# cortes-ciriano-lab/DeMethify

Hardware: AMD Instinct MI355X
Metric: NMF update iters/sec (1e6 CpG x 256 samples x 16 types) (higher is better)
Workload: dtype f64; 1 GPU; headline_1e6x256_12+4; N_cpg=1000000, S_samples=256, n_known=12, n_unknown=4, inner_iters=20, restarts=64, restart_seed=1 + k, restart_placement=k mod n_gpus, parallelism=restart-sharded x1

## Files before the change

demethify_amd/_lib.py:

```python
from __future__ import annotations

import ctypes as C
from pathlib import Path

LIB_PATH = Path(__file__).resolve().parent / "libdemethify_hip.so"

DMF_OK = 0
DMF_PTR_DEVICE = 1
DMF_INIT_IN_UNIT_RANGE = 4
DMF_SELECT_COUNTS_F32_EXACT, DMF_SELECT_PURITY, DMF_SELECT_ALPHA_OUTSIDE_UNIT, DMF_SELECT_V_UNALIGNED = 1, 2, 4, 8
DMF_SELECT_X16 = 16
DMF_COUNTS_F64 = 2
DMF_WLS_TARGET_V, DMF_WLS_TARGET_DV = 0, 1
DMF_WLS_F64_ARRAYS = 8
DMF_ERR_BAD_ARG, DMF_ERR_NONFINITE, DMF_ERR_UNSUPPORTED = 1, 4, 5
DMF_ERR_BAD_SHAPE = 2
DMF_GRAM_INTEGER, DMF_GRAM_FP64, DMF_GRAM_LAST = 0, 1, 2
DMF_ROUTE_SOLVER, DMF_ROUTE_UPDATE_U = 0, 1
MOMENTUM_SCALARS = ("a1", "a2", "l_w", "l_w_prev", "l_h", "l_h_prev", "dsq", "rt_norm2", "u_norm2", "cf", "cf_prev",
                    "iters", "done", "arrive", "mom_n", "mom_i")
REPORT_INTS = ("N", "S", "n_c", "ND", "SD", "N16", "plane_stride", "has_D16", "has_X16", "has_W16", "has_Dt8", "has_mask_bits",
               "rtp_width", "rtp_borrows_rt", "n_test", "d_f32_exact")
REPORT_DBLS = ("kDsq", "kRtSumsq", "kDmax", "kF32ResidualMax", "kIntCountMax", "kRtOutsideUnit", "x16_dev", "x16_sum")
PROBLEM_ARRAYS = {"V": 0, "D": 1, "Rt": 2, "Rtp": 3, "D16": 4, "X16": 5, "W16": 6, "Dt8": 7, "mask_bits": 8, "consts": 9}
DMF_MODE_PARTIAL = 0
DMF_MODE_UNSUPERVISED = 1
MAX_K = 64
SVD_MAX_S, SVD_MAX_NC, SVD_MAX_RANK, SVD_MAX_LDS = 512, 64, 64, 160 * 1024


def svd_project_lds_bytes(n_samples, rank):
    return 8 * (n_samples * rank + 8 * ((n_samples + 63) // 64 * 64 + 16) + 512)


KERNEL_ROWPASS, KERNEL_GRAM, KERNEL_ALPHA, KERNEL_COST = 0, 1, 2, 3
KERNEL_FAMILIES = ("rowpass", "gram", "alpha", "cost")

_p = C.c_void_p
_i64 = C.c_int64
_dbl_p = C.POINTER(C.c_double)

SIGNATURES = {
    "dmf_status_string": (C.c_char_p, [C.c_int]),
    "dmf_last_error": (C.c_char_p, []),
    "dmf_abi_version": (C.c_int, []),
    "dmf_context_create": (C.c_int, [C.c_int, _p, C.POINTER(_p)]),
    "dmf_context_destroy": (C.c_int, [_p]),
    "dmf_context_synchronize": (C.c_int, [_p]),
    "dmf_context_set_profiling": (C.c_int, [_p, C.c_int]),
    "dmf_context_kernel_time": (C.c_int, [_p, C.c_int, _dbl_p, C.POINTER(_i64)]),
    "dmf_context_reset_kernel_time": (C.c_int, [_p]),
    "dmf_context_set_generic": (C.c_int, [_p, C.c_int]),
    "dmf_context_set_x16": (C.c_int, [_p, C.c_int]),
    "dmf_context_set_rowpass_pair": (C.c_int, [_p, C.c_int]),
    "dmf_context_set_stop_confirmation": (C.c_int, [_p, C.c_int]),
    "dmf_problem_create": (C.c_int, [_p, _i64, _i64, _i64, _p, _p, _p, C.c_int, C.POINTER(_p)]),
    "dmf_problem_gather": (C.c_int, [_p, _p, _p, _i64, C.POINTER(_p)]),
    "dmf_problem_gather_device": (C.c_int, [_p, _p, _p, _i64, C.POINTER(_p)]),
    "dmf_problem_mask": (C.c_int, [_p, _p, _p, C.c_int, C.POINTER(_p)]),
    "dmf_solver_holdout_error": (C.c_int, [_p, _p, _dbl_p, C.POINTER(_i64)]),
    "dmf_problem_destroy": (C.c_int, [_p]),
    "dmf_problem_shape": (C.c_int, [_p, C.POINTER(_i64), C.POINTER(_i64), C.POINTER(_i64)]),
    "dmf_problem_gram_known": (C.c_int, [_p, _p, C.c_char_p, _i64]),
    "dmf_problem_report": (C.c_int, [_p, C.POINTER(_i64), _dbl_p]),
    "dmf_problem_copy_out": (C.c_int, [_p, C.c_int, _p, _i64]),
    "dmf_gram_i8_describe": (C.c_int, [_i64, _i64, _i64, _i64, C.c_int, C.c_char_p, _i64]),
    "dmf_solver_gram": (C.c_int, [_p, C.c_int, _p, C.c_char_p, _i64]),
    "dmf_solver_row_moments": (C.c_int, [_p, _p, C.c_char_p, _i64]),
    "dmf_solver_momentum_state": (C.c_int, [_p, _dbl_p, _p, _p]),
    "dmf_cost": (C.c_int, [_p, _p, _p, _i64, _p, C.c_int, _dbl_p]),
    "dmf_cost_describe": (C.c_int, [_i64, _i64, _i64, C.c_int, _i64, C.c_int, C.c_int, C.c_int, C.c_char_p, _i64]),
    "dmf_problem_cost_describe": (C.c_int, [_p, _p, _i64, C.c_char_p, _i64]),
    "dmf_project_simplex": (C.c_int, [_p, _p, _i64, _i64, C.c_double, C.c_int, _p]),
    "dmf_update_u": (C.c_int, [_p, _p, _p, _p, _p, _i64, _i64, C.c_int, C.c_int, _dbl_p, _p, _p]),
    "dmf_update_alpha": (C.c_int, [_p, _p, _p, _i64, _p, _p, _i64, C.c_int, _dbl_p, _p, _p]),
    "dmf_wls_intercept": (C.c_int, [_p, _p, _p, _i64, C.c_int, C.c_int, _p, C.POINTER(C.c_int)]),
    "dmf_svd_gram": (C.c_int, [_p, _p, _p, C.c_int, _p, C.POINTER(_i64)]),
    "dmf_svd_factor": (C.c_int, [_p, _p, _p, _p, _i64, C.c_int, _p, C.POINTER(_p)]),
    "dmf_svd_finish": (C.c_int, [_p, _p, _i64, _i64, _p, _p, C.c_int, _p]),
    "dmf_percentile_axis0": (C.c_int, [_p, _p, _i64, _i64, _p, _i64, C.c_int, _p]),
    "dmf_solver_create": (C.c_int, [_p, _p, _p, _p, _i64, C.c_int, C.c_int, C.POINTER(_p)]),
    "dmf_solver_set_purity": (C.c_int, [_p, _p, C.c_int]),
    "dmf_solver_step": (C.c_int, [_p, _i64, _i64, C.c_double, C.POINTER(_i64), C.POINTER(C.c_int)]),
    "dmf_solver_get": (C.c_int, [_p, C.c_int, _p, _p, _dbl_p, C.POINTER(_i64)]),
    "dmf_solver_match_components": (C.c_int, [_p, _p, _i64, _p, _p]),
    "dmf_solver_get_u_permuted": (C.c_int, [_p, C.POINTER(C.c_int32), _p]),
    "dmf_solver_cost": (C.c_int, [_p, _dbl_p]),
    "dmf_solver_cost_begin": (C.c_int, [_p]),
    "dmf_solver_cost_end": (C.c_int, [_p, _dbl_p]),
    "dmf_solver_destroy": (C.c_int, [_p]),
    "dmf_solver_describe": (C.c_int, [_p, _i64, C.c_char_p, _i64]),
    "dmf_select_describe": (C.c_int, [_i64, _i64, _i64, _i64, C.c_int, C.c_int, _i64, C.c_int, C.c_char_p, _i64]),
    "dmf_u_phase_describe": (C.c_int, [_i64, _i64, _i64, _i64, C.c_int, C.c_int, _i64, C.c_int, C.c_int, C.c_char_p, _i64]),
    "dmf_solver_u_phase_describe": (C.c_int, [_p, _i64, C.c_int, C.c_char_p, _i64]),
    "dmf_solver_stop_info": (C.c_int, [_p, C.POINTER(C.c_int), C.POINTER(_i64), C.POINTER(_i64), _dbl_p]),
    "dmf_solver_rowpass_launches": (C.c_int, [_p, C.POINTER(_i64), C.POINTER(_i64)]),
    "dmf_table_scan": (C.c_int, [C.c_char_p, C.c_char, C.POINTER(_i64), C.POINTER(C.c_int), C.POINTER(C.c_int),
                                 C.POINTER(C.c_int)]),
    "dmf_table_read": (C.c_int, [C.c_char_p, C.c_char, C.c_int, C.c_int, _i64, _p, _i64, C.c_double, _p, _i64, C.c_int]),
    "dmf_host_alloc": (_p, [C.c_size_t, C.POINTER(C.c_int)]),
    "dmf_host_free": (None, [_p, C.c_int]),
    "dmf_write_interval_csv": (C.c_int, [C.c_char_p, C.c_char_p, _p, _p, _i64, C.c_int, C.c_int, C.c_int]),
    "dmf_stage_upload": (C.c_int, [_p, _p, C.c_size_t, C.POINTER(C.c_void_p)]),
    "dmf_stage_free": (C.c_int, [_p, _p]),
    "dmf_stage_download": (C.c_int, [_p, _p, C.c_size_t, _p]),
    "dmf_mask_draw": (C.c_int, [_p, _p, C.POINTER(C.c_int), _i64, _i64, C.c_uint64, C.POINTER(C.c_void_p),
                                C.POINTER(_i64)]),
    "dmf_solve": (C.c_int, [_p, _p, _p, _p, _i64, C.c_int, _i64, _i64, C.c_double, C.c_int, _p, _p,
                            _dbl_p, C.POINTER(_i64)]),
}

_lib = None


class DemethifyHipError(RuntimeError):

    def __init__(self, status: int, where: str, detail: str = ""):
        self.status = status
        msg = f"{where}: status {status}"
        if detail:
            msg += f" ({detail})"
        super().__init__(msg)


def _preload_torch_hip_runtime():
    import importlib.util
    import os

    if os.environ.get("DEMETHIFY_SYSTEM_HIP") == "1":
        return
    try:
        spec = importlib.util.find_spec("torch")
        if spec is None or not spec.submodule_search_locations:
            return
        cand = Path(list(spec.submodule_search_locations)[0]) / "lib" / "libamdhip64.so"
        if cand.exists():
            C.CDLL(str(cand), mode=C.RTLD_GLOBAL)
    except Exception:
        pass


def load():
    global _lib
    if _lib is not None:
        return _lib
    if not LIB_PATH.exists():
        raise ImportError(
            f"{LIB_PATH} is missing: build it with `python -m demethify_amd._build` "
            "(there is no CPU fallback)")
    import sys

    torch = sys.modules.get("torch")
    if torch is not None:
        try:
            if torch.cuda.is_available():
# ... 21 lines not shown
```

demethify_amd/csrc/dmf_api.h:

```cpp
#pragma once
#include <hip/hip_runtime.h>

#include <cmath>
#include <cstdio>
#include <cstdlib>
#include <cstring>
#include <memory>
#include <mutex>
#include <new>
#include <unordered_map>
#include <utility>
#include <vector>

#include "../../include/demethify_hip.h"
#include "dmf_internal.h"
#include "dmf_select.h"

using dmf::SolverState;

namespace dmf_api {

int hip_fail(hipError_t e, const char* what, const char* file, int line);

#define HIP_TRY(expr)                                                                          \
    do {                                                                                       \
        hipError_t e_ = (expr);                                                                \
        if (e_ != hipSuccess) return dmf_api::hip_fail(e_, #expr, __FILE_NAME__, __LINE__);    \
    } while (0)

#define DMF_TRY(expr)                 \
    do {                              \
        int s_ = (expr);              \
        if (s_ != DMF_OK) return s_;  \
    } while (0)

constexpr int kEventPool = 2048;

struct FamilyClock {
    std::vector<hipEvent_t> start, stop;
    int used = 0;
    double total_ms = 0.0;
    int64_t launches = 0;
};

}

struct dmf_context {
    int device = 0;
    hipStream_t stream = nullptr;
    bool own_stream = false;
    unsigned profiling = 0;
    int stop_confirmation = 0;
    int generic_level = 0;
    bool x16 = true;
    bool rowpass_pair = true;
    double* scratch = nullptr;
    hipMemPool_t pool = nullptr;
    std::unordered_map<void*, size_t> live;
    std::unordered_map<size_t, std::vector<void*>> kept;
    size_t kept_bytes = 0;
    std::vector<hipEvent_t> events;
    std::vector<double*> pinned_moms;
    std::vector<void*> pinned_states;
    hipStream_t copy_stream = nullptr;
    std::mutex copy_mutex;
    dmf_api::FamilyClock clocks[DMF_KERNEL_FAMILIES];
};

namespace dmf_api {

hipError_t pool_alloc(dmf_context* ctx, void** p, size_t bytes);
void pool_free(dmf_context* ctx, void* p);
hipError_t stage_alloc(dmf_context* ctx, hipStream_t st, void** p, size_t bytes);
void stage_release(dmf_context* ctx, hipStream_t st, void* p);

template <class T>
class DevBuf {
  public:
    DevBuf() = default;
    DevBuf(DevBuf&& o) noexcept : ctx_(o.ctx_), ptr_(o.ptr_), owned_(o.owned_), stage_(o.stage_) {
        o.ptr_ = nullptr, o.owned_ = false;
    }
    DevBuf& operator=(DevBuf&& o) noexcept {
        if (this != &o) {
            reset();
            ctx_ = o.ctx_, ptr_ = o.ptr_, owned_ = o.owned_, stage_ = o.stage_;
            o.ptr_ = nullptr, o.owned_ = false;
        }
        return *this;
    }
    ~DevBuf() { reset(); }
    hipError_t alloc(dmf_context* ctx, size_t count) {
        reset();
        const hipError_t e = pool_alloc(ctx, (void**)&ptr_, count * sizeof(T));
        if (e != hipSuccess) ptr_ = nullptr;
        ctx_ = ctx, owned_ = e == hipSuccess, stage_ = nullptr;
        return e;
    }
    hipError_t alloc_staged(dmf_context* ctx, size_t count, hipStream_t st) {
        reset();
        const hipError_t e = stage_alloc(ctx, st, (void**)&ptr_, count * sizeof(T));
        if (e != hipSuccess) ptr_ = nullptr;
        ctx_ = ctx, owned_ = e == hipSuccess, stage_ = st;
        return e;
    }
    T* release() {
        T* p = ptr_;
        ptr_ = nullptr, owned_ = false;
        return p;
    }
    void borrow(const T* p) { reset(), ptr_ = const_cast<T*>(p); }
    void reset() {
        if (owned_ && stage_ != nullptr) stage_release(ctx_, stage_, ptr_);
        else if (owned_) pool_free(ctx_, ptr_);
        ptr_ = nullptr, owned_ = false;
    }
    T* get() const { return ptr_; }
    operator T*() const { return ptr_; }
    T* operator->() const { return ptr_; }

  private:
    dmf_context* ctx_ = nullptr;
    T* ptr_ = nullptr;
    bool owned_ = false;
    hipStream_t stage_ = nullptr;
};

enum ProblemConst { kDsq, kRtSumsq, kDmax, kF32ResidualMax, kIntCountMax, kRtOutsideUnit, kProblemConsts };

struct JobTable {
    std::vector<short> h_k, h_l;
    std::vector<int> h_dst;
    DevBuf<short> k, l;
    DevBuf<int> dst;
    int n = 0;
    template <class Keep>
    void build(int l_first, int l_last, Keep keep) {
        for (int ll = l_first; ll <= l_last; ++ll)
            for (int kk = 0; kk <= ll; ++kk) {
                if (!keep(kk, ll)) continue;
                h_k.push_back((short)kk);
                h_l.push_back((short)ll);
                h_dst.push_back(dmf::tri(kk, ll));
            }
        n = (int)h_k.size();
    }
    int upload(dmf_context* ctx) {
        HIP_TRY(k.alloc(ctx, n));
        HIP_TRY(l.alloc(ctx, n));
        HIP_TRY(dst.alloc(ctx, n));
        HIP_TRY(hipMemcpyAsync(k, h_k.data(), n * sizeof(short), hipMemcpyHostToDevice, ctx->stream));
        HIP_TRY(hipMemcpyAsync(l, h_l.data(), n * sizeof(short), hipMemcpyHostToDevice, ctx->stream));
        HIP_TRY(hipMemcpyAsync(dst, h_dst.data(), n * sizeof(int), hipMemcpyHostToDevice, ctx->stream));
        return DMF_OK;
    }
};

}

struct dmf_problem {
    dmf_context* ctx = nullptr;
    int64_t N = 0, S = 0, n_c = 0;
    dmf_api::DevBuf<double> V, D, Rt;
    dmf_api::DevBuf<double> Rtp;
    dmf_api::DevBuf<double> consts;
    double h_consts[dmf_api::kProblemConsts] = {};
    dmf_api::DevBuf<unsigned short> D16;
    dmf_api::DevBuf<signed char> Dt8;
    int ND = 0;
    int SD = 0;
    int64_t N16 = 0, plane_stride = 0;
    dmf_api::DevBuf<unsigned short> X16;
    double x16_dev = 0.0, x16_sum = 0.0;
    bool d_f32_exact = false;
    dmf_api::DevBuf<double> gb_known;
    dmf::GramRan known_ran;
    dmf_api::DevBuf<unsigned char> mask_bits;
    dmf_api::DevBuf<unsigned short> W16;
    int64_t n_test = 0;
    dmf::ProblemView view() const {
        dmf::ProblemView v;
        v.V = V, v.D = D, v.D16 = D16, v.X16 = X16, v.Dt8 = Dt8;
        v.plane_stride = plane_stride, v.SD = SD, v.ND = ND;
        v.Rt = Rt, v.Rtp = Rtp;
        v.N = N, v.S = (int)S, v.n_c = (int)n_c;
        return v;
    }
};

constexpr size_t kPinnedStateBytes = (sizeof(SolverState) + 15) / 16 * 16 + 16;

struct dmf_solver {
    dmf_context* ctx = nullptr;
    const dmf_problem* p = nullptr;
    int64_t n_u = 0;
    int mode = 0;
    dmf::ShapeKey key;
    dmf::PathSpec spec;
    dmf_api::DevBuf<double> cm;
    dmf_api::DevBuf<double> beta_tab;
    int64_t beta_cap = 0;
    dmf_api::DevBuf<long long> slab_i8;
    int64_t slab_i8_words = 0;
    dmf_api::DevBuf<long long> acc_i8;
    dmf_api::DevBuf<double> purity;
    dmf_api::DevBuf<double> u2_partials;
    dmf_api::DevBuf<double> u, u_prev, u_next;
    dmf_api::DevBuf<double> alpha, alpha_prev;
    dmf_api::DevBuf<double> gb;
    dmf::GramRan last_gram;
    int last_gram_source = -1;
    dmf_api::DevBuf<double> slab;
    int64_t slab_doubles = 0;
    dmf_api::DevBuf<double> partials;
    dmf_api::DevBuf<SolverState> state;
    SolverState* h_state = nullptr;
    dmf_api::JobTable jobs;
    bool cf_pending = true;
    double* mom_host = nullptr;
    dmf_api::DevBuf<double> mom_dev;
    hipEvent_t cost_event = nullptr;
    bool cost_pending = false;
    bool in_flight = false;
    bool confirm_stops = false;
    double cf_stream = 0.0;
    long long cf_stream_iter = -1;
    long long n_rowpass = 0, n_rowpass_pair = 0;
    long long n_confirmed = 0, n_unconfirmed = 0;
    dmf::IterateView iterate() const {
        dmf::IterateView it;
        it.u = u, it.u_prev = u_prev, it.alpha = alpha, it.state = state;
        it.n_u = (int)n_u, it.mode = mode;
        return it;
    }
    dmf::AlphaView alpha_view() const {
        dmf::AlphaView a;
        a.gb = gb, a.alpha = alpha, a.alpha_prev = alpha_prev, a.purity = purity, a.state = state, a.partials = partials;
        a.S = (int)p->S, a.n_c = (int)p->n_c, a.n_u = (int)n_u;
        return a;
    }
    dmf::UScratch scratch() const {
        dmf::UScratch sc;
        sc.cm = cm, sc.beta = beta_tab, sc.slab = slab, sc.u2_partials = u2_partials;
        return sc;
    }
};

namespace dmf_api {

struct HandleDeleter {
    void operator()(dmf_problem* p) const { dmf_problem_destroy(p); }
    void operator()(dmf_solver* s) const { dmf_solver_destroy(s); }
};
using ProblemPtr = std::unique_ptr<dmf_problem, HandleDeleter>;
using SolverPtr = std::unique_ptr<dmf_solver, HandleDeleter>;

int clock_drain(dmf_context* ctx, FamilyClock& c);

struct FamilyScope {
    dmf_context* ctx;
    FamilyClock* c = nullptr;
    int slot = -1;
    FamilyScope(dmf_context* ctx_, int family) : ctx(ctx_) {
        if (!((ctx->profiling >> family) & 1u)) return;
        c = &ctx->clocks[family];
        if (c->start.empty()) {
            c->start.resize(kEventPool);
            c->stop.resize(kEventPool);
            for (int i = 0; i < kEventPool; ++i) {
                hipEventCreateWithFlags(&c->start[i], hipEventDisableSystemFence);
                hipEventCreateWithFlags(&c->stop[i], hipEventDisableSystemFence);
            }
        }
        if (c->used == kEventPool) clock_drain(ctx, *c);
        slot = c->used++;
        hipEventRecord(c->start[slot], ctx->stream);
    }
    ~FamilyScope() {
        if (c != nullptr) hipEventRecord(c->stop[slot], ctx->stream);
    }
};

int check_ctx(dmf_context* ctx);

template <class T>
int import_array(dmf_context* ctx, const void* src, size_t count, int flags, DevBuf<T>& dst) {
    dst.reset();
    if (count == 0) return DMF_OK;
    if (flags & DMF_PTR_DEVICE) {
        dst.borrow(static_cast<const T*>(src));
        return DMF_OK;
    }
    HIP_TRY(dst.alloc(ctx, count));
    HIP_TRY(hipMemcpyAsync(dst, src, count * sizeof(T), hipMemcpyHostToDevice, ctx->stream));
    HIP_TRY(hipStreamSynchronize(ctx->stream));
    return DMF_OK;
}
int export_array(dmf_context* ctx, const void* dev_src, size_t bytes, int flags, void* dst);

hipError_t enqueue_cost(dmf_context* ctx, const dmf::ProblemView& p, const double* u, const double* alpha, int n_u,
                        double* scratch, double* out);
// ... 14 lines not shown
```

demethify_amd/csrc/dmf_api_context.hip:

```cpp
#include "dmf_api.h"

namespace dmf_api {

static thread_local char g_last_error[512] = "";

int hip_fail(hipError_t e, const char* what, const char* file, int line) {
    snprintf(g_last_error, sizeof(g_last_error), "%s failed at %s:%d: %s", what, file, line, hipGetErrorString(e));
    return DMF_ERR_HIP;
}

int clock_drain(dmf_context* ctx, FamilyClock& c) {
    if (c.used == 0) return DMF_OK;
    HIP_TRY(hipStreamSynchronize(ctx->stream));
    for (int i = 0; i < c.used; ++i) {
        float ms = 0.f;
        HIP_TRY(hipEventElapsedTime(&ms, c.start[i], c.stop[i]));
        c.total_ms += ms;
    }
    c.launches += c.used;
    c.used = 0;
    return DMF_OK;
}

static bool pool_enabled() {
// ... 206 lines not shown
    if (ctx == nullptr || key == nullptr || pos == nullptr || out_bits == nullptr || n_kept == nullptr) return DMF_ERR_BAD_ARG;
    *out_bits = nullptr;
    if (*pos < 0 || *pos > 624 || N < 1 || S < 1 || threshold > ((uint64_t)1 << 53)) return DMF_ERR_BAD_ARG;
    if (S > dmf::kMaskDrawMaxS || N > dmf::kMaskDrawMaxElements / S) return DMF_ERR_UNSUPPORTED;
    HIP_TRY(hipSetDevice(ctx->device));
    std::lock_guard<std::mutex> lock(ctx->copy_mutex);
    if (ctx->copy_stream == nullptr) HIP_TRY(hipStreamCreateWithFlags(&ctx->copy_stream, hipStreamNonBlocking));
    const hipStream_t st = ctx->copy_stream;
    constexpr size_t kStateWords = 624 + 4;
    DevBuf<unsigned char> bits;
    DevBuf<uint32_t> state;
    HIP_TRY(bits.alloc_staged(ctx, (size_t)N * (size_t)((S + 7) / 8), st));
    HIP_TRY(state.alloc_staged(ctx, kStateWords, st));
    uint32_t h_state[kStateWords] = {};
    std::memcpy(h_state, key, 624 * sizeof(uint32_t));
    HIP_TRY(hipMemcpyAsync(state, h_state, sizeof(h_state), hipMemcpyHostToDevice, st));
    HIP_TRY(dmf::launch_mask_draw(state, *pos, N, S, threshold, bits, reinterpret_cast<unsigned long long*>(state + 624), st));
    HIP_TRY(hipMemcpyAsync(h_state, state, sizeof(h_state), hipMemcpyDeviceToHost, st));
    HIP_TRY(hipStreamSynchronize(st));
    unsigned long long result[2];
    std::memcpy(result, h_state + 624, sizeof(result));
    std::memcpy(key, h_state, 624 * sizeof(uint32_t));
    *pos = (int)result[1];
    *n_kept = (int64_t)result[0];
    *out_bits = bits.release();
    return DMF_OK;
}

int dmf_stage_free(dmf_context* ctx, void* dev) {
    if (ctx == nullptr) return DMF_ERR_BAD_ARG;
    if (dev == nullptr) return DMF_OK;
    HIP_TRY(hipSetDevice(ctx->device));
    pool_free(ctx, dev);
    return DMF_OK;
}

int dmf_context_synchronize(dmf_context* ctx) {
    DMF_TRY(check_ctx(ctx));
    HIP_TRY(hipStreamSynchronize(ctx->stream));
    return DMF_OK;
}

int dmf_context_set_profiling(dmf_context* ctx, int enabled) {
    DMF_TRY(check_ctx(ctx));
    if (!enabled)
        for (auto& c : ctx->clocks) DMF_TRY(clock_drain(ctx, c));
    ctx->profiling = enabled == 0 ? 0u : enabled == 1 ? ~0u : (unsigned)enabled >> 1;
    return DMF_OK;
}

int dmf_context_kernel_time(dmf_context* ctx, int family, double* total_ms, int64_t* launches) {
    DMF_TRY(check_ctx(ctx));
    if (family < 0 || family >= DMF_KERNEL_FAMILIES) return DMF_ERR_BAD_ARG;
    FamilyClock& c = ctx->clocks[family];
    DMF_TRY(clock_drain(ctx, c));
    if (total_ms) *total_ms = c.total_ms;
    if (launches) *launches = c.launches;
    return DMF_OK;
}

int dmf_context_reset_kernel_time(dmf_context* ctx) {
    DMF_TRY(check_ctx(ctx));
    for (auto& c : ctx->clocks) {
        DMF_TRY(clock_drain(ctx, c));
        c.total_ms = 0.0;
        c.launches = 0;
    }
    return DMF_OK;
}

int dmf_context_set_generic(dmf_context* ctx, int enabled) {
    if (ctx == nullptr) return DMF_ERR_BAD_ARG;
    if (enabled < 0 || enabled > 4) return DMF_ERR_BAD_ARG;
    ctx->generic_level = enabled;
    return DMF_OK;
}

int dmf_context_set_x16(dmf_context* ctx, int enabled) {
    if (ctx == nullptr || enabled < 0 || enabled > 1) return DMF_ERR_BAD_ARG;
    ctx->x16 = enabled != 0;
    return DMF_OK;
}

int dmf_context_set_rowpass_pair(dmf_context* ctx, int enabled) {
    if (ctx == nullptr || enabled < 0 || enabled > 1) return DMF_ERR_BAD_ARG;
    ctx->rowpass_pair = enabled != 0;
    return DMF_OK;
}

int dmf_context_set_stop_confirmation(dmf_context* ctx, int mode) {
    if (ctx == nullptr || mode < 0 || mode > 2) return DMF_ERR_BAD_ARG;
    ctx->stop_confirmation = mode;
    return DMF_OK;
}

}
```

demethify_amd/csrc/dmf_api_entry.hip:

```cpp
#include "dmf_api.h"

using namespace dmf_api;

static double advance_momentum(double a, int64_t n) {
    for (int64_t t = 0; t < n; ++t) a = (1.0 + std::sqrt(1.0 + 4.0 * a * a)) / 2.0;
    return a;
}

static dmf::PercentilePlan percentile_plan(int64_t n, double q_percent) {
#pragma clang fp contract(off)
    dmf::PercentilePlan pl{};
    const double quantile = q_percent / 100.0;
    const double vi = (double)(n - 1) * quantile;
    if (vi >= (double)(n - 1)) {
        pl.k_prev = pl.k_next = n - 1;
        pl.gamma = 0.0;
    } else if (vi < 0.0) {
        pl.k_prev = pl.k_next = 0;
        pl.gamma = 0.0;
    } else {
        const double fl = std::floor(vi);
        pl.k_prev = (long long)fl;
        pl.k_next = pl.k_prev + 1;
        pl.gamma = vi - fl;
    }
    return pl;
}

static int result_array(dmf_context* ctx, double* out, size_t count, int flags, DevBuf<double>& dst) {
    if (flags & DMF_PTR_DEVICE) dst.borrow(out);
    else HIP_TRY(dst.alloc(ctx, count));
    return DMF_OK;
}
static int deliver_result(dmf_context* ctx, const double* dev, size_t count, int flags, double* out) {
    if (!(flags & DMF_PTR_DEVICE)) HIP_TRY(hipMemcpyAsync(out, dev, count * sizeof(double), hipMemcpyDeviceToHost, ctx->stream));
    HIP_TRY(hipStreamSynchronize(ctx->stream));
    return DMF_OK;
}

extern "C" {

static int select_key(int64_t N, int64_t S, int64_t n_c, int64_t n_u, int nd, int level, int64_t n_iter2, int flags,
                      const char* buf, int64_t cap, dmf::ShapeKey& key) {
    if (buf == nullptr || cap < 1 || N < 1 || S < 1 || n_c < 0 || n_u < 1 || nd < 0 || nd > 2 || n_iter2 < 0 ||
        n_c + n_u > dmf::kMaxK)
        return DMF_ERR_BAD_ARG;
    key.N = N;
    key.S = (int)S;
    key.n_c = (int)n_c;
    key.n_u = (int)n_u;
    key.nd = (S >= 2 && S <= 2048 && n_c <= 48) ? nd : 0;
    key.SD = key.nd > 0 ? (int)((S + 63) / 64 * 64) : 0;
    key.level = level;
    key.d_f32_exact = (flags & DMF_SELECT_COUNTS_F32_EXACT) != 0;
    key.rtp_present = true;
    key.v_align = (flags & DMF_SELECT_V_UNALIGNED) ? 8 : 0;
    key.x16 = key.nd > 0 && (flags & DMF_SELECT_X16) != 0;
    key.rtp_align = 0;
    key.alpha_unit = !(flags & DMF_SELECT_ALPHA_OUTSIDE_UNIT);
    return DMF_OK;
}

int dmf_u_phase_describe(int64_t N, int64_t S, int64_t n_c, int64_t n_u, int nd, int level, int64_t n_iter2, int flags, int route,
                         char* buf, int64_t cap) {
    dmf::ShapeKey key;
    if (n_iter2 > (1 << 20) || S > (1 << 24) || (route != DMF_ROUTE_SOLVER && route != DMF_ROUTE_UPDATE_U)) return DMF_ERR_BAD_ARG;
    DMF_TRY(select_key(N, S, n_c, n_u, nd, level, n_iter2, flags, buf, cap, key));
    const dmf::PathSpec spec = dmf::select_path(key);
    if (!spec.supported) return DMF_ERR_UNSUPPORTED;
    dmf::describe_u_phase(key, spec, (int)n_iter2, (flags & DMF_SELECT_PURITY) != 0, route == DMF_ROUTE_UPDATE_U, buf, (size_t)cap);
    return DMF_OK;
}

int dmf_select_describe(int64_t N, int64_t S, int64_t n_c, int64_t n_u, int nd, int level, int64_t n_iter2, int flags,
                        char* buf, int64_t cap) {
    dmf::ShapeKey key;
    DMF_TRY(select_key(N, S, n_c, n_u, nd, level, n_iter2, flags, buf, cap, key));
    const dmf::PathSpec spec = dmf::select_path(key);
    if (!spec.supported) return DMF_ERR_UNSUPPORTED;
    const dmf::IterationPlan plan = dmf::plan_iteration(key, spec, (int)n_iter2, (flags & DMF_SELECT_PURITY) != 0);
    dmf::describe_plan(key, plan, buf, (size_t)cap);
    return DMF_OK;
}

int dmf_cost_describe(int64_t S, int64_t n_c, int64_t n_u, int has_u16, int64_t SD, int v_align, int rtp_present, int level,
                      char* buf, int64_t cap) {
    if (buf == nullptr || cap < 1 || S < 1 || S > (1 << 24) || n_c < 0 || n_u < 0 || n_c + n_u < 1 || n_c + n_u > dmf::kMaxK ||
        SD < 0 || SD > (1 << 24) || (has_u16 && SD < S) || v_align < 0 || v_align > 15 || level < 0 || level > 4)
        return DMF_ERR_BAD_ARG;
    dmf::CostKey key;
    key.S = (int)S;
    key.n_c = (int)n_c;
    key.n_u = (int)n_u;
    key.d16 = has_u16 != 0;
    key.SD = (int)SD;
    key.v_align = (unsigned)v_align;
    key.rtp_present = rtp_present != 0;
    key.level = level;
    dmf::describe_cost_plan(dmf::cost_plan(key), buf, (size_t)cap);
    return DMF_OK;
}

int dmf_gram_i8_describe(int64_t N, int64_t S, int64_t n_c, int64_t n_u, int nd, char* buf, int64_t cap) {
    if (buf == nullptr || cap < 1 || N < 1 || S < 1 || S > (1 << 24) || n_c < 0 || n_u < 0 || n_c + n_u < 1 ||
        n_c + n_u > dmf::kMaxK)
        return DMF_ERR_BAD_ARG;
    const dmf::GramI8Plan g = dmf::gram_i8_plan(N, (int)((S + 63) / 64 * 64), (int)n_c, (int)n_u, nd);
    if (!g.supported) return DMF_ERR_UNSUPPORTED;
    dmf::describe_gram_i8_plan(g, buf, (size_t)cap);
    return DMF_OK;
}

int dmf_cost(dmf_context* ctx, const dmf_problem* p, const double* u, int64_t n_u, const double* alpha,
             int flags, double* out_cost) {
    DMF_TRY(check_ctx(ctx));
    if (p == nullptr || alpha == nullptr || out_cost == nullptr || n_u < 0) return DMF_ERR_BAD_ARG;
    if (n_u > 0 && u == nullptr) return DMF_ERR_BAD_ARG;
    const int64_t K = p->n_c + n_u;
    if (K < 1) return DMF_ERR_BAD_ARG;
    DevBuf<double> du, da, dout;
    DMF_TRY(import_array(ctx, u, (size_t)p->N * n_u, flags, du));
    DMF_TRY(import_array(ctx, alpha, (size_t)K * p->S, flags, da));
    HIP_TRY(dout.alloc(ctx, 1));
    {
        FamilyScope scope(ctx, DMF_KERNEL_COST);
        HIP_TRY(enqueue_cost(ctx, p->view(), du, da, (int)n_u, ctx->scratch + 1024, dout));
    }
    HIP_TRY(hipMemcpyAsync(out_cost, dout, sizeof(double), hipMemcpyDeviceToHost, ctx->stream));
    HIP_TRY(hipStreamSynchronize(ctx->stream));
    return DMF_OK;
}

int dmf_project_simplex(dmf_context* ctx, const double* X, int64_t K, int64_t S, double z, int flags,
                        double* out) {
    DMF_TRY(check_ctx(ctx));
    if (X == nullptr || out == nullptr || K < 1 || S < 1) return DMF_ERR_BAD_ARG;
    if (K > dmf::kMaxK) return DMF_ERR_UNSUPPORTED;
    const size_t count = (size_t)K * S;
    DevBuf<double> dx, dout;
    DMF_TRY(import_array(ctx, X, count, flags, dx));
    DMF_TRY(result_array(ctx, out, count, flags, dout));
    HIP_TRY(dmf::launch_project_simplex(dx, dout, (int)K, (int)S, z, ctx->stream));
    return deliver_result(ctx, dout, count, flags, out);
}

int dmf_percentile_axis0(dmf_context* ctx, const double* x, int64_t n, int64_t m, const double* q, int64_t n_q,
                         int flags, double* out) {
    DMF_TRY(check_ctx(ctx));
    if (x == nullptr || q == nullptr || out == nullptr || n < 1 || m < 1 || n_q < 1) return DMF_ERR_BAD_ARG;
    for (int64_t i = 0; i < n_q; ++i)
        if (!(q[i] >= 0.0 && q[i] <= 100.0)) return DMF_ERR_BAD_ARG;
    if (n > dmf::percentile_max_replicates()) return DMF_ERR_UNSUPPORTED;
    DevBuf<double> dx, dout;
    DMF_TRY(import_array(ctx, x, (size_t)n * m, flags, dx));
    DMF_TRY(result_array(ctx, out, (size_t)n_q * m, flags, dout));
    for (int64_t i = 0; i < n_q; i += 2) {
        const dmf::PercentilePlan p0 = percentile_plan(n, q[i]);
        const bool two = i + 1 < n_q;
        const dmf::PercentilePlan p1 = two ? percentile_plan(n, q[i + 1]) : p0;
        HIP_TRY(dmf::launch_percentile_pair(dx, n, m, p0, p1, dout + i * m, two ? dout + (i + 1) * m : nullptr, ctx->stream));
    }
    return deliver_result(ctx, dout, (size_t)n_q * m, flags, out);
}

int dmf_update_u(dmf_context* ctx, const dmf_problem* p, const double* u, const double* u_prev,
                 const double* alpha, int64_t n_u, int64_t n_iter2, int mode, int flags,
                 double* scalars_io, double* out_u, double* out_u_prev) {
    if (u_prev == nullptr || scalars_io == nullptr || out_u == nullptr || out_u_prev == nullptr || n_iter2 < 0)
        return DMF_ERR_BAD_ARG;
    dmf_solver* raw = nullptr;
    DMF_TRY(dmf_solver_create(ctx, p, u, alpha, n_u, mode, flags, &raw));
    SolverPtr s(raw);
    const size_t un = (size_t)p->N * n_u * sizeof(double);
    const hipMemcpyKind in_kind = (flags & DMF_PTR_DEVICE) ? hipMemcpyDeviceToDevice : hipMemcpyHostToDevice;
    HIP_TRY(hipMemcpyAsync(s->u_prev, u_prev, un, in_kind, ctx->stream));
    DMF_TRY(fetch_state(raw));
    s->h_state->a1 = scalars_io[0];
    s->h_state->l_w_prev = scalars_io[1];
    s->h_state->l_w = scalars_io[2];
    DMF_TRY(push_state(raw));
    DMF_TRY(enqueue_u_phase(raw, (int)n_iter2, standalone_row_kind(raw, (int)n_iter2)));
    DMF_TRY(export_array(ctx, s->u, un, flags, out_u));
    DMF_TRY(export_array(ctx, s->u_prev, un, flags, out_u_prev));
// ... 34 lines not shown
```

demethify_amd/csrc/dmf_api_problem.hip:

```cpp
#include "dmf_api.h"

namespace dmf_api {

static int alloc_count_copies(dmf_problem* p, int ND, bool x16, bool w16) {
    dmf_context* ctx = p->ctx;
    p->ND = ND;
    p->SD = (int)((p->S + 63) / 64 * 64);
    p->N16 = (p->N + 15) / 16 * 16;
    p->plane_stride = ((p->N + 31) / 32) * (p->SD / 32) * 1024;
    const size_t u16_elems = (size_t)p->N16 * p->SD;
    HIP_TRY(p->D16.alloc(ctx, u16_elems));
    HIP_TRY(p->Dt8.alloc(ctx, (size_t)p->plane_stride * ND));
    if (x16) HIP_TRY(p->X16.alloc(ctx, u16_elems));
    if (w16) HIP_TRY(p->W16.alloc(ctx, u16_elems));
    return DMF_OK;
}

static void known_route(dmf_problem* p, const char* piece) {
    char* t = p->known_ran.text;
    const size_t have = std::strlen(t), cap = sizeof(p->known_ran.text);
    snprintf(t + have, cap - have, "%s%s", have > 0 ? " " : "", piece);
}

static int problem_finalize(dmf_problem* p, bool counts_done = false) {
    dmf_context* ctx = p->ctx;
    const int64_t N = p->N, S = p->S, n_c = p->n_c;
    double* const h = p->h_consts;
    HIP_TRY(p->consts.alloc(ctx, kProblemConsts));
    if (!counts_done) HIP_TRY(dmf::launch_max_f64(p->D, N * S, ctx->scratch, p->consts + kDmax, ctx->stream));
    if (n_c > 0) {
        HIP_TRY(dmf::launch_sumsq_f64(p->Rt, N * n_c, ctx->scratch + 1024, p->consts + kRtSumsq, nullptr, ctx->stream));
    } else {
        HIP_TRY(hipMemsetAsync(p->consts + kRtSumsq, 0, sizeof(double), ctx->stream));
    }
    if (!counts_done) {
        HIP_TRY(dmf::launch_f32_residual_max(p->D, N * S, ctx->scratch + 2048, p->consts + kF32ResidualMax, ctx->stream));
        HIP_TRY(dmf::launch_int_count_max(p->D, N * S, ctx->scratch + 3072, p->consts + kIntCountMax, ctx->stream));
        if (n_c > 0) {
            HIP_TRY(dmf::launch_unit_range_check(p->Rt, N * n_c, ctx->scratch, p->consts + kRtOutsideUnit, ctx->stream));
        } else {
            HIP_TRY(hipMemsetAsync(p->consts + kRtOutsideUnit, 0, sizeof(double), ctx->stream));
        }
    }
    {
        double got[kProblemConsts];
        HIP_TRY(hipMemcpyAsync(got, p->consts, sizeof(got), hipMemcpyDeviceToHost, ctx->stream));
        HIP_TRY(hipStreamSynchronize(ctx->stream));
        h[kRtSumsq] = got[kRtSumsq];
        if (!counts_done)
            for (int i = kDmax; i < kProblemConsts; ++i) h[i] = got[i];
    }
    h[kDsq] = h[kDmax] * h[kDmax];
    p->d_f32_exact = h[kF32ResidualMax] == 0.0;
    HIP_TRY(hipMemcpyAsync(p->consts, h, kProblemConsts * sizeof(double), hipMemcpyHostToDevice, ctx->stream));
    HIP_TRY(hipStreamSynchronize(ctx->stream));
    if (!std::isfinite(h[kDmax]) || !std::isfinite(h[kRtSumsq])) return DMF_ERR_NONFINITE;

    if (!counts_done && ctx->generic_level == 0 && h[kIntCountMax] <= 32639.0 && h[kRtOutsideUnit] == 0.0 && S >= 2 &&
        S <= 2048 && n_c <= 48) {
        DMF_TRY(alloc_count_copies(p, h[kIntCountMax] <= 127.0 ? 1 : 2, ctx->x16, false));
        DevBuf<unsigned long long> x_stats;
        if (ctx->x16) HIP_TRY(x_stats.alloc(ctx, 3));
        HIP_TRY(dmf::launch_build_counts_int(p->D, p->V, N, (int)S, p->ND, p->D16, p->X16, p->N16, p->SD, p->Dt8,
                                             p->plane_stride, x_stats, ctx->stream));
        if (p->X16 != nullptr) {
            unsigned long long got[3] = {1, 0, 0};
            HIP_TRY(hipMemcpyAsync(got, x_stats, sizeof(got), hipMemcpyDeviceToHost, ctx->stream));
            HIP_TRY(hipStreamSynchronize(ctx->stream));
            if (got[0] != 0) {
                p->X16.reset();
            } else {
                std::memcpy(&p->x16_dev, &got[1], sizeof(double));
                p->x16_sum = (double)got[2];
            }
        }
    }

    if (n_c > 0 && n_c <= 48) {
        const int nct = (int)((n_c + 3) / 4 * 4);
        if (nct == n_c) {
            p->Rtp.borrow(p->Rt);
        } else {
            HIP_TRY(p->Rtp.alloc(ctx, (size_t)N * nct));
            HIP_TRY(dmf::launch_pad_rows(p->Rt, p->Rtp, N, (int)n_c, nct, ctx->stream));
        }
    }

    const dmf::ProblemView pv = p->view();
    JobTable jobs;
    jobs.build(0, (int)n_c, [](int, int) { return true; });
    const int n_jobs = jobs.n;
    const bool mfma = n_c >= 1 && ctx->generic_level != 1 && ctx->generic_level != 2;
    const int n_fast = mfma ? n_jobs - 1 : 0, n_dense = (int)(n_c * (n_c + 1) / 2);
    const bool int_known = mfma && ctx->generic_level == 0 && p->Dt8 != nullptr && p->D16 != nullptr && p->Rtp != nullptr &&
                           (reinterpret_cast<uintptr_t>(p->Rtp.get()) & 15) == 0 &&
                           dmf::gram_i8_known_supported((int)n_c, p->ND, N, p->SD);
    int64_t slab_doubles = dmf::gram_slab_doubles(N, (int)S, mfma ? 1 : n_jobs);
    if (mfma && !int_known) {
        const int64_t need = dmf::gram_mfma_slab_doubles(N, (int)S, n_fast);
        if (need > slab_doubles) slab_doubles = need;
    }
    DevBuf<double> slab, slab_bu;
    DevBuf<long long> slab_i8, acc;
    HIP_TRY(p->gb_known.alloc(ctx, (size_t)n_jobs * S));
    DMF_TRY(jobs.upload(ctx));
    HIP_TRY(slab.alloc(ctx, (size_t)slab_doubles));
    bool vdv_done = true;
    if (int_known) {
        const int64_t slab_words = dmf::gram_i8_slab_words_nf(N, p->SD, n_dense);
        const int64_t acc_words = dmf::gram_i8_acc_words_nf((int)S, n_dense, (int)n_c + 1);
        HIP_TRY(slab_i8.alloc(ctx, (size_t)slab_words));
        HIP_TRY(acc.alloc(ctx, (size_t)acc_words));
        HIP_TRY(slab_bu.alloc(ctx, (size_t)dmf::bu_cols_grid(N) * (n_c + 1) * S));
        HIP_TRY(hipMemsetAsync(acc, 0, (size_t)acc_words * sizeof(long long), ctx->stream));
        int ny = 0, n_slabs = 0;
        dmf::GramRan ran;
        HIP_TRY(dmf::launch_gram_i8(pv, nullptr, 0, jobs.k, jobs.l, n_dense, slab_i8, slab_words, nullptr, &ny, ctx->stream, &ran));
        known_route(p, "int_known");
        known_route(p, ran.text);
        HIP_TRY(dmf::launch_bu_cols(pv, p->Rt, (int)n_c, slab_bu, nullptr, &n_slabs, ctx->stream, &vdv_done));
        known_route(p, vdv_done ? "+ k_bu_cols2 with vDv" : "+ k_bu_cols");
        HIP_TRY(dmf::launch_gram_v2_reduce(slab_i8, ny, n_dense, p->SD, slab_bu, n_slabs, (int)n_c + (vdv_done ? 1 : 0), (int)S,
                                           acc, jobs.dst, p->gb_known, nullptr, nullptr, 0, nullptr, ctx->stream));
    } else if (mfma) {
        dmf::GramJobTable fast{jobs.k, jobs.l, jobs.dst, n_fast};
        int ny = 0;
        dmf::GramRan ran;
        HIP_TRY(dmf::launch_gram_mfma(pv, nullptr, 0, fast, n_dense, slab, slab_doubles, nullptr, &ny, ctx->stream, &ran));
        known_route(p, "fp64");
        known_route(p, ran.text);
        HIP_TRY(dmf::launch_gram_reduce(slab, ny, n_fast, (int)S, jobs.dst, p->gb_known, nullptr, ctx->stream));
    }
    if (int_known && vdv_done) {
    } else if (n_jobs - n_fast == 1 && ctx->generic_level != 1 && ctx->generic_level != 2 &&
               (int64_t)dmf::vdv_cols_grid(N) * S <= slab_doubles) {
        HIP_TRY(dmf::launch_vdv_cols(pv, slab, p->gb_known + (int64_t)jobs.h_dst[n_jobs - 1] * S, ctx->stream));
        known_route(p, p->known_ran.text[0] == 0 ? "fp64 k_vdv_cols" : "+ k_vdv_cols");
    } else {
        dmf::GramJobTable rest{jobs.k + n_fast, jobs.l + n_fast, jobs.dst + n_fast, n_jobs - n_fast};
        dmf::GramRan ran;
        if (p->known_ran.text[0] == 0) known_route(p, "fp64");
        else known_route(p, "+");
        HIP_TRY(dmf::launch_gram(pv, nullptr, 0, rest, slab, slab_doubles, p->gb_known, nullptr, ctx->stream, &ran));
        known_route(p, ran.text);
    }
    HIP_TRY(hipStreamSynchronize(ctx->stream));
    return DMF_OK;
}

static dmf::CostPlan cost_plan_of(dmf_context* ctx, const dmf::ProblemView& p, int n_u) {
    return dmf::cost_plan(dmf::cost_key(p, n_u, ctx->generic_level));
}

hipError_t enqueue_cost(dmf_context* ctx, const dmf::ProblemView& p, const double* u, const double* alpha, int n_u,
                        double* scratch, double* out) {
    return dmf::launch_cost_plan(cost_plan_of(ctx, p, n_u), p, u, alpha, n_u, scratch, out, ctx->stream);
}

bool cost_reads_u16_only(dmf_context* ctx, const dmf::ProblemView& p, int n_u) { return cost_plan_of(ctx, p, n_u).d16; }

int cost_to_host(dmf_context* ctx, const dmf::ProblemView& p, const double* u, const double* alpha, int n_u,
                 double* host_slot, bool wait) {
    {
        FamilyScope scope(ctx, DMF_KERNEL_COST);
        HIP_TRY(enqueue_cost(ctx, p, u, alpha, n_u, ctx->scratch + 1024, ctx->scratch + 3072));
    }
    HIP_TRY(hipMemcpyAsync(host_slot, ctx->scratch + 3072, sizeof(double), hipMemcpyDeviceToHost, ctx->stream));
    if (wait) HIP_TRY(hipStreamSynchronize(ctx->stream));
    return DMF_OK;
}

static int problem_gather(dmf_context* ctx, const dmf_problem* src, const int64_t* idx, int64_t n_idx, bool idx_dev,
                          dmf_problem** out) {
    DevBuf<long long> d_idx;
    if (idx_dev) {
        DevBuf<unsigned int> d_bad;
        unsigned int h_bad = 1;
        HIP_TRY(d_bad.alloc(ctx, 1));
        HIP_TRY(dmf::launch_index_range_check(reinterpret_cast<const long long*>(idx), n_idx, src->N, d_bad, ctx->stream));
        HIP_TRY(hipMemcpyAsync(&h_bad, d_bad, sizeof(h_bad), hipMemcpyDeviceToHost, ctx->stream));
        HIP_TRY(hipStreamSynchronize(ctx->stream));
        if (h_bad != 0) return DMF_ERR_BAD_ARG;
        d_idx.borrow(reinterpret_cast<const long long*>(idx));
    } else {
        HIP_TRY(d_idx.alloc(ctx, (size_t)n_idx));
        HIP_TRY(hipMemcpyAsync(d_idx, idx, (size_t)n_idx * sizeof(long long), hipMemcpyHostToDevice, ctx->stream));
    }
    ProblemPtr p(new (std::nothrow) dmf_problem());
    if (p == nullptr) return DMF_ERR_BAD_ARG;
    p->ctx = ctx;
    p->N = n_idx;
    p->S = src->S;
    p->n_c = src->n_c;
    HIP_TRY(p->V.alloc(ctx, (size_t)n_idx * p->S));
    HIP_TRY(p->D.alloc(ctx, (size_t)n_idx * p->S));
    if (p->n_c > 0) HIP_TRY(p->Rt.alloc(ctx, (size_t)n_idx * p->n_c));
    HIP_TRY(dmf::launch_gather_rows(src->V, p->V, d_idx, n_idx, p->S, ctx->stream));
    HIP_TRY(dmf::launch_gather_rows(src->D, p->D, d_idx, n_idx, p->S, ctx->stream));
    if (p->n_c > 0) HIP_TRY(dmf::launch_gather_rows(src->Rt, p->Rt, d_idx, n_idx, p->n_c, ctx->stream));
    bool counts_done = false;
    if (src->D16 != nullptr && src->ND > 0 && ctx->generic_level == 0) {
        const bool x16 = src->X16 != nullptr && ctx->x16;
        DevBuf<unsigned int> d_max;
        DevBuf<unsigned long long> d_xsum;
        DMF_TRY(alloc_count_copies(p.get(), src->ND, x16, false));
        HIP_TRY(d_max.alloc(ctx, 1));
        if (x16) HIP_TRY(d_xsum.alloc(ctx, 1));
        HIP_TRY(dmf::launch_gather_counts_int(src->D16, x16 ? src->X16.get() : nullptr, d_idx, n_idx, p->SD, p->ND, p->D16,
                                              p->X16, p->N16, p->Dt8, p->plane_stride, d_max, d_xsum, ctx->stream));
        unsigned int h_max = 0;
        unsigned long long h_xsum = 0;
        HIP_TRY(hipMemcpyAsync(&h_max, d_max, sizeof(h_max), hipMemcpyDeviceToHost, ctx->stream));
        if (x16) HIP_TRY(hipMemcpyAsync(&h_xsum, d_xsum, sizeof(h_xsum), hipMemcpyDeviceToHost, ctx->stream));
        HIP_TRY(hipStreamSynchronize(ctx->stream));
        p->h_consts[kDmax] = p->h_consts[kIntCountMax] = (double)h_max;
        p->h_consts[kF32ResidualMax] = src->h_consts[kF32ResidualMax];
        p->h_consts[kRtOutsideUnit] = src->h_consts[kRtOutsideUnit];
        p->x16_dev = x16 ? src->x16_dev : 0.0;
        p->x16_sum = (double)h_xsum;
        counts_done = true;
    }
    HIP_TRY(hipStreamSynchronize(ctx->stream));
    d_idx.reset();
    DMF_TRY(problem_finalize(p.get(), counts_done));
    *out = p.release();
    return DMF_OK;
}

}

using namespace dmf_api;

extern "C" {

int dmf_problem_create(dmf_context* ctx, int64_t N, int64_t S, int64_t n_c, const double* V,
                       const void* counts, const double* Rt, int flags, dmf_problem** out) {
    DMF_TRY(check_ctx(ctx));
    if (out == nullptr) return DMF_ERR_BAD_ARG;
    *out = nullptr;
    if (N <= 0 || S <= 0 || n_c < 0 || V == nullptr || counts == nullptr) return DMF_ERR_BAD_ARG;
    if (n_c > 0 && Rt == nullptr) return DMF_ERR_BAD_ARG;
    if (n_c > dmf::kMaxK || S > (1 << 24)) return DMF_ERR_UNSUPPORTED;
    ProblemPtr p(new (std::nothrow) dmf_problem());
    if (p == nullptr) return DMF_ERR_BAD_ARG;
    p->ctx = ctx;
    p->N = N;
    p->S = S;
    p->n_c = n_c;
    DMF_TRY(import_array(ctx, V, (size_t)N * S, flags, p->V));
    if (flags & DMF_COUNTS_F64) {
        DMF_TRY(import_array(ctx, counts, (size_t)N * S, flags, p->D));
    } else {
        DevBuf<long long> raw;
        DMF_TRY(import_array(ctx, counts, (size_t)N * S, flags, raw));
        HIP_TRY(p->D.alloc(ctx, (size_t)N * S));
        HIP_TRY(dmf::launch_convert_counts(raw, p->D, N * S, ctx->stream));
        HIP_TRY(hipStreamSynchronize(ctx->stream));
    }
    DMF_TRY(import_array(ctx, Rt, (size_t)N * n_c, flags, p->Rt));
    DMF_TRY(problem_finalize(p.get()));
    *out = p.release();
    return DMF_OK;
}

int dmf_problem_gather(dmf_context* ctx, const dmf_problem* src, const int64_t* idx, int64_t n_idx,
                       dmf_problem** out) {
    DMF_TRY(check_ctx(ctx));
    if (src == nullptr || idx == nullptr || out == nullptr || n_idx <= 0) return DMF_ERR_BAD_ARG;
    *out = nullptr;
    if (src->mask_bits != nullptr) return DMF_ERR_BAD_ARG;
    for (int64_t r = 0; r < n_idx; ++r)
        if (idx[r] < 0 || idx[r] >= src->N) return DMF_ERR_BAD_ARG;
    return problem_gather(ctx, src, idx, n_idx, false, out);
}

int dmf_problem_gather_device(dmf_context* ctx, const dmf_problem* src, const int64_t* idx_dev, int64_t n_idx,
                              dmf_problem** out) {
    DMF_TRY(check_ctx(ctx));
    if (src == nullptr || idx_dev == nullptr || out == nullptr || n_idx <= 0) return DMF_ERR_BAD_ARG;
    *out = nullptr;
    if (src->mask_bits != nullptr) return DMF_ERR_BAD_ARG;
    return problem_gather(ctx, src, idx_dev, n_idx, true, out);
}

int dmf_problem_mask(dmf_context* ctx, const dmf_problem* src, const uint8_t* train_bits, int flags, dmf_problem** out) {
    DMF_TRY(check_ctx(ctx));
    if (src == nullptr || train_bits == nullptr || out == nullptr) return DMF_ERR_BAD_ARG;
    *out = nullptr;
    if (src->ctx != ctx || src->mask_bits != nullptr) return DMF_ERR_BAD_ARG;
    ProblemPtr p(new (std::nothrow) dmf_problem());
    if (p == nullptr) return DMF_ERR_BAD_ARG;
    const int64_t N = src->N, S = src->S, n_c = src->n_c;
    p->ctx = ctx;
    p->N = N;
    p->S = S;
    p->n_c = n_c;
    const size_t bit_bytes = (size_t)N * (size_t)((S + 7) / 8), elems = (size_t)N * S;
    HIP_TRY(p->mask_bits.alloc(ctx, bit_bytes));
    HIP_TRY(hipMemcpyAsync(p->mask_bits, train_bits, bit_bytes,
                           (flags & DMF_PTR_DEVICE) ? hipMemcpyDeviceToDevice : hipMemcpyHostToDevice, ctx->stream));
    HIP_TRY(p->V.alloc(ctx, elems));
    HIP_TRY(p->D.alloc(ctx, elems));
    if (n_c > 0) {
        HIP_TRY(p->Rt.alloc(ctx, (size_t)N * n_c));
        HIP_TRY(hipMemcpyAsync(p->Rt, src->Rt, (size_t)N * n_c * sizeof(double), hipMemcpyDeviceToDevice, ctx->stream));
    }
    const bool ints = src->D16 != nullptr && src->ND > 0 && ctx->generic_level == 0;
    const bool x16 = ints && src->X16 != nullptr && ctx->x16;
    if (ints) DMF_TRY(alloc_count_copies(p.get(), src->ND, x16, true));
    DevBuf<unsigned long long> d_stats;
    HIP_TRY(d_stats.alloc(ctx, 3));
    HIP_TRY(dmf::launch_mask_problem(src->V, src->D, ints ? src->D16.get() : nullptr, x16 ? src->X16.get() : nullptr,
                                     p->mask_bits, p->V, p->D, p->D16, p->X16, p->W16, N, p->N16, (int)S, p->SD, d_stats,
                                     ctx->stream));
    if (ints) HIP_TRY(dmf::launch_build_dt8(p->D16, N, p->SD, p->ND, p->Dt8, p->plane_stride, ctx->stream));
    unsigned long long h_stats[3] = {0, 0, 0};
    HIP_TRY(hipMemcpyAsync(h_stats, d_stats, sizeof(h_stats), hipMemcpyDeviceToHost, ctx->stream));
    HIP_TRY(hipStreamSynchronize(ctx->stream));
    d_stats.reset();
    double dmax;
    std::memcpy(&dmax, &h_stats[0], sizeof(dmax));
    p->h_consts[kDmax] = dmax;
    p->h_consts[kF32ResidualMax] = src->h_consts[kF32ResidualMax];
    p->h_consts[kIntCountMax] = std::isfinite(src->h_consts[kIntCountMax]) ? dmax : src->h_consts[kIntCountMax];
    p->h_consts[kRtOutsideUnit] = src->h_consts[kRtOutsideUnit];
    p->x16_dev = x16 ? src->x16_dev : 0.0;
    p->x16_sum = (double)h_stats[1];
    p->n_test = (int64_t)h_stats[2];
    DMF_TRY(problem_finalize(p.get(), true));
    *out = p.release();
    return DMF_OK;
}

int dmf_problem_destroy(dmf_problem* p) {
    if (p == nullptr) return DMF_OK;
    hipSetDevice(p->ctx->device);
    delete p;
    return DMF_OK;
}

int dmf_problem_cost_describe(dmf_context* ctx, const dmf_problem* p, int64_t n_u, char* buf, int64_t cap) {
    if (ctx == nullptr || p == nullptr || buf == nullptr || cap < 1 || n_u < 0 || p->ctx != ctx) return DMF_ERR_BAD_ARG;
    if (p->n_c + n_u < 1 || p->n_c + n_u > dmf::kMaxK) return DMF_ERR_BAD_ARG;
    dmf::describe_cost_plan(cost_plan_of(ctx, p->view(), (int)n_u), buf, (size_t)cap);
    return DMF_OK;
}

int dmf_problem_gram_known(const dmf_problem* p, double* out, char* out_text, int64_t cap) {
    if (p == nullptr || out == nullptr || (out_text != nullptr && cap < 1)) return DMF_ERR_BAD_ARG;
    dmf_context* ctx = p->ctx;
    DMF_TRY(check_ctx(ctx));
    const size_t n = (size_t)(p->n_c + 1) * (p->n_c + 2) / 2 * p->S;
    HIP_TRY(hipMemcpyAsync(out, p->gb_known, n * sizeof(double), hipMemcpyDeviceToHost, ctx->stream));
    HIP_TRY(hipStreamSynchronize(ctx->stream));
    if (out_text != nullptr) snprintf(out_text, (size_t)cap, "%s", p->known_ran.text);
    return DMF_OK;
}

int dmf_problem_report(const dmf_problem* p, int64_t* out_ints, double* out_dbls) {
    if (p == nullptr || out_ints == nullptr || out_dbls == nullptr) return DMF_ERR_BAD_ARG;
    const int64_t rtp_width = p->Rtp != nullptr ? (p->n_c + 3) / 4 * 4 : 0;
    const int64_t ints[DMF_REPORT_INTS] = {p->N, p->S, p->n_c, p->ND, p->SD, p->N16, p->plane_stride,
                                           p->D16 != nullptr, p->X16 != nullptr, p->W16 != nullptr, p->Dt8 != nullptr,
                                           p->mask_bits != nullptr, rtp_width,
                                           p->Rtp != nullptr && p->Rtp.get() == p->Rt.get(), p->n_test, p->d_f32_exact};
    std::memcpy(out_ints, ints, sizeof(ints));
    for (int i = 0; i < kProblemConsts; ++i) out_dbls[i] = p->h_consts[i];
    out_dbls[kProblemConsts] = p->x16_dev;
    out_dbls[kProblemConsts + 1] = p->x16_sum;
    return DMF_OK;
}

int dmf_problem_copy_out(const dmf_problem* p, int which, void* out, int64_t bytes) {
    if (p == nullptr || out == nullptr) return DMF_ERR_BAD_ARG;
    dmf_context* ctx = p->ctx;
    DMF_TRY(check_ctx(ctx));
    const size_t elems = (size_t)p->N * p->S, u16_bytes = (size_t)p->N16 * p->SD * sizeof(unsigned short);
    const void* src = nullptr;
    size_t size = 0;
    switch (which) {
        case DMF_ARRAY_V: src = p->V, size = elems * sizeof(double); break;
        case DMF_ARRAY_D: src = p->D, size = elems * sizeof(double); break;
        case DMF_ARRAY_RT: src = p->Rt, size = (size_t)p->N * p->n_c * sizeof(double); break;
        case DMF_ARRAY_RTP: src = p->Rtp, size = (size_t)p->N * ((p->n_c + 3) / 4 * 4) * sizeof(double); break;
        case DMF_ARRAY_D16: src = p->D16, size = u16_bytes; break;
        case DMF_ARRAY_X16: src = p->X16, size = u16_bytes; break;
        case DMF_ARRAY_W16: src = p->W16, size = u16_bytes; break;
        case DMF_ARRAY_DT8: src = p->Dt8, size = (size_t)p->plane_stride * p->ND; break;
        case DMF_ARRAY_MASK_BITS: src = p->mask_bits, size = (size_t)p->N * (size_t)((p->S + 7) / 8); break;
        case DMF_ARRAY_CONSTS: src = p->consts, size = kProblemConsts * sizeof(double); break;
        default: return DMF_ERR_BAD_ARG;
    }
    if (src == nullptr || size == 0) return DMF_ERR_BAD_ARG;
    if (bytes < 0 || (size_t)bytes != size) return DMF_ERR_BAD_SHAPE;
    return export_array(ctx, src, size, 0, out);
}

int dmf_problem_shape(const dmf_problem* p, int64_t* N, int64_t* S, int64_t* n_c) {
    if (p == nullptr) return DMF_ERR_BAD_ARG;
    if (N) *N = p->N;
    if (S) *S = p->S;
    if (n_c) *n_c = p->n_c;
    return DMF_OK;
}

}
```

demethify_amd/csrc/dmf_api_solver.hip:

```cpp
#include "dmf_api.h"

namespace dmf_api {

using dmf::kSplitInnerSteps;

static int ensure_split_scratch(dmf_solver* s, int n_iter2) {
    dmf_context* ctx = s->ctx;
    if (s->cm == nullptr) HIP_TRY(s->cm.alloc(ctx, (size_t)dmf::u_phase_split_cm_doubles(s->p->N, (int)s->n_u)));
    if (s->beta_cap < n_iter2 || s->beta_tab == nullptr) {
        s->beta_cap = n_iter2 > 0 ? n_iter2 : 1;
        HIP_TRY(s->beta_tab.alloc(ctx, (size_t)s->beta_cap));
    }
    return DMF_OK;
}

int enqueue_u_phase(dmf_solver* s, int n_iter2, dmf::RowKind row) {
    dmf_context* ctx = s->ctx;
    const dmf::ProblemView pv = s->p->view();
    FamilyScope scope(ctx, DMF_KERNEL_ROWPASS);
    switch (row) {
        case dmf::RowKind::CmI8InnerRows:
            DMF_TRY(ensure_split_scratch(s, n_iter2));
            HIP_TRY(dmf::launch_u_phase_split_i8(pv, s->iterate(), n_iter2, s->scratch(), ctx->stream));
            return DMF_OK;
// ... 113 lines not shown
    return enqueue_alpha_phase(s, alpha, n_iter2);
}

static int enqueue_outer_iteration(dmf_solver* s, int n_iter2) {
    dmf_context* ctx = s->ctx;
    s->in_flight = true;
    const dmf_problem* p = s->p;
    const int S = (int)p->S;
    const dmf::IterationPlan plan = dmf::plan_iteration(s->key, s->spec, n_iter2, s->purity != nullptr);
    if (plan.row == dmf::RowKind::RowpassV2) {
        int grid = 0;
        bool paired = false;
        {
            FamilyScope scope(ctx, DMF_KERNEL_ROWPASS);
            dmf::ProblemView pv = p->view();
            if (!s->key.x16) pv.X16 = nullptr;
            HIP_TRY(dmf::launch_rowpass_v2(pv, s->iterate(), n_iter2, s->scratch(), &grid, s->key.rowpass_pair, &paired,
                                           ctx->stream));
            ++s->n_rowpass;
            s->n_rowpass_pair += paired ? 1 : 0;
        }
        return enqueue_gram_i8_tail(s, plan.alpha, n_iter2, grid);
    }
    if (plan.row == dmf::RowKind::CmI8InnerBu) {
        int grid = 0;
        DMF_TRY(ensure_split_scratch(s, n_iter2));
        {
            FamilyScope scope(ctx, DMF_KERNEL_ROWPASS);
            HIP_TRY(dmf::launch_u_phase_split_i8_bu(p->view(), s->iterate(), n_iter2, s->scratch(), &grid, ctx->stream));
        }
        return enqueue_gram_i8_tail(s, plan.alpha, n_iter2, grid);
    }
    if (plan.row == dmf::RowKind::RowpassFused) {
        const int64_t n_full = p->N - (p->N & 15), n_tail = p->N - n_full;
        const dmf::ProblemView pv = p->view();
        int grid = 0, ny_tail = 0;
        {
            FamilyScope scope(ctx, DMF_KERNEL_ROWPASS);
            HIP_TRY(dmf::launch_rowpass_fused(pv.rows(0, n_full), s->iterate(), n_iter2, s->scratch(), &grid, ctx->stream));
        }
        if (n_tail > 0) {
            const dmf::ProblemView tail = pv.rows(n_full, n_tail);
            const dmf::IterateView it_tail = s->iterate().rows(n_full);
            HIP_TRY(dmf::launch_u_phase_mfma(tail, it_tail, n_iter2, ctx->stream));
            HIP_TRY(dmf::launch_sumsq_f64(it_tail.u, n_tail * s->n_u, ctx->scratch, s->u2_partials + grid, &s->state->done,
                                          ctx->stream));
            HIP_TRY(dmf::launch_gram_u(tail, it_tail.u, it_tail.n_u, s->slab + (int64_t)2 * grid * s->jobs.n * S,
                                       &s->state->done, &ny_tail, ctx->stream));
        }
        if (dmf::GramRan* ran = last_gram_slot(s, kLastGramFused))
            snprintf(ran->text, sizeof(ran->text), "k_rowpass_fused<%d,%d> phase C slabs=%d%s", (int)(p->n_c + 3) / 4, (int)s->n_u,
                     2 * grid, n_tail > 0 ? " + k_gram_u tail" : "");
        HIP_TRY(dmf::launch_finish_u_norm(s->u2_partials, grid + (n_tail > 0 ? 1 : 0), s->state, ctx->stream));
        {
            FamilyScope scope(ctx, DMF_KERNEL_GRAM);
            HIP_TRY(dmf::launch_gram_reduce(s->slab, 2 * grid + ny_tail, s->jobs.n, S, s->jobs.dst, s->gb,
                                            &s->state->done, ctx->stream));
        }
        return enqueue_alpha_phase(s, plan.alpha, n_iter2);
    }
    DMF_TRY(enqueue_u_phase(s, n_iter2, plan.row));
    HIP_TRY(dmf::launch_sumsq_f64(s->u, p->N * s->n_u, ctx->scratch, &s->state->u_norm2, &s->state->done,
                                  ctx->stream));
    HIP_TRY(dmf::launch_set_lh(s->state, ctx->stream));
    DMF_TRY(enqueue_gram(s, plan.gram, true, last_gram_slot(s, (int)plan.gram)));
    return enqueue_alpha_phase(s, plan.alpha, n_iter2);
}

int fetch_state(dmf_solver* s) {
    HIP_TRY(hipMemcpyAsync(s->h_state, s->state, sizeof(SolverState), hipMemcpyDeviceToHost, s->ctx->stream));
    HIP_TRY(hipStreamSynchronize(s->ctx->stream));
    s->in_flight = false;
    return DMF_OK;
}

int push_state(dmf_solver* s) {
    HIP_TRY(hipMemcpyAsync(s->state, s->h_state, sizeof(SolverState), hipMemcpyHostToDevice, s->ctx->stream));
    HIP_TRY(hipStreamSynchronize(s->ctx->stream));
    return DMF_OK;
}

constexpr int kMomRows = 64, kMomSteps = 64;

__global__ void k_set_momentum(SolverState* state, const double* mom, int stride, int rows, int n) {
    state->mom = mom;
    state->mom_stride = stride;
    state->mom_rows = rows;
    state->mom_i = 0;
    state->mom_n = n;
}

static double momentum_advance(double& a) {
#pragma clang fp contract(off)
    const double a0 = a;
    const double sq = 4.0 * a0 * a0;
    a = (1.0 + std::sqrt(1.0 + sq)) / 2.0;
    return (a0 - 1.0) / a;
}

static int upload_momentum_rows(dmf_solver* s, int rows, int n) {
    dmf_context* ctx = s->ctx;
    const int stride = 2 + 2 * n;
    if (s->mom_host == nullptr) {
        if (!ctx->pinned_moms.empty()) {
            s->mom_host = ctx->pinned_moms.back();
            ctx->pinned_moms.pop_back();
        } else {
            HIP_TRY(hipHostMalloc((void**)&s->mom_host, (size_t)kMomRows * (2 + 2 * kMomSteps) * sizeof(double)));
        }
        HIP_TRY(s->mom_dev.alloc(ctx, (size_t)kMomRows * (2 + 2 * kMomSteps)));
    }
    double a1 = s->h_state->a1, a2 = s->h_state->a2;
    for (int r = 0; r < rows; ++r) {
        double* row = s->mom_host + (size_t)r * stride;
        for (int t = 0; t < n; ++t) {
            row[2 + t] = momentum_advance(a1);
            row[2 + n + t] = momentum_advance(a2);
        }
        row[0] = a1;
        row[1] = a2;
    }
    HIP_TRY(hipMemcpyAsync(s->mom_dev, s->mom_host, (size_t)rows * stride * sizeof(double), hipMemcpyHostToDevice, ctx->stream));
    hipLaunchKernelGGL(k_set_momentum, dim3(1), dim3(1), 0, ctx->stream, s->state.get(), (const double*)s->mom_dev.get(), stride,
                       rows, n);
    HIP_TRY(hipGetLastError());
    return DMF_OK;
}

__global__ void k_set_tol(SolverState* state, double tol, double band) {
    state->tol = tol;
    state->band = band;
}

constexpr double kConfirmBand = 10.0;
constexpr double kGramCostRelErr = 1e-15;

static double* cost_slot(const dmf_solver* s) {
    return reinterpret_cast<double*>(reinterpret_cast<char*>(s->h_state) + kPinnedStateBytes - 16);
}

static int solver_setup(dmf_solver* s, const double* u0, const double* alpha0, int flags) {
    dmf_context* ctx = s->ctx;
    const dmf_problem* p = s->p;
    const int64_t N = p->N, S = p->S, n_c = p->n_c, n_u = s->n_u, K = n_c + n_u;
    dmf::ShapeKey& key = s->key;
    key.N = N;
    key.S = (int)S;
    key.n_c = (int)n_c;
    key.n_u = (int)n_u;
    key.nd = (p->ND > 0 && p->D16 != nullptr) ? p->ND : 0;
    key.SD = p->SD;
    key.x16 = key.nd > 0 && p->X16 != nullptr;
    key.rowpass_pair = ctx->rowpass_pair;
    key.level = ctx->generic_level;
    key.d_f32_exact = p->d_f32_exact;
    key.rtp_present = n_c == 0 || p->Rtp != nullptr;
    key.v_align = (unsigned)(reinterpret_cast<uintptr_t>(p->V.get()) & 15);
    key.rtp_align = (unsigned)(reinterpret_cast<uintptr_t>(p->Rtp.get()) & 15);
    key.alpha_unit = true;
    s->spec = dmf::select_path(key);
    if ((s->spec.use_v2 || s->spec.use_cm_i8) && !(flags & DMF_INIT_IN_UNIT_RANGE)) {
        bool in_unit = true;
        if (flags & DMF_PTR_DEVICE) {
            double outside = 0.0;
            HIP_TRY(dmf::launch_unit_range_check(alpha0, K * S, ctx->scratch, ctx->scratch + 2048, ctx->stream));
            HIP_TRY(hipMemcpyAsync(&outside, ctx->scratch + 2048, sizeof(double), hipMemcpyDeviceToHost, ctx->stream));
            HIP_TRY(hipStreamSynchronize(ctx->stream));
            in_unit = outside == 0.0;
        } else {
            for (int64_t i = 0; i < K * S; ++i)
                if (!(alpha0[i] >= 0.0 && alpha0[i] <= 1.0)) {
                    in_unit = false;
                    break;
                }
        }
        if (!in_unit) {
            key.alpha_unit = false;
            s->spec = dmf::select_path(key);
        }
    }
    if (!s->spec.supported) return DMF_ERR_UNSUPPORTED;
    s->in_flight = true;
    s->jobs.build((int)n_c, (int)K, [n_c, K](int k, int l) {
        if (l == (int)K && k < (int)n_c) return false;
        return !(l == (int)K && k == (int)K);
    });
    const int n_jobs = s->jobs.n;
    s->slab_doubles = dmf::gram_slab_doubles(N, (int)S, n_jobs);
    if (s->spec.use_gram_spec) {
        const int64_t spec = dmf::gram_u_slab_doubles(N, (int)S, (int)n_c, (int)n_u);
        if (spec > s->slab_doubles) s->slab_doubles = spec;
    }
    if (s->spec.use_gram_mfma) {
        const int64_t need = dmf::gram_mfma_slab_doubles(N, (int)S, n_jobs);
        if (need > s->slab_doubles) s->slab_doubles = need;
    }
    if (s->spec.use_fused) {
        const int64_t spec = dmf::rowpass_fused_slab_doubles(N - (N & 15), (int)S, (int)n_c, (int)n_u) +
                             dmf::gram_u_slab_doubles(16, (int)S, (int)n_c, (int)n_u);
        if (spec > s->slab_doubles) s->slab_doubles = spec;
    }
    if (s->spec.use_v2) {
        const int64_t bu = (int64_t)dmf::rowpass_v2_grid(N, (int)S) * n_u * S;
        if (bu > s->slab_doubles) s->slab_doubles = bu;
    }
    if (s->spec.use_gram_i8) {
        const int64_t bu = (int64_t)dmf::bu_cols_grid(N) * n_u * S;
        if (bu > s->slab_doubles) s->slab_doubles = bu;
        if (s->spec.use_cm_i8) {
            const int64_t bu2 = (int64_t)dmf::u_inner_bu_grid(N, (int)S) * n_u * S;
            if (bu2 > s->slab_doubles) s->slab_doubles = bu2;
        }
    }
    const size_t un = (size_t)N * n_u, an = (size_t)K * S;
    const size_t un_alloc = (un + 1) & ~(size_t)1;
    const size_t gbn = (size_t)(K + 1) * (K + 2) / 2 * S;
    const int nb_alpha = (int)((S + 63) / 64);
    HIP_TRY(s->u.alloc(ctx, un_alloc));
    HIP_TRY(s->u_prev.alloc(ctx, un_alloc));
    if (s->spec.u_path == 2) HIP_TRY(s->u_next.alloc(ctx, un_alloc));
    HIP_TRY(s->alpha.alloc(ctx, an));
    HIP_TRY(s->alpha_prev.alloc(ctx, an));
    HIP_TRY(s->gb.alloc(ctx, gbn));
    HIP_TRY(s->slab.alloc(ctx, (size_t)s->slab_doubles));
    HIP_TRY(s->partials.alloc(ctx, (size_t)2 * (nb_alpha + S)));
    HIP_TRY(s->u2_partials.alloc(ctx, 4096));
    if (s->spec.use_v2 || s->spec.use_gram_i8) {
        s->slab_i8_words = dmf::gram_i8_slab_words(N, p->SD, (int)n_c, (int)n_u);
        HIP_TRY(s->slab_i8.alloc(ctx, (size_t)s->slab_i8_words));
        const size_t acc_words = (size_t)dmf::gram_i8_acc_words((int)S, (int)n_c, (int)n_u);
        HIP_TRY(s->acc_i8.alloc(ctx, acc_words));
        HIP_TRY(hipMemsetAsync(s->acc_i8, 0, acc_words * sizeof(long long), ctx->stream));
    }
    HIP_TRY(s->state.alloc(ctx, 1));
    if (!ctx->pinned_states.empty()) {
        s->h_state = (SolverState*)ctx->pinned_states.back();
        ctx->pinned_states.pop_back();
    } else {
        HIP_TRY(hipHostMalloc((void**)&s->h_state, kPinnedStateBytes));
    }
    const hipMemcpyKind in_kind = (flags & DMF_PTR_DEVICE) ? hipMemcpyDeviceToDevice : hipMemcpyHostToDevice;
    HIP_TRY(hipMemsetAsync(s->state, 0, sizeof(SolverState), ctx->stream));
    HIP_TRY(hipMemsetAsync(s->gb, 0, gbn * sizeof(double), ctx->stream));
    HIP_TRY(hipMemcpyAsync(s->u, u0, un * sizeof(double), in_kind, ctx->stream));
    HIP_TRY(hipMemcpyAsync(s->u_prev, s->u, un * sizeof(double), hipMemcpyDeviceToDevice, ctx->stream));
    HIP_TRY(hipMemcpyAsync(s->alpha, alpha0, an * sizeof(double), in_kind, ctx->stream));
    HIP_TRY(hipMemcpyAsync(s->alpha_prev, s->alpha, an * sizeof(double), hipMemcpyDeviceToDevice, ctx->stream));
    DMF_TRY(s->jobs.upload(ctx));
    HIP_TRY(dmf::launch_scatter_known_block(p->gb_known, s->gb, (int)n_c, (int)K, (int)S, ctx->stream));
    HIP_TRY(dmf::launch_sumsq_f64(s->u, N * n_u, ctx->scratch, &s->state->u_norm2, nullptr, ctx->stream));
    HIP_TRY(dmf::launch_init_state(s->state, p->consts, s->alpha, (int)S, (int)n_c, (int)n_u, ctx->stream));
    if (!(flags & DMF_PTR_DEVICE)) HIP_TRY(hipStreamSynchronize(ctx->stream));
    return DMF_OK;
}

}

using namespace dmf_api;

extern "C" {

int dmf_solver_create(dmf_context* ctx, const dmf_problem* p, const double* u0, const double* alpha0,
                      int64_t n_u, int mode, int flags, dmf_solver** out) {
    DMF_TRY(check_ctx(ctx));
    if (out == nullptr) return DMF_ERR_BAD_ARG;
    *out = nullptr;
    if (p == nullptr || u0 == nullptr || alpha0 == nullptr || n_u < 1) return DMF_ERR_BAD_ARG;
    if (mode != DMF_MODE_PARTIAL && mode != DMF_MODE_UNSUPERVISED) return DMF_ERR_BAD_ARG;
    if (p->n_c + n_u > dmf::kMaxK) return DMF_ERR_UNSUPPORTED;
    SolverPtr s(new (std::nothrow) dmf_solver());
    if (s == nullptr) return DMF_ERR_BAD_ARG;
    s->ctx = ctx;
    s->p = p;
    s->n_u = n_u;
    s->mode = mode;
    DMF_TRY(solver_setup(s.get(), u0, alpha0, flags));
    *out = s.release();
    return DMF_OK;
}

int dmf_solver_step(dmf_solver* s, int64_t n_outer, int64_t n_iter2, double tol,
                    int64_t* iters_done_total, int* converged) {
    if (s == nullptr || n_outer < 0 || n_iter2 < 0 || n_iter2 > (1 << 20)) return DMF_ERR_BAD_ARG;
    dmf_context* ctx = s->ctx;
    DMF_TRY(check_ctx(ctx));
    const dmf_problem* p = s->p;
    const double gram_err = kGramCostRelErr * (double)p->N * (double)p->S * p->h_consts[kDmax] +
                            (s->key.x16 ? p->x16_dev * p->x16_sum : 0.0);
    s->confirm_stops = tol > 0.0 && ctx->stop_confirmation != 2 && (ctx->stop_confirmation == 1 || gram_err >= tol / 20.0);
    hipLaunchKernelGGL(k_set_tol, dim3(1), dim3(1), 0, ctx->stream, s->state.get(), tol, s->confirm_stops ? kConfirmBand : 1.0);
    HIP_TRY(hipGetLastError());
    if (s->cf_pending && tol > 0.0 && n_outer > 0) {
        FamilyScope scope(ctx, DMF_KERNEL_COST);
        HIP_TRY(enqueue_cost(ctx, p->view(), s->u, s->alpha, (int)s->n_u, ctx->scratch + 1024, &s->state->cf));
        s->cf_pending = false;
        s->cf_stream_iter = -2;
    }
    DMF_TRY(fetch_state(s));
    if (s->cf_stream_iter == -2) {
        s->cf_stream = s->h_state->cf;
        s->cf_stream_iter = s->h_state->iters;
    }
    int64_t check_every = s->spec.u_path != 2 ? 8 : 1;
    if (tol == 0.0 && s->spec.u_path != 2) check_every = kMomRows;
    const long long iters0 = s->h_state->iters;
    const dmf::IterationPlan plan = dmf::plan_iteration(s->key, s->spec, (int)n_iter2, s->purity != nullptr);
    const bool use_mom = n_iter2 >= 1 && n_iter2 <= kMomSteps && plan.row == dmf::RowKind::RowpassV2 &&
                         plan.alpha == dmf::AlphaKind::PhaseRow16;
    if (!use_mom && s->h_state->mom_n >= 0) {
        hipLaunchKernelGGL(k_set_momentum, dim3(1), dim3(1), 0, ctx->stream, s->state.get(), (const double*)nullptr, 0, 0, -1);
        HIP_TRY(hipGetLastError());
    }
    while (s->h_state->iters - iters0 < n_outer && s->h_state->done != 1) {
        const int64_t left = n_outer - (s->h_state->iters - iters0);
        const int64_t batch = left < check_every ? left : check_every;
        if (use_mom) DMF_TRY(upload_momentum_rows(s, (int)batch, (int)n_iter2));
        for (int64_t b = 0; b < batch; ++b) DMF_TRY(enqueue_outer_iteration(s, (int)n_iter2));
        DMF_TRY(fetch_state(s));
        if (s->h_state->iters > iters0) s->cf_pending = false;
        if (s->h_state->done == 2) {
            double cs = 0.0;
            DMF_TRY(cost_to_host(ctx, p->view(), s->u, s->alpha, (int)s->n_u, &cs, true));
            bool stop;
            if (s->cf_stream_iter == s->h_state->iters - 1) {
                stop = std::fabs(cs - s->cf_stream) < tol;
                s->n_confirmed += 1;
            } else {
                stop = std::fabs(s->h_state->cf - s->h_state->cf_prev) < tol;
                s->n_unconfirmed += 1;
            }
            s->cf_stream = cs;
            s->cf_stream_iter = s->h_state->iters;
            s->h_state->done = stop ? 1 : 0;
            DMF_TRY(push_state(s));
            check_every = 1;
        } else if (s->spec.u_path != 2 && check_every < 64 && check_every > 1) {
            check_every *= 2;
        }
    }
    if (iters_done_total) *iters_done_total = s->h_state->iters;
    if (converged) *converged = s->h_state->done == 1;
    return DMF_OK;
}

int dmf_solver_set_purity(dmf_solver* s, const double* purity, int flags) {
    if (s == nullptr || purity == nullptr) return DMF_ERR_BAD_ARG;
    dmf_context* ctx = s->ctx;
    DMF_TRY(check_ctx(ctx));
    if (s->mode != DMF_MODE_PARTIAL) return DMF_ERR_BAD_ARG;
    const size_t bytes = (size_t)s->p->S * sizeof(double);
    if (s->purity == nullptr) HIP_TRY(s->purity.alloc(ctx, (size_t)s->p->S));
    const hipMemcpyKind kind = (flags & DMF_PTR_DEVICE) ? hipMemcpyDeviceToDevice : hipMemcpyHostToDevice;
    HIP_TRY(hipMemcpyAsync(s->purity, purity, bytes, kind, ctx->stream));
    HIP_TRY(hipStreamSynchronize(ctx->stream));
    return DMF_OK;
}

int dmf_solver_get(dmf_solver* s, int flags, double* out_u, double* out_alpha, double* out_cost,
                   int64_t* out_iters) {
    if (s == nullptr) return DMF_ERR_BAD_ARG;
    dmf_context* ctx = s->ctx;
    DMF_TRY(check_ctx(ctx));
    const dmf_problem* p = s->p;
    DMF_TRY(export_array(ctx, s->u, (size_t)p->N * s->n_u * sizeof(double), flags, out_u));
    DMF_TRY(export_array(ctx, s->alpha, (size_t)(p->n_c + s->n_u) * p->S * sizeof(double), flags, out_alpha));
    if (s->cf_pending && out_cost != nullptr) {
        FamilyScope scope(ctx, DMF_KERNEL_COST);
        HIP_TRY(enqueue_cost(ctx, p->view(), s->u, s->alpha, (int)s->n_u, ctx->scratch + 1024, &s->state->cf));
        s->cf_pending = false;
    }
    DMF_TRY(fetch_state(s));
    if (out_cost) *out_cost = s->h_state->cf;
    if (out_iters) *out_iters = s->h_state->iters;
    return DMF_OK;
}

int dmf_solver_cost(dmf_solver* s, double* out_cost) {
    if (s == nullptr || out_cost == nullptr) return DMF_ERR_BAD_ARG;
    DMF_TRY(check_ctx(s->ctx));
    return cost_to_host(s->ctx, s->p->view(), s->u, s->alpha, (int)s->n_u, out_cost, true);
}

int dmf_solver_cost_begin(dmf_solver* s) {
    if (s == nullptr) return DMF_ERR_BAD_ARG;
    dmf_context* ctx = s->ctx;
    DMF_TRY(check_ctx(ctx));
    if (s->cost_event == nullptr) {
        if (!ctx->events.empty()) {
            s->cost_event = ctx->events.back();
            ctx->events.pop_back();
        } else {
            HIP_TRY(hipEventCreateWithFlags(&s->cost_event, hipEventDisableTiming));
        }
    }
    DMF_TRY(cost_to_host(ctx, s->p->view(), s->u, s->alpha, (int)s->n_u, cost_slot(s), false));
    HIP_TRY(hipEventRecord(s->cost_event, ctx->stream));
    s->cost_pending = true;
    return DMF_OK;
}

int dmf_solver_cost_end(dmf_solver* s, double* out_cost) {
    if (s == nullptr || out_cost == nullptr || !s->cost_pending) return DMF_ERR_BAD_ARG;
    DMF_TRY(check_ctx(s->ctx));
    HIP_TRY(hipEventSynchronize(s->cost_event));
    s->cost_pending = false;
    *out_cost = *cost_slot(s);
    return DMF_OK;
}

int dmf_solver_holdout_error(dmf_solver* s, const dmf_problem* full, double* sum_sq, int64_t* n_test) {
    if (s == nullptr || full == nullptr || sum_sq == nullptr || n_test == nullptr) return DMF_ERR_BAD_ARG;
    dmf_context* ctx = s->ctx;
    DMF_TRY(check_ctx(ctx));
    const dmf_problem* p = s->p;
    if (p->mask_bits == nullptr || full->mask_bits != nullptr || full->ctx != ctx) return DMF_ERR_BAD_ARG;
    if (full->N != p->N || full->S != p->S || full->n_c != p->n_c) return DMF_ERR_BAD_SHAPE;
    *n_test = p->n_test;
    *sum_sq = 0.0;
    if (p->n_test == 0) return DMF_OK;
    dmf::ProblemView pv;
    pv.N = p->N, pv.S = (int)p->S, pv.n_c = (int)p->n_c;
    pv.V = full->V, pv.Rt = p->Rt, pv.Rtp = p->Rtp;
// ... 177 lines not shown
```

demethify_amd/csrc/dmf_internal.h:

```cpp
#pragma once
#include <hip/hip_runtime.h>
#include <stdint.h>

#include "dmf_select.h"

namespace dmf {

struct SolverState {
    double a1;
    double a2;
    double l_w;
    double l_w_prev;
    double l_h;
    double l_h_prev;
    double dsq;
    double rt_norm2;
    double u_norm2;
    double cf;
    double cf_prev;
    double tol;
    long long iters;
    double band;
    int done;
    int arrive;
    const double* mom;
    int mom_stride, mom_rows, mom_i, mom_n;
};

__device__ __forceinline__ const double* momentum_row(const SolverState* __restrict__ state, int n_iter2) {
    return (state->mom != nullptr && state->mom_n == n_iter2 && state->mom_i < state->mom_rows)
               ? state->mom + (int64_t)state->mom_i * state->mom_stride
               : nullptr;
}

__host__ __device__ inline int tri(int k, int l) { return l * (l + 1) / 2 + k; }

constexpr int kMaxK = 64;
constexpr int kGramChunk = 16;
constexpr int kRowsPerBlockU = 64;

struct GramJobTable {
    const short* k_idx;
    const short* l_idx;
    const int* dst_row;
    int count;
};

struct PercentilePlan {
    long long k_prev, k_next;
    double gamma;
    int from_top;
    int pad;
};

struct ProblemView {
    const double* V = nullptr;
    const double* D = nullptr;
    const unsigned short* D16 = nullptr;
    const unsigned short* X16 = nullptr;
    const signed char* Dt8 = nullptr;
    int64_t plane_stride = 0;
    int SD = 0, ND = 0;
    const double* Rt = nullptr;
    const double* Rtp = nullptr;
    int64_t N = 0;
    int S = 0, n_c = 0;
    unsigned v_align() const { return (unsigned)(reinterpret_cast<uintptr_t>(V) & 15); }
    ProblemView rows(int64_t first, int64_t count) const {
        ProblemView r;
        r.V = V + first * S;
        r.D = D + first * S;
        r.Rt = Rt ? Rt + first * n_c : nullptr;
        r.Rtp = Rtp ? Rtp + first * ((n_c + 3) / 4 * 4) : nullptr;
        r.N = count;
        r.S = S;
        r.n_c = n_c;
        return r;
    }
};

struct IterateView {
    double* u = nullptr;
    double* u_prev = nullptr;
    const double* alpha = nullptr;
    SolverState* state = nullptr;
    int n_u = 0, mode = 0;
    IterateView rows(int64_t first) const {
        IterateView r = *this;
        r.u = u + first * n_u;
        r.u_prev = u_prev + first * n_u;
        return r;
    }
};

struct AlphaView {
    const double* gb = nullptr;
    double* alpha = nullptr;
    double* alpha_prev = nullptr;
    const double* purity = nullptr;
    SolverState* state = nullptr;
    double* partials = nullptr;
    int S = 0, n_c = 0, n_u = 0;
};

struct UScratch {
    double* cm = nullptr;
    double* beta = nullptr;
    double* slab = nullptr;
    double* u2_partials = nullptr;
};


hipError_t launch_convert_counts(const long long* src, double* dst, int64_t n, hipStream_t st);
hipError_t launch_max_f64(const double* x, int64_t n, double* scratch, double* out, hipStream_t st);
hipError_t launch_f32_residual_max(const double* x, int64_t n, double* scratch, double* out, hipStream_t st);
hipError_t launch_int_count_max(const double* x, int64_t n, double* scratch, double* out, hipStream_t st);
hipError_t launch_unit_range_check(const double* x, int64_t n, double* scratch, double* out, hipStream_t st);
hipError_t launch_sumsq_f64(const double* x, int64_t n, double* scratch, double* out,
                            const int* done_flag, hipStream_t st);
hipError_t launch_pad_rows(const double* src, double* dst, int64_t n_rows, int width_src, int width_dst,
                           hipStream_t st);
hipError_t launch_index_range_check(const long long* idx, int64_t n_idx, int64_t n_src, unsigned int* flag, hipStream_t st);
hipError_t launch_gather_rows(const double* src, double* dst, const long long* idx, int64_t n_idx,
                              int64_t width, hipStream_t st);

inline CostKey cost_key(const ProblemView& p, int n_u, int level) {
    CostKey k;
    k.S = p.S, k.n_c = p.n_c, k.n_u = n_u;
    k.d16 = p.D16 != nullptr;
    k.SD = p.SD;
    k.v_align = p.v_align();
    k.rtp_present = p.Rtp != nullptr;
    k.level = level;
    return k;
}
hipError_t launch_cost_plan(const CostPlan& plan, const ProblemView& p, const double* u, const double* alpha, int n_u,
                            double* scratch, double* out, hipStream_t st);
int vdv_cols_grid(int64_t N);
hipError_t launch_vdv_cols(const ProblemView& p, double* slab, double* out, hipStream_t st);

struct GramRan {
    char text[192] = "";
};

hipError_t launch_gram(const ProblemView& p, const double* u, int n_u, GramJobTable jobs, double* slab, int64_t slab_doubles,
                       double* gb, const int* done_flag, hipStream_t st, GramRan* ran = nullptr);
int64_t gram_slab_doubles(int64_t N, int S, int n_jobs);
hipError_t launch_gram_reduce(const double* slab, int ny, int n_jobs, int S, const int* dst_row,
                              double* gb, const int* done_flag, hipStream_t st);
bool gram_u_supported(int n_c, int n_u);
int64_t gram_u_slab_doubles(int64_t N, int S, int n_c, int n_u);
hipError_t launch_gram_u(const ProblemView& p, const double* u, int n_u, double* slab, const int* done_flag, int* ny_out,
                         hipStream_t st, GramRan* ran = nullptr);

struct RowLaunch {
    bool supported = false;
    int nw = 0;
    int grid = 0;
    size_t lds = 0;
    bool raise = false;
    int64_t blocks_per_wg = 0;
};
struct UPhaseMfmaPlan : RowLaunch {
    int nkc = 0, nu = 0;
    bool vec = false, d16 = false;
    bool split = false;
};
UPhaseMfmaPlan u_phase_mfma_plan(int64_t N, int S, int n_c, int n_u, int n_iter2, bool has_d16, int SD, bool split);
struct RowpassFusedPlan : RowLaunch {
    int nkc = 0, nu = 0;
};
RowpassFusedPlan rowpass_fused_plan(int64_t N, int S, int n_c, int n_u, int n_iter2);
struct UPhaseBigPlan : RowLaunch {
    int nkc = 0, gs = 16, n_u = 0;
};
UPhaseBigPlan u_phase_big_plan(int64_t N, int S, int n_c, int n_u, int n_iter2);
struct UPhaseGramPlan : RowLaunch {
    int nu = 0;
    bool alpha_in_lds = false;
};
UPhaseGramPlan u_phase_gram_plan(int64_t N, int S, int n_c, int n_u);
struct UStepDirectPlan : RowLaunch {
    int n_u = 0;
};
UStepDirectPlan u_step_direct_plan(int64_t N, int S, int n_c, int n_u);
int describe_row_launch(const UPhaseMfmaPlan& g, char* buf, size_t cap);
int describe_row_launch(const RowpassFusedPlan& g, char* buf, size_t cap);
int describe_row_launch(const UPhaseBigPlan& g, char* buf, size_t cap);
int describe_row_launch(const UPhaseGramPlan& g, char* buf, size_t cap);
int describe_row_launch(const UStepDirectPlan& g, char* buf, size_t cap);

hipError_t launch_u_phase_gram(const ProblemView& p, const IterateView& it, int n_iter2, hipStream_t st);
bool u_phase_gram_supported(int S, int n_c, int n_u);
bool u_phase_mfma_supported(int S, int n_c, int n_u);
hipError_t launch_u_phase_mfma(const ProblemView& p, const IterateView& it, int n_iter2, hipStream_t st);
hipError_t launch_u_phase_mfma_impl(const ProblemView& p, const IterateView& it, int n_iter2, double* cm_out, hipStream_t st);
bool rowpass_fused_supported(int S, int n_c, int n_u);
int rowpass_fused_grid(int64_t N, int S);
int64_t rowpass_fused_slab_doubles(int64_t N, int S, int n_c, int n_u);
hipError_t launch_rowpass_fused(const ProblemView& p, const IterateView& it, int n_iter2, const UScratch& scratch,
                                int* grid_out, hipStream_t st);
hipError_t launch_finish_u_norm(const double* u2_partials, int n, SolverState* state, hipStream_t st);
hipError_t launch_u_step_direct(const ProblemView& p, const IterateView& it, double* u_next, int t, hipStream_t st);
bool u_step_direct_supported(int S, int n_c, int n_u);

hipError_t launch_alpha(AlphaKind kind, const AlphaView& a, int n_iter2, hipStream_t st);
hipError_t launch_set_lh(SolverState* state, hipStream_t st);
hipError_t launch_project_simplex(const double* X, double* out, int K, int S, double z,
                                  hipStream_t st);
hipError_t launch_scatter_known_block(const double* gb_known, double* gb, int n_c, int K, int S,
                                      hipStream_t st);
hipError_t launch_init_state(SolverState* state, const double* consts, const double* alpha,
                             int S, int n_c, int n_u, hipStream_t st);

int64_t u_phase_split_cm_doubles(int64_t N, int n_u);
hipError_t launch_u_phase_split(const ProblemView& p, const IterateView& it, int n_iter2, const UScratch& scratch,
                                hipStream_t st);

bool cm_i8_supported(unsigned v_align, int S, int n_c, int n_u, int ND, int SD);
struct CmI8Launch {
    int mt0 = 0, mt1 = 0;
    int c_tile = 0, c_store = 0;
    size_t lds = 0;
    int grid = 0;
    int64_t blocks_per_wave = 0;
};
struct CmI8Panel {
    int col0 = 0, Sp = 0;
    bool s4 = false;
    int ncgx = 2;
    int tpl = 0;
    int n_launch = 0;
    CmI8Launch first, last;
};
constexpr int kCmMaxPanels = 8;
struct CmI8Plan {
    bool supported = false;
    int64_t N = 0;
    int S = 0, n_c = 0, n_u = 0;
    int nkc = 0, nd = 1;
    int nmt = 0, n_ct = 0;
    int n_panels = 0;
    CmI8Panel panel[kCmMaxPanels];
};
CmI8Plan cm_i8_plan(int64_t N, int S, int n_c, int n_u, int ND);
CmI8Launch cm_i8_launch_of(const CmI8Plan& g, int panel, int li);
int describe_cm_i8_plan(const CmI8Plan& g, char* buf, size_t cap);
struct CmRan {
    char text[2048] = "";
};
hipError_t launch_cm_i8(const ProblemView& p, const IterateView& it, double* cm, hipStream_t st, CmRan* ran = nullptr);
hipError_t launch_u_phase_split_i8(const ProblemView& p, const IterateView& it, int n_iter2, const UScratch& scratch,
                                   hipStream_t st);

bool u_inner_bu_supported(unsigned v_align, int S, int SD, int n_u, int n_iter2);
int u_inner_bu_grid(int64_t N, int S);
hipError_t launch_u_phase_split_i8_bu(const ProblemView& p, const IterateView& it, int n_iter2, const UScratch& scratch,
                                      int* grid_out, hipStream_t st);

bool u_phase_big_supported(int S, int n_c, int n_u, int n_iter2);
hipError_t launch_u_phase_big(const ProblemView& p, const IterateView& it, int n_iter2, hipStream_t st);

hipError_t launch_gram_mfma(const ProblemView& p, const double* u, int n_u, GramJobTable jobs, int n_dense, double* slab,
                            int64_t slab_doubles, const int* done_flag, int* ny_out, hipStream_t st, GramRan* ran = nullptr);
int64_t gram_mfma_slab_doubles(int64_t N, int S, int n_jobs);

hipError_t launch_gather_counts_int(const unsigned short* src16, const unsigned short* src_x16, const long long* idx,
                                    int64_t n_idx, int SD, int ND, unsigned short* D16, unsigned short* X16, int64_t N16,
                                    signed char* Dt8, int64_t plane_stride, unsigned int* max_out,
                                    unsigned long long* xsum_out, hipStream_t st);
constexpr double kX16MaxDev = 8.0 * 0x1p-53;
hipError_t launch_build_counts_int(const double* D, const double* V, int64_t N, int S, int ND, unsigned short* D16,
                                   unsigned short* X16, int64_t N16, int SD, signed char* Dt8, int64_t plane_stride,
                                   unsigned long long* x_stats, hipStream_t st);
hipError_t launch_build_dt8(const unsigned short* D16, int64_t N, int SD, int ND, signed char* Dt8, int64_t plane_stride,
                            hipStream_t st);
hipError_t launch_mask_problem(const double* srcV, const double* srcD, const unsigned short* src16,
                               const unsigned short* srcX, const unsigned char* bits, double* dstV, double* dstD,
                               unsigned short* dst16, unsigned short* dstX, unsigned short* W16, int64_t N, int64_t N16, int S,
                               int SD, unsigned long long* stats, hipStream_t st);
hipError_t launch_holdout_weights_f64(const unsigned char* bits, double* W, int64_t N, int S, hipStream_t st);
constexpr int64_t kMaskDrawMaxS = ((int64_t)1 << 31) - 1, kMaskDrawMaxElements = (int64_t)1 << 60;
hipError_t launch_mask_draw(unsigned int* key_io, int pos, int64_t N, int64_t S, unsigned long long threshold,
                            unsigned char* bits, unsigned long long* result, hipStream_t st);
bool rowpass_v2_supported(int S, int n_c, int n_u, int n_iter2);
int rowpass_v2_grid(int64_t N, int S);
hipError_t launch_rowpass_v2(const ProblemView& p, const IterateView& it, int n_iter2, const UScratch& scratch, int* grid_out,
                             bool pair, bool* paired_out, hipStream_t st);
bool rowpass_v2_pair_fits(int S, int n_u, int n_iter2);
bool gram_i8_supported(int n_c, int n_u, int ND, int64_t N, int SD);
struct GramI8Plan {
    bool supported = false;
    int xl = 1, nd = 1, ring = 8;
    int nf = 0, launches = 0;
    int nsh = 0, ny = 0;
    int64_t rows_per_wg = 0;
    int blocks = 0, last = 0;
    int tail = 0;
    bool xcd = false;
};
GramI8Plan gram_i8_plan(int64_t N, int SD, int n_c, int n_u, int ND);
void describe_gram_i8_plan(const GramI8Plan& g, char* buf, size_t cap);
int64_t gram_i8_slab_words(int64_t N, int SD, int n_c, int n_u);
int64_t gram_i8_acc_words(int S, int n_c, int n_u);
bool gram_i8_known_supported(int n_c, int ND, int64_t N, int SD);
int64_t gram_i8_slab_words_nf(int64_t N, int SD, int nf);
int64_t gram_i8_acc_words_nf(int S, int nf, int n_bu);
hipError_t launch_gram_i8(const ProblemView& p, const double* u, int n_u, const short* feat_a, const short* feat_b, int NF,
                          long long* slab, int64_t slab_words, const int* done_flag, int* ny_out, hipStream_t st,
                          GramRan* ran = nullptr);
int bu_cols_grid(int64_t N);
hipError_t launch_bu_cols(const ProblemView& p, const double* u, int n_u, double* slab, const int* done_flag,
                          int* n_slabs_out, hipStream_t st, bool* with_vdv = nullptr);
hipError_t launch_gram_v2_reduce(const long long* slab_i8, int ny, int NF, int SD, const double* slab_bu, int n_bu_slabs,
                                 int n_u, int S, long long* acc_words, const int* dst_row, double* gb, const int* done_flag,
                                 const double* u2_partials, int n_u2, SolverState* state, hipStream_t st);

hipError_t launch_percentile_pair(const double* x, int64_t n, int64_t m, PercentilePlan p0, PercentilePlan p1,
                                  double* out0, double* out1, hipStream_t st);
int64_t percentile_max_replicates();

int wls_moments_grid(int64_t N);
int64_t wls_slab_doubles(int64_t N, int S, int K);
hipError_t launch_wls_moments(const ProblemView& p, const double* u, int n_u, int target_dv, double* slab, double* mom,
                              hipStream_t st);
hipError_t launch_nnls_intercept(const double* gb, const double* mom, int K, int S, double* out, int* status, hipStream_t st);

constexpr int kSvdMaxS = 512, kSvdMaxNc = 64, kSvdMaxRank = 64;
constexpr size_t kSvdMaxLds = 160 * 1024;
size_t svd_project_lds_bytes(int S, int rank);
struct SvdColumns {
    double sign[kSvdMaxRank], scale[kSvdMaxRank];
};
bool svd_supported(int S, int n_c, int rank);
int svd_gram_grid(int64_t N, int S);
int64_t svd_gram_slab_doubles(int64_t N, int S);
hipError_t launch_svd_gram(const ProblemView& p, const double* H1, double* slab, int* flags, double* C, hipStream_t st);
int64_t svd_project_slab_doubles(int64_t N, int rank);
hipError_t launch_svd_project(const ProblemView& p, const double* H1, const double* Es, int rank, double* T, double* slab,
                              double* norms, hipStream_t st);
hipError_t launch_svd_finish(double* T, int64_t N, int rank, const SvdColumns& cols, hipStream_t st);

struct MatchColumns {
    int src[kMaxK];
};
int match_gram_grid(int64_t N, int n_u);
int64_t match_gram_slab_doubles(int64_t N, int n_u);
hipError_t launch_match_gram(const double* u, const double* anchor, const long long* idx, int64_t N, int64_t n_anchor_rows,
                             int n_u, double* slab, int* flags, double* P, hipStream_t st);
hipError_t launch_copy_cols_permuted(const double* u, double* dst, int64_t N, int n_u, const MatchColumns& cols,
                                     hipStream_t st);

}
```

demethify_amd/csrc/dmf_kernels_alpha.hip:

```cpp
#include "dmf_device.h"
#include "dmf_dispatch.h"
#include "dmf_internal.h"

namespace dmf {

template <int KMAX>
__device__ __forceinline__ void sort_desc(double (&x)[KMAX]) {
#pragma unroll
    for (int k = 2; k <= KMAX; k <<= 1) {
#pragma unroll
        for (int j = k >> 1; j > 0; j >>= 1) {
#pragma unroll
            for (int i = 0; i < KMAX; ++i) {
                const int l = i ^ j;
                if (l > i) {
                    const double lo = fmin(x[i], x[l]), hi = fmax(x[i], x[l]);
                    if ((i & k) == 0) { x[i] = hi; x[l] = lo; }
                    else { x[i] = lo; x[l] = hi; }
                }
            }
        }
    }
}

// ... 647 lines not shown
        const int in_lds = lds <= 150 * 1024;
        if (in_lds && lds > 48 * 1024) {
            const hipError_t e = raise_dynamic_lds<k_alpha_phase<KMAX>>(lds);
            if (e != hipSuccess) return e;
        }
        hipLaunchKernelGGL(k_alpha_phase<KMAX>, dim3(nb), dim3(64), in_lds ? lds : 0, st, a.gb, a.alpha, a.alpha_prev, a.state,
                           a.S, K, a.n_u, n_iter2, in_lds, a.partials);
    } else {
        hipLaunchKernelGGL(k_alpha_phase_dyn, dim3(nb), dim3(64), 0, st, a.gb, a.alpha, a.alpha_prev, a.state, a.S, K, a.n_u,
                           n_iter2, a.partials);
    }
    return launch_finish_iteration(a.partials, nb, a.state, n_iter2, st);
}

template <int G>
static hipError_t launch_alpha_lanes(const AlphaView& a, int n_iter2, hipStream_t st) {
    const int nb = (a.S * G + 63) / 64;
    hipLaunchKernelGGL(k_alpha_phase_lanes<G>, dim3(nb), dim3(64), 0, st, a.gb, a.alpha, a.alpha_prev, a.state, a.S,
                       a.n_c + a.n_u, a.n_u, n_iter2, a.partials);
    return launch_finish_iteration(a.partials, nb, a.state, n_iter2, st);
}

hipError_t launch_alpha(AlphaKind kind, const AlphaView& a, int n_iter2, hipStream_t st) {
    const int S = a.S, K = a.n_c + a.n_u, nb4 = (S + 3) / 4, nb64 = (S + 63) / 64;
    if (K < 1 || K > kMaxK) return hipErrorInvalidValue;
    switch (kind) {
        case AlphaKind::PhaseRow16:
            if (K > 16) break;
            hipLaunchKernelGGL(k_alpha_phase_row16, dim3(nb4), dim3(64), 0, st, a.gb, a.alpha, a.alpha_prev, a.state, S, K, a.n_u,
                               n_iter2, a.partials);
            return hipGetLastError();
        case AlphaKind::PhaseLanes:
            if (K <= 16) break;
            return K <= 32 ? launch_alpha_lanes<32>(a, n_iter2, st) : launch_alpha_lanes<64>(a, n_iter2, st);
        case AlphaKind::Phase:
            if (K > 16) break;
            return dispatch_kmax(K, [&](auto kmax) { return launch_alpha_thread<kmax>(a, n_iter2, st); });
        case AlphaKind::PhaseDyn:
            if (K <= 16) break;
            return launch_alpha_thread<0>(a, n_iter2, st);
        case AlphaKind::FrankWolfeRow16:
            if (K > 16 || a.n_c < 1 || a.purity == nullptr) break;
            hipLaunchKernelGGL(k_alpha_frank_wolfe_row16, dim3(nb4), dim3(64), 0, st, a.gb, a.alpha, a.purity, a.state, S, K,
                               a.n_u, n_iter2, a.partials);
            return launch_finish_iteration(a.partials, nb4, a.state, n_iter2, st);
        case AlphaKind::FrankWolfe:
            if (a.purity == nullptr) break;
            hipLaunchKernelGGL(k_alpha_frank_wolfe, dim3(nb64), dim3(64), 0, st, a.gb, a.alpha, a.purity, a.state, S, K, a.n_u,
                               n_iter2, a.partials);
            return launch_finish_iteration(a.partials, nb64, a.state, n_iter2, st);
    }
    return hipErrorInvalidValue;
}

template <int KMAX>
__global__ __launch_bounds__(64) void k_project(const double* __restrict__ X, double* __restrict__ out,
                                                int K, int S, double z) {
    const int s = blockIdx.x * 64 + threadIdx.x;
    if (s >= S) return;
    double x[KMAX];
#pragma unroll
    for (int k = 0; k < KMAX; ++k) x[k] = k < K ? X[(int64_t)k * S + s] : 0.0;
    project_column<KMAX>(x, K, z);
#pragma unroll
    for (int k = 0; k < KMAX; ++k)
        if (k < K) out[(int64_t)k * S + s] = x[k];
}

hipError_t launch_project_simplex(const double* X, double* out, int K, int S, double z,
                                  hipStream_t st) {
    const dim3 grid((S + 63) / 64), block(64);
    if (K < 1 || K > kMaxK) return hipErrorInvalidValue;
    return dispatch_kmax(K, [&](auto kmax) {
        if constexpr (kmax > 0) hipLaunchKernelGGL(k_project<kmax>, grid, block, 0, st, X, out, K, S, z);
        else hipLaunchKernelGGL(k_project_dyn, grid, block, 0, st, X, out, K, S, z);
        return hipGetLastError();
    });
}

__global__ __launch_bounds__(256) void k_scatter_known(const double* __restrict__ gb_known,
                                                       double* __restrict__ gb, int n_c, int K, int S) {
    const int s = blockIdx.x * 256 + threadIdx.x;
    if (s >= S) return;
    for (int l = 0; l <= n_c; ++l) {
        const int ld = l == n_c ? K : l;
        for (int k = 0; k <= l; ++k) {
            const int kd = k == n_c ? K : k;
            gb[(int64_t)tri(kd, ld) * S + s] = gb_known[(int64_t)tri(k, l) * S + s];
        }
    }
}

hipError_t launch_scatter_known_block(const double* gb_known, double* gb, int n_c, int K, int S,
                                      hipStream_t st) {
    hipLaunchKernelGGL(k_scatter_known, dim3((S + 255) / 256), dim3(256), 0, st, gb_known, gb, n_c, K, S);
    return hipGetLastError();
}

__global__ __launch_bounds__(256) void k_init_state(SolverState* __restrict__ state,
                                                    const double* __restrict__ consts,
                                                    const double* __restrict__ alpha, int S, int n_c,
                                                    int n_u) {
    __shared__ double red[4];
    double acc = 0.0;
    const double* A2 = alpha + (int64_t)n_c * S;
    for (int i = threadIdx.x; i < n_u * S; i += 256) acc = fma(A2[i], A2[i], acc);
    const double n2 = block_sum<256>(acc, red);
    if (threadIdx.x == 0) {
        const double dsq = consts[0], rt2 = consts[1];
        state->a1 = 1.0;
        state->a2 = 1.0;
        state->dsq = dsq;
        state->rt_norm2 = rt2;
        state->l_w = n2 * dsq;
        state->l_w_prev = state->l_w;
        state->l_h = (rt2 + state->u_norm2) * dsq;
        state->l_h_prev = state->l_h;
        state->cf = __longlong_as_double(0x7FF8000000000000ll);
        state->cf_prev = state->cf;
        state->tol = 0.0;
        state->band = 1.0;
        state->mom = nullptr;
        state->mom_n = -1;
        state->iters = 0;
        state->done = 0;
        state->arrive = 0;
    }
}

hipError_t launch_init_state(SolverState* state, const double* consts, const double* alpha, int S,
                             int n_c, int n_u, hipStream_t st) {
    hipLaunchKernelGGL(k_init_state, dim3(1), dim3(256), 0, st, state, consts, alpha, S, n_c, n_u);
    return hipGetLastError();
}

}
```

demethify_amd/csrc/dmf_kernels_gram_i8.hip:

```cpp
#include <cstdint>
#include <cstdio>
#include <cstdlib>

#include "dmf_device.h"
#include "dmf_dispatch.h"
#include "dmf_internal.h"
#include "dmf_fixedpoint.h"

namespace dmf {

typedef int v4i __attribute__((ext_vector_type(4)));
typedef int v16i __attribute__((ext_vector_type(16)));
typedef unsigned int v4u __attribute__((ext_vector_type(4)));

namespace {
constexpr int kNSL = 7;
constexpr int kRing = 8;
constexpr int kMaxFeat = 576;
}

__global__ __launch_bounds__(256) void k_build_d16(const double* __restrict__ D, const double* __restrict__ V, int64_t N, int S,
                                                   unsigned short* __restrict__ D16, unsigned short* __restrict__ X16,
                                                   int64_t N16, int SD, unsigned long long* __restrict__ x_stats) {
    const int64_t chunks = N16 * (SD / 8);
    unsigned long long bad = 0, xsum = 0;
    double dev = 0.0;
    for (int64_t c = (int64_t)blockIdx.x * 256 + threadIdx.x; c < chunks; c += (int64_t)gridDim.x * 256) {
        const int64_t row = c / (SD / 8);
        const int col0 = (int)(c - row * (SD / 8)) * 8;
        unsigned int w[4], xw[4];
#pragma unroll
        for (int e = 0; e < 4; ++e) {
            unsigned int dh[2] = {0, 0}, xh[2] = {0, 0};
#pragma unroll
            for (int h = 0; h < 2; ++h) {
                const int col = col0 + 2 * e + h;
                if (row < N && col < S) {
                    const double d = D[row * S + col];
                    dh[h] = (unsigned int)d;
                    if (X16 != nullptr && d > 0.0) {
                        const double v = V[row * S + col];
                        const double x = rint(v * d);
                        const double err = fabs(fma(v, d, -x));
                        const double xm = fmax(x, 1.0);
                        if (x >= 0.0 && x <= d && err <= kX16MaxDev * xm) {
                            xh[h] = (unsigned int)x;
                            xsum += xh[h];
                            dev = fmax(dev, err / xm);
                        } else {
                            ++bad;
                        }
                    }
                }
            }
            w[e] = dh[0] | (dh[1] << 16);
            xw[e] = xh[0] | (xh[1] << 16);
        }
        *reinterpret_cast<v4u*>(D16 + row * SD + col0) = v4u{w[0], w[1], w[2], w[3]};
        if (X16 != nullptr) *reinterpret_cast<v4u*>(X16 + row * SD + col0) = v4u{xw[0], xw[1], xw[2], xw[3]};
    }
    if (X16 == nullptr) return;
#pragma unroll
    for (int off = 32; off > 0; off >>= 1) {
        bad += __shfl_xor(bad, off, 64);
        xsum += __shfl_xor(xsum, off, 64);
        dev = fmax(dev, __shfl_xor(dev, off, 64));
    }
    __shared__ unsigned long long wst[4][3];
    const int wave = threadIdx.x >> 6;
    if ((threadIdx.x & 63) == 0) {
        wst[wave][0] = bad;
        wst[wave][1] = (unsigned long long)__double_as_longlong(dev);
        wst[wave][2] = xsum;
    }
    __syncthreads();
    if (threadIdx.x == 0) {
        unsigned long long b = 0, m = 0, x = 0;
        for (int w = 0; w < 4; ++w) {
            b += wst[w][0];
            m = m > wst[w][1] ? m : wst[w][1];
            x += wst[w][2];
        }
        if (b > 0) atomicAdd(x_stats, b);
        if (m > 0) atomicMax(x_stats + 1, m);
        if (x > 0) atomicAdd(x_stats + 2, x);
    }
}

__global__ __launch_bounds__(256) void k_build_dt8(const unsigned short* __restrict__ D16, int64_t N, int SD, int ND,
                                                   signed char* __restrict__ Dt8, int64_t plane_stride, int64_t n_tiles) {
    const int lane = threadIdx.x & 63;
    const int n = lane & 31, h = lane >> 5;
    const int SB = SD / 32;
    for (int64_t tile = (int64_t)blockIdx.x * 4 + (threadIdx.x >> 6); tile < n_tiles; tile += (int64_t)gridDim.x * 4) {
        const int64_t rb = tile / SB;
        const int sb = (int)(tile - rb * SB);
        unsigned int p0[4] = {0, 0, 0, 0}, p1[4] = {0, 0, 0, 0};
#pragma unroll
        for (int j = 0; j < 16; ++j) {
            const int64_t row = rb * 32 + 16 * h + j;
            unsigned int d = row < N ? D16[row * SD + sb * 32 + n] : 0u;
            unsigned int b0 = d, b1 = 0;
            if (ND == 2) {
                d += 128u;
                b0 = (d & 0xFFu) ^ 0x80u;
                b1 = d >> 8;
            }
            p0[j >> 2] |= (b0 & 0xFFu) << (8 * (j & 3));
            p1[j >> 2] |= (b1 & 0xFFu) << (8 * (j & 3));
        }
        signed char* __restrict__ dst = Dt8 + tile * 1024 + n * 32 + h * 16;
        *reinterpret_cast<v4u*>(dst) = v4u{p0[0], p0[1], p0[2], p0[3]};
        if (ND == 2) *reinterpret_cast<v4u*>(dst + plane_stride) = v4u{p1[0], p1[1], p1[2], p1[3]};
    }
}

hipError_t launch_build_counts_int(const double* D, const double* V, int64_t N, int S, int ND, unsigned short* D16,
                                   unsigned short* X16, int64_t N16, int SD, signed char* Dt8, int64_t plane_stride,
                                   unsigned long long* x_stats, hipStream_t st) {
    const int64_t chunks = N16 * (SD / 8);
    int64_t g = (chunks + 255) / 256;
    if (g > 8192) g = 8192;
    if (g < 1) g = 1;
    if (X16 != nullptr) {
        if (V == nullptr || x_stats == nullptr) return hipErrorInvalidValue;
        const hipError_t e = hipMemsetAsync(x_stats, 0, 3 * sizeof(unsigned long long), st);
        if (e != hipSuccess) return e;
    }
    hipLaunchKernelGGL(k_build_d16, dim3((unsigned)g), dim3(256), 0, st, D, V, N, S, D16, X16, N16, SD, x_stats);
    if (Dt8 != nullptr) {
        const int64_t n_tiles = ((N + 31) / 32) * (SD / 32);
        int64_t gt = (n_tiles + 3) / 4;
        if (gt > 16384) gt = 16384;
        hipLaunchKernelGGL(k_build_dt8, dim3((unsigned)gt), dim3(256), 0, st, D16, N, SD, ND, Dt8, plane_stride, n_tiles);
    }
    return hipGetLastError();
}

hipError_t launch_build_dt8(const unsigned short* D16, int64_t N, int SD, int ND, signed char* Dt8, int64_t plane_stride,
                            hipStream_t st) {
    const int64_t n_tiles = ((N + 31) / 32) * (SD / 32);
    int64_t gt = (n_tiles + 3) / 4;
    if (gt > 16384) gt = 16384;
    hipLaunchKernelGGL(k_build_dt8, dim3((unsigned)gt), dim3(256), 0, st, D16, N, SD, ND, Dt8, plane_stride, n_tiles);
    return hipGetLastError();
}

__global__ __launch_bounds__(256) void k_gather_rows_u16(const unsigned short* __restrict__ src, unsigned short* __restrict__ dst,
                                                         const unsigned short* __restrict__ src_x, unsigned short* __restrict__ dst_x,
                                                         const long long* __restrict__ idx, int64_t n_idx, int64_t N16, int SD,
                                                         unsigned int* __restrict__ max_out, unsigned long long* __restrict__ xsum_out) {
    const int wave = threadIdx.x >> 6, lane = threadIdx.x & 63;
    unsigned int mx = 0u;
    unsigned long long xs = 0;
    for (int64_t r = (int64_t)blockIdx.x * 4 + wave; r < N16; r += (int64_t)gridDim.x * 4) {
        const int64_t r_src = r < n_idx ? idx[r] : -1;
        const unsigned short* __restrict__ s = r_src >= 0 ? src + r_src * SD : nullptr;
        for (int c = lane * 8; c < SD; c += 512) {
            v4u w = v4u{0u, 0u, 0u, 0u};
            if (s != nullptr) w = *reinterpret_cast<const v4u*>(s + c);
            *reinterpret_cast<v4u*>(dst + r * SD + c) = w;
#pragma unroll
            for (int e = 0; e < 4; ++e) {
                const unsigned int lo = w[e] & 0xFFFFu, hi = w[e] >> 16;
                mx = mx > lo ? mx : lo;
                mx = mx > hi ? mx : hi;
            }
            if (dst_x != nullptr) {
                v4u x = v4u{0u, 0u, 0u, 0u};
                if (s != nullptr) x = *reinterpret_cast<const v4u*>(src_x + r_src * SD + c);
                *reinterpret_cast<v4u*>(dst_x + r * SD + c) = x;
#pragma unroll
                for (int e = 0; e < 4; ++e) xs += (x[e] & 0xFFFFu) + (x[e] >> 16);
            }
        }
    }
#pragma unroll
    for (int off = 32; off > 0; off >>= 1) {
        const unsigned int o = (unsigned int)__shfl_xor((int)mx, off, 64);
        mx = mx > o ? mx : o;
        xs += __shfl_xor(xs, off, 64);
    }
    __shared__ unsigned int wmax[4];
    __shared__ unsigned long long wsum[4];
    if (lane == 0) wmax[wave] = mx, wsum[wave] = xs;
    __syncthreads();
    if (threadIdx.x == 0) {
        unsigned int m = wmax[0];
        unsigned long long x = wsum[0];
        for (int w = 1; w < 4; ++w) m = m > wmax[w] ? m : wmax[w], x += wsum[w];
        if (m > 0u) atomicMax(max_out, m);
        if (dst_x != nullptr && x > 0) atomicAdd(xsum_out, x);
    }
}

hipError_t launch_gather_counts_int(const unsigned short* src16, const unsigned short* src_x16, const long long* idx,
                                    int64_t n_idx, int SD, int ND, unsigned short* D16, unsigned short* X16, int64_t N16,
                                    signed char* Dt8, int64_t plane_stride, unsigned int* max_out,
                                    unsigned long long* xsum_out, hipStream_t st) {
    int64_t g = (N16 + 3) / 4;
    if (g > 2048) g = 2048;
    if (g < 1) g = 1;
    if ((src_x16 == nullptr) != (X16 == nullptr) || (X16 != nullptr && xsum_out == nullptr)) return hipErrorInvalidValue;
    hipError_t e = hipMemsetAsync(max_out, 0, sizeof(unsigned int), st);
    if (e == hipSuccess && X16 != nullptr) e = hipMemsetAsync(xsum_out, 0, sizeof(unsigned long long), st);
    if (e != hipSuccess) return e;
    hipLaunchKernelGGL(k_gather_rows_u16, dim3((unsigned)g), dim3(256), 0, st, src16, D16, src_x16, X16, idx, n_idx, N16, SD,
                       max_out, xsum_out);
    if (Dt8 != nullptr) {
// ... 655 lines not shown
```

demethify_amd/csrc/dmf_kernels_stream.hip:

```cpp
#include <cstdio>

#include "dmf_device.h"
#include "dmf_dispatch.h"
#include "dmf_internal.h"

namespace dmf {

__global__ __launch_bounds__(256) void k_convert_counts(const long long* __restrict__ src,
                                                        double* __restrict__ dst, int64_t n) {
    int64_t i = (int64_t)blockIdx.x * 256 + threadIdx.x;
    const int64_t stride = (int64_t)gridDim.x * 256;
    for (; i < n; i += stride) dst[i] = (double)src[i];
}

hipError_t launch_convert_counts(const long long* src, double* dst, int64_t n, hipStream_t st) {
    if (n <= 0) return hipSuccess;
    int blocks = (int)((n + 255) / 256 < 8192 ? (n + 255) / 256 : 8192);
    hipLaunchKernelGGL(k_convert_counts, dim3(blocks), dim3(256), 0, st, src, dst, n);
    return hipGetLastError();
}

template <int MODE>
__global__ __launch_bounds__(256) void k_reduce_partial(const double* __restrict__ x, int64_t n,
                                                        double* __restrict__ partial,
                                                        const int* __restrict__ done_flag) {
    __shared__ double red[4];
    if (done_flag != nullptr && *done_flag) return;
    double acc = MODE == 1 ? 0.0 : -INFINITY;
    int64_t i = (int64_t)blockIdx.x * 256 + threadIdx.x;
    const int64_t stride = (int64_t)gridDim.x * 256;
    for (; i < n; i += stride) {
        const double v = x[i];
        if (MODE == 1) acc = fma(v, v, acc);
        else if (MODE == 0) acc = fmax(acc, v);
        else if (MODE == 2) acc = fmax(acc, fabs(v - (double)(float)v));
        else if (MODE == 3) acc = fmax(acc, (v >= 0.0 && v == rint(v)) ? v : INFINITY);
        else acc = fmax(acc, (v >= 0.0 && v <= 1.0) ? 0.0 : 1.0);
    }
    const double tot = MODE == 1 ? block_sum<256>(acc, red) : block_max<256>(acc, red);
    if (threadIdx.x == 0) partial[blockIdx.x] = tot;
}

template <int MODE>
__global__ __launch_bounds__(256) void k_reduce_final(const double* __restrict__ partial, int n,
                                                      double* __restrict__ out,
                                                      const int* __restrict__ done_flag) {
    __shared__ double red[4];
    if (done_flag != nullptr && *done_flag) return;
    double acc = MODE == 1 ? 0.0 : -INFINITY;
    for (int i = threadIdx.x; i < n; i += 256) {
        if (MODE == 1) acc += partial[i];
        else acc = fmax(acc, partial[i]);
    }
    const double tot = MODE == 1 ? block_sum<256>(acc, red) : block_max<256>(acc, red);
    if (threadIdx.x == 0) *out = tot;
}

static inline int reduce_blocks(int64_t n) {
    int64_t b = (n + 255) / 256;
    if (b > 1024) b = 1024;
    if (b < 1) b = 1;
    return (int)b;
}

hipError_t launch_max_f64(const double* x, int64_t n, double* scratch, double* out, hipStream_t st) {
    const int nb = reduce_blocks(n);
    hipLaunchKernelGGL(k_reduce_partial<0>, dim3(nb), dim3(256), 0, st, x, n, scratch, (const int*)nullptr);
    hipLaunchKernelGGL(k_reduce_final<0>, dim3(1), dim3(256), 0, st, scratch, nb, out, (const int*)nullptr);
    return hipGetLastError();
}

hipError_t launch_f32_residual_max(const double* x, int64_t n, double* scratch, double* out, hipStream_t st) {
    const int nb = reduce_blocks(n);
    hipLaunchKernelGGL(k_reduce_partial<2>, dim3(nb), dim3(256), 0, st, x, n, scratch, (const int*)nullptr);
    hipLaunchKernelGGL(k_reduce_final<0>, dim3(1), dim3(256), 0, st, scratch, nb, out, (const int*)nullptr);
    return hipGetLastError();
}

hipError_t launch_int_count_max(const double* x, int64_t n, double* scratch, double* out, hipStream_t st) {
    const int nb = reduce_blocks(n);
    hipLaunchKernelGGL(k_reduce_partial<3>, dim3(nb), dim3(256), 0, st, x, n, scratch, (const int*)nullptr);
    hipLaunchKernelGGL(k_reduce_final<0>, dim3(1), dim3(256), 0, st, scratch, nb, out, (const int*)nullptr);
    return hipGetLastError();
}

hipError_t launch_unit_range_check(const double* x, int64_t n, double* scratch, double* out, hipStream_t st) {
    const int nb = reduce_blocks(n);
    hipLaunchKernelGGL(k_reduce_partial<4>, dim3(nb), dim3(256), 0, st, x, n, scratch, (const int*)nullptr);
    hipLaunchKernelGGL(k_reduce_final<0>, dim3(1), dim3(256), 0, st, scratch, nb, out, (const int*)nullptr);
    return hipGetLastError();
}

hipError_t launch_sumsq_f64(const double* x, int64_t n, double* scratch, double* out,
                            const int* done_flag, hipStream_t st) {
    const int nb = reduce_blocks(n);
    hipLaunchKernelGGL(k_reduce_partial<1>, dim3(nb), dim3(256), 0, st, x, n, scratch, done_flag);
    hipLaunchKernelGGL(k_reduce_final<1>, dim3(1), dim3(256), 0, st, scratch, nb, out, done_flag);
    return hipGetLastError();
}

__global__ __launch_bounds__(256) void k_gather_rows(const double* __restrict__ src,
                                                     double* __restrict__ dst,
                                                     const long long* __restrict__ idx,
                                                     int64_t n_idx, int64_t width) {
    const int wave = threadIdx.x >> 6, lane = threadIdx.x & 63;
    int64_t r = (int64_t)blockIdx.x * 4 + wave;
    const int64_t stride = (int64_t)gridDim.x * 4;
    for (; r < n_idx; r += stride) {
        const double* s = src + idx[r] * width;
        double* d = dst + r * width;
        for (int64_t c = lane; c < width; c += 64) d[c] = s[c];
    }
}

hipError_t launch_gather_rows(const double* src, double* dst, const long long* idx, int64_t n_idx,
                              int64_t width, hipStream_t st) {
    if (n_idx <= 0 || width <= 0) return hipSuccess;
    int64_t b = (n_idx + 3) / 4;
    if (b > 65536) b = 65536;
    hipLaunchKernelGGL(k_gather_rows, dim3((unsigned)b), dim3(256), 0, st, src, dst, idx, n_idx, width);
    return hipGetLastError();
}

__global__ __launch_bounds__(256) void k_index_range_check(const long long* __restrict__ idx, int64_t n_idx, int64_t n_src,
                                                           unsigned int* __restrict__ flag) {
    bool bad = false;
    for (int64_t r = (int64_t)blockIdx.x * 256 + threadIdx.x; r < n_idx; r += (int64_t)gridDim.x * 256) {
        const long long v = idx[r];
        bad = bad || v < 0 || v >= n_src;
    }
    if (__ballot(bad) != 0ull && (threadIdx.x & 63) == 0) atomicOr(flag, 1u);
}

hipError_t launch_index_range_check(const long long* idx, int64_t n_idx, int64_t n_src, unsigned int* flag, hipStream_t st) {
    hipError_t e = hipMemsetAsync(flag, 0, sizeof(unsigned int), st);
    if (e != hipSuccess) return e;
    int64_t b = (n_idx + 255) / 256;
    if (b > 1024) b = 1024;
    hipLaunchKernelGGL(k_index_range_check, dim3((unsigned)(b < 1 ? 1 : b)), dim3(256), 0, st, idx, n_idx, n_src, flag);
    return hipGetLastError();
}

__global__ __launch_bounds__(256) void k_pad_rows(const double* __restrict__ src, double* __restrict__ dst,
                                                  int64_t n_rows, int width_src, int width_dst) {
    int64_t e = (int64_t)blockIdx.x * 256 + threadIdx.x;
    const int64_t total = n_rows * width_dst, stride = (int64_t)gridDim.x * 256;
    for (; e < total; e += stride) {
        const int64_t r = e / width_dst;
        const int c = (int)(e - r * width_dst);
        dst[e] = c < width_src ? src[r * width_src + c] : 0.0;
    }
}

hipError_t launch_pad_rows(const double* src, double* dst, int64_t n_rows, int width_src, int width_dst,
                           hipStream_t st) {
    if (n_rows <= 0 || width_dst <= 0) return hipSuccess;
    int64_t b = (n_rows * width_dst + 255) / 256;
    if (b > 8192) b = 8192;
    hipLaunchKernelGGL(k_pad_rows, dim3((unsigned)b), dim3(256), 0, st, src, dst, n_rows, width_src, width_dst);
    return hipGetLastError();
}

__global__ __launch_bounds__(256) void k_cost(const double* __restrict__ V, const double* __restrict__ D,
                                              const double* __restrict__ Rt, const double* __restrict__ u,
                                              const double* __restrict__ alpha, int64_t N, int S,
                                              int n_c, int n_u, int alpha_in_lds,
                                              double* __restrict__ partial) {
    extern __shared__ double lds_dyn[];
    __shared__ double red[4];
    const int K = n_c + n_u;
    const double* A = alpha;
    if (alpha_in_lds) {
        for (int i = threadIdx.x; i < K * S; i += 256) lds_dyn[i] = alpha[i];
        __syncthreads();
        A = lds_dyn;
    }
    const int tpr = S < 256 ? S : 256;
    const int rows_per_tile = 256 / tpr;
    const int r = threadIdx.x / tpr, c = threadIdx.x - r * tpr;
    double acc = 0.0;
    if (r < rows_per_tile) {
        const int64_t stride = (int64_t)gridDim.x * rows_per_tile;
        for (int64_t i0 = (int64_t)blockIdx.x * rows_per_tile + r; i0 < N; i0 += 4 * stride) {
// ... 6 lines not shown
                row[x] = i < N ? i : N - 1;
            }
            for (int s = c; s < S; s += tpr) {
                double v[4], d[4], pred[4];
#pragma unroll
                for (int x = 0; x < 4; ++x) {
                    v[x] = V[row[x] * S + s];
                    d[x] = D[row[x] * S + s];
                    pred[x] = 0.0;
                }
                for (int k = 0; k < n_c; ++k) {
                    const double ak = A[k * S + s];
#pragma unroll
                    for (int x = 0; x < 4; ++x) pred[x] = fma(Rt[row[x] * n_c + k], ak, pred[x]);
                }
                for (int j = 0; j < n_u; ++j) {
                    const double aj = A[(n_c + j) * S + s];
#pragma unroll
                    for (int x = 0; x < 4; ++x) pred[x] = fma(u[row[x] * n_u + j], aj, pred[x]);
                }
#pragma unroll
                for (int x = 0; x < 4; ++x) {
                    const double e = v[x] - pred[x];
                    acc = fma(w[x] * d[x] * e, e, acc);
                }
            }
        }
    }
    const double tot = block_sum<256>(acc, red);
    if (threadIdx.x == 0) partial[blockIdx.x] = tot;
}

template <int NKC, int NU, bool D16>
__global__ __launch_bounds__(256) void k_cost_cols(const double* __restrict__ V, const void* __restrict__ Dv, int SD,
                                                   const double* __restrict__ Rtp, const double* __restrict__ u,
                                                   const double* __restrict__ alpha, int64_t N, int S, int n_c,
                                                   double* __restrict__ partial) {
    constexpr int NCT = 4 * NKC;
    constexpr int kRows = 8;
    __shared__ double red[4];
    const int wave = __builtin_amdgcn_readfirstlane(threadIdx.x >> 6), lane = threadIdx.x & 63;
    const int s = blockIdx.y * 64 + lane;
    const bool active = s < S;
    const int sc = active ? s : S - 1;
    double ak[NCT > 0 ? NCT : 1], aj[NU > 0 ? NU : 1];
#pragma unroll
    for (int k = 0; k < NCT; ++k) ak[k] = k < n_c ? alpha[(int64_t)k * S + sc] : 0.0;
#pragma unroll
    for (int j = 0; j < NU; ++j) aj[j] = alpha[(int64_t)(n_c + j) * S + sc];
    const double* __restrict__ Df = reinterpret_cast<const double*>(Dv);
    const unsigned short* __restrict__ Dh = reinterpret_cast<const unsigned short*>(Dv);
    double acc = 0.0;
    const int64_t stride = (int64_t)gridDim.x * 4;
    for (int64_t i0 = (int64_t)blockIdx.x * 4 + wave; i0 < N; i0 += kRows * stride) {
        double v[kRows], d[kRows];
        int64_t row[kRows];
#pragma unroll
        for (int x = 0; x < kRows; ++x) {
            const int64_t i = i0 + x * stride;
            row[x] = i < N ? i : N - 1;
            v[x] = V[row[x] * S + sc];
            if constexpr (D16) d[x] = (double)Dh[row[x] * SD + sc];
            else d[x] = Df[row[x] * S + sc];
            if (i >= N) d[x] = 0.0;
        }
#pragma unroll
        for (int x = 0; x < kRows; ++x) {
            const double* __restrict__ rt_row = Rtp + row[x] * NCT;
            const double* __restrict__ u_row = u + row[x] * NU;
            double pred = 0.0;
#pragma unroll
            for (int k = 0; k < NCT; ++k) pred = fma(rt_row[k], ak[k], pred);
#pragma unroll
            for (int j = 0; j < NU; ++j) pred = fma(u_row[j], aj[j], pred);
            const double e = v[x] - pred;
            acc = fma(d[x] * e, e, acc);
        }
    }
    if (!active) acc = 0.0;
    const double tot = block_sum<256>(acc, red);
    if (threadIdx.x == 0) partial[blockIdx.y * gridDim.x + blockIdx.x] = tot;
}

template <int NKC, int NU, bool ODD>
__global__ __launch_bounds__(256) void k_cost_cols2(const double* __restrict__ V, const unsigned short* __restrict__ Dh, int SD,
                                                    const double* __restrict__ Rtp, const double* __restrict__ u,
                                                    const double* __restrict__ alpha, int64_t N, int S, int n_c,
                                                    double* __restrict__ partial) {
    typedef double v2d __attribute__((ext_vector_type(2)));
    constexpr int NCT = 4 * NKC;
    constexpr int kRows = 8;
    __shared__ double red[4];
    const int wave = __builtin_amdgcn_readfirstlane(threadIdx.x >> 6), lane = threadIdx.x & 63;
    const int s = blockIdx.y * 128 + 2 * lane;
    const bool active = s < S;
    const bool lone = ODD && s == S - 1;
    const int sc = lone ? S - 2 : (active ? s : 0);
    const int sd = active ? s : 0;
    typedef double v2d_u __attribute__((ext_vector_type(2), aligned(8)));
    double ak[NCT > 0 ? NCT : 1][2], aj[NU > 0 ? NU : 1][2];
#pragma unroll
    for (int k = 0; k < NCT; ++k) {
#pragma unroll
        for (int h = 0; h < 2; ++h) ak[k][h] = k < n_c ? alpha[(int64_t)k * S + sc + h] : 0.0;
        if (lone) ak[k][0] = ak[k][1];
    }
#pragma unroll
    for (int j = 0; j < NU; ++j) {
#pragma unroll
        for (int h = 0; h < 2; ++h) aj[j][h] = alpha[(int64_t)(n_c + j) * S + sc + h];
        if (lone) aj[j][0] = aj[j][1];
    }
    double acc0 = 0.0, acc1 = 0.0;
    const int64_t stride = (int64_t)gridDim.x * 4;
    for (int64_t i0 = (int64_t)blockIdx.x * 4 + wave; i0 < N; i0 += kRows * stride) {
        v2d v[kRows];
        unsigned int dd[kRows];
        int64_t row[kRows];
#pragma unroll
        for (int x = 0; x < kRows; ++x) {
            const int64_t i = i0 + x * stride;
            row[x] = i < N ? i : N - 1;
            const v2d_u vl = *reinterpret_cast<const v2d_u*>(V + row[x] * S + sc);
            v[x] = v2d{lone ? vl.y : vl.x, vl.y};
            dd[x] = *reinterpret_cast<const unsigned int*>(Dh + row[x] * SD + sd);
            if (i >= N) dd[x] = 0u;
        }
#pragma unroll
        for (int x = 0; x < kRows; ++x) {
            const double* __restrict__ rt_row = Rtp + row[x] * NCT;
            const double* __restrict__ u_row = u + row[x] * NU;
            double p0 = 0.0, p1 = 0.0;
#pragma unroll
            for (int k = 0; k < NCT; ++k) {
                const double r = rt_row[k];
                p0 = fma(r, ak[k][0], p0);
                p1 = fma(r, ak[k][1], p1);
            }
#pragma unroll
            for (int j = 0; j < NU; ++j) {
                const double r = u_row[j];
                p0 = fma(r, aj[j][0], p0);
                p1 = fma(r, aj[j][1], p1);
            }
            const double e0 = v[x].x - p0, e1 = v[x].y - p1;
            acc0 = fma((double)(dd[x] & 0xFFFFu) * e0, e0, acc0);
            acc1 = fma((double)(dd[x] >> 16) * e1, e1, acc1);
        }
    }
    double acc = acc0 + acc1;
    if (!active) acc = 0.0;
    const double tot = block_sum<256>(acc, red);
    if (threadIdx.x == 0) partial[blockIdx.y * gridDim.x + blockIdx.x] = tot;
}

template <bool D16>
__global__ __launch_bounds__(256) void k_vdv_cols(const double* __restrict__ V, const void* __restrict__ Dv, int SD, int64_t N,
                                                  int S, double* __restrict__ slab) {
    constexpr int kRows = 8;
    __shared__ double red[3][64];
    const int wave = __builtin_amdgcn_readfirstlane(threadIdx.x >> 6), lane = threadIdx.x & 63;
    const int s = blockIdx.y * 64 + lane;
    const bool active = s < S;
    const int sc = active ? s : S - 1;
    const double* __restrict__ Df = reinterpret_cast<const double*>(Dv);
    const unsigned short* __restrict__ Dh = reinterpret_cast<const unsigned short*>(Dv);
    double acc = 0.0;
    const int64_t stride = (int64_t)gridDim.x * 4;
    for (int64_t i0 = (int64_t)blockIdx.x * 4 + wave; i0 < N; i0 += kRows * stride) {
        double v[kRows], d[kRows];
#pragma unroll
        for (int x = 0; x < kRows; ++x) {
            const int64_t i = i0 + x * stride;
            const int64_t row = i < N ? i : N - 1;
            v[x] = V[row * S + sc];
            if constexpr (D16) d[x] = (double)Dh[row * SD + sc];
            else d[x] = Df[row * S + sc];
            if (i >= N) d[x] = 0.0;
        }
#pragma unroll
        for (int x = 0; x < kRows; ++x) acc = fma(d[x] * v[x], v[x], acc);
    }
    if (wave > 0) red[wave - 1][lane] = acc;
    __syncthreads();
    if (wave == 0 && active) slab[(int64_t)blockIdx.x * S + s] = ((acc + red[0][lane]) + red[1][lane]) + red[2][lane];
}

__global__ __launch_bounds__(64) void k_vdv_finish(const double* __restrict__ slab, int nb, int S, double* __restrict__ out) {
    const int s = blockIdx.x * 64 + threadIdx.x;
    if (s >= S) return;
    double acc = 0.0;
    for (int b = 0; b < nb; b += 8) {
        double v[8];
#pragma unroll
        for (int q = 0; q < 8; ++q) v[q] = slab[(int64_t)(b + q < nb ? b + q : b) * S + s];
#pragma unroll
        for (int q = 0; q < 8; ++q)
            if (b + q < nb) acc += v[q];
    }
    out[s] = acc;
}

int vdv_cols_grid(int64_t N) {
    int64_t want = (N + 4 * 8 - 1) / (4 * 8);
    if (want > 256) want = 256;
    return (int)(want < 1 ? 1 : want);
}

hipError_t launch_vdv_cols(const ProblemView& p, double* slab, double* out, hipStream_t st) {
    const int S = p.S, nbx = vdv_cols_grid(p.N);
    const dim3 grid(nbx, (S + 63) / 64);
    if (p.D16 != nullptr) hipLaunchKernelGGL((k_vdv_cols<true>), grid, dim3(256), 0, st, p.V, (const void*)p.D16, p.SD, p.N, S, slab);
    else hipLaunchKernelGGL((k_vdv_cols<false>), grid, dim3(256), 0, st, p.V, (const void*)p.D, S, p.N, S, slab);
    hipLaunchKernelGGL(k_vdv_finish, dim3((S + 63) / 64), dim3(64), 0, st, slab, nbx, S, out);
    return hipGetLastError();
}

CostPlan cost_plan(const CostKey& k) {
    CostPlan plan;
    const int S = k.S, K = k.n_c + k.n_u;
    const bool rtp_ok = k.n_c == 0 || k.rtp_present;
    const bool pair_ok = k.d16 && k.SD % 2 == 0 && (k.v_align & 7) == 0 && (S + 127) / 128 <= kCostPartials;
    plan.nkc = (k.n_c + 3) / 4;
    plan.nu = k.n_u;
    plan.odd = (S & 1) != 0;
    if ((k.level == 0 || k.level == 3 || k.level == 4) && rtp_ok && k.n_c <= 16 && k.n_u >= 0 && k.n_u <= 4 && K >= 1) {
        if (pair_ok && S >= 128) {
            plan.kind = CostKind::Cols2;
            plan.d16 = true;
            return plan;
        }
        if ((S + 63) / 64 <= kCostPartials) {
            plan.kind = CostKind::Cols;
            plan.d16 = k.d16;
            plan.odd = false;
            return plan;
        }
    } else if (k.level == 0 && rtp_ok && k.n_c <= 16 && k.n_u >= 5 && k.n_u <= 16 && pair_ok && S >= 32) {
        plan.kind = CostKind::Cols2Wide;
        plan.d16 = true;
        return plan;
    }
    plan = CostPlan{};
    plan.alpha_in_lds = (size_t)K * S * sizeof(double) <= 48 * 1024;
    return plan;
}

int describe_cost_plan(const CostPlan& plan, char* buf, size_t cap) {
    switch (plan.kind) {
        case CostKind::Cols:
            return snprintf(buf, cap, "cost=k_cost_cols<%d,%d,%s>", plan.nkc, plan.nu, plan.d16 ? "u16" : "f64");
        case CostKind::Cols2:
        case CostKind::Cols2Wide:
            return snprintf(buf, cap, "cost=k_cost_cols2<%d,%d,%s>", plan.nkc, plan.nu, plan.odd ? "odd" : "even");
        default: return snprintf(buf, cap, "cost=k_cost alpha=%s", plan.alpha_in_lds ? "lds" : "global");
    }
}

static int cost_cols_row_blocks(int64_t N, int ny) {
    const int64_t want = (N + 4 * 8 - 1) / (4 * 8);
    int nbx = (int)(want < 1 ? 1 : want);
    if (nbx > kCostPartials / ny) nbx = kCostPartials / ny;
    return nbx;
}

template <int NKC, int NU>
static hipError_t launch_cost_cols2_t(bool odd, const ProblemView& p, const double* u, const double* alpha, double* scratch,
                                      double* out, hipStream_t st) {
    const int S = p.S, ny2 = (S + 127) / 128;
    const int nbx = cost_cols_row_blocks(p.N, ny2);
    if (odd)
        hipLaunchKernelGGL((k_cost_cols2<NKC, NU, true>), dim3(nbx, ny2), dim3(256), 0, st, p.V, p.D16, p.SD, p.Rtp, u, alpha,
                           p.N, S, p.n_c, scratch);
    else
        hipLaunchKernelGGL((k_cost_cols2<NKC, NU, false>), dim3(nbx, ny2), dim3(256), 0, st, p.V, p.D16, p.SD, p.Rtp, u, alpha,
                           p.N, S, p.n_c, scratch);
    hipLaunchKernelGGL(k_reduce_final<1>, dim3(1), dim3(256), 0, st, scratch, nbx * ny2, out, (const int*)nullptr);
    return hipGetLastError();
}

template <int NKC, int NU>
static hipError_t launch_cost_cols_t(bool d16, const ProblemView& p, const double* u, const double* alpha, double* scratch,
                                     double* out, hipStream_t st) {
    const int S = p.S, ny = (S + 63) / 64;
    const int nbx = cost_cols_row_blocks(p.N, ny);
    if (d16)
        hipLaunchKernelGGL((k_cost_cols<NKC, NU, true>), dim3(nbx, ny), dim3(256), 0, st, p.V, (const void*)p.D16, p.SD, p.Rtp, u,
                           alpha, p.N, S, p.n_c, scratch);
    else
        hipLaunchKernelGGL((k_cost_cols<NKC, NU, false>), dim3(nbx, ny), dim3(256), 0, st, p.V, (const void*)p.D, S, p.Rtp, u,
                           alpha, p.N, S, p.n_c, scratch);
    hipLaunchKernelGGL(k_reduce_final<1>, dim3(1), dim3(256), 0, st, scratch, nbx * ny, out, (const int*)nullptr);
    return hipGetLastError();
}

static hipError_t launch_cost(bool in_lds, const ProblemView& p, const double* u, const double* alpha, int n_u, double* scratch,
                              double* out, hipStream_t st) {
    const int S = p.S, K = p.n_c + n_u;
    const int tpr = S < 256 ? S : 256;
    const int rows_per_tile = 256 / tpr;
    int64_t tiles = (p.N + rows_per_tile - 1) / rows_per_tile;
    const int nb = (int)(tiles < kCostPartials ? (tiles < 1 ? 1 : tiles) : kCostPartials);
    const size_t lds = (size_t)K * S * sizeof(double);
    hipLaunchKernelGGL(k_cost, dim3(nb), dim3(256), in_lds ? lds : 0, st, p.V, p.D, p.Rt, u, alpha, p.N, S, p.n_c, n_u,
                       in_lds ? 1 : 0, scratch);
    hipLaunchKernelGGL(k_reduce_final<1>, dim3(1), dim3(256), 0, st, scratch, nb, out,
                       (const int*)nullptr);
    return hipGetLastError();
}

hipError_t launch_cost_plan(const CostPlan& plan, const ProblemView& p, const double* u, const double* alpha, int n_u,
                            double* scratch, double* out, hipStream_t st) {
    if (plan.kind != CostKind::Generic &&
        (plan.nkc != (p.n_c + 3) / 4 || plan.nu != n_u || (plan.d16 && p.D16 == nullptr) || (!plan.d16 && p.D == nullptr) ||
         (p.n_c > 0 && p.Rtp == nullptr)))
        return hipErrorInvalidValue;
    if (plan.kind == CostKind::Generic && p.D == nullptr) return hipErrorInvalidValue;
    switch (plan.kind) {
        case CostKind::Cols:
        case CostKind::Cols2:
            return dispatch_int<0, 4>(plan.nkc, [&](auto nkc) {
                return dispatch_int<0, 4>(plan.nu, [&](auto nu) {
                    constexpr int NKC = decltype(nkc)::value, NU = decltype(nu)::value;
                    if (plan.kind == CostKind::Cols2)
                        return launch_cost_cols2_t<NKC, NU>(plan.odd, p, u, alpha, scratch, out, st);
                    return launch_cost_cols_t<NKC, NU>(plan.d16, p, u, alpha, scratch, out, st);
                });
            });
        case CostKind::Cols2Wide:
            return dispatch_int<0, 4>(plan.nkc, [&](auto nkc) {
                return dispatch_int<5, 16>(plan.nu, [&](auto nu) {
                    return launch_cost_cols2_t<decltype(nkc)::value, decltype(nu)::value>(plan.odd, p, u, alpha, scratch, out,
                                                                                         st);
                });
            });
        default: return launch_cost(plan.alpha_in_lds, p, u, alpha, n_u, scratch, out, st);
    }
}

static void gram_geometry(int64_t N, int S, int n_jobs, int* nsx, int* nz, int* ny,
                          int64_t* rows_per_chunk) {
    *nsx = (S + 63) / 64;
    *nz = (n_jobs + kGramChunk - 1) / kGramChunk;
    int64_t want = 4096 / ((int64_t)(*nsx) * (*nz));
    if (want < 1) want = 1;
    int64_t rpc = (N + want - 1) / want;
    if (rpc < 256) rpc = 256;
    *rows_per_chunk = rpc;
    *ny = (int)((N + rpc - 1) / rpc);
    if (*ny < 1) *ny = 1;
}

int64_t gram_slab_doubles(int64_t N, int S, int n_jobs) {
    int nsx, nz, ny;
    int64_t rpc;
    gram_geometry(N, S, n_jobs, &nsx, &nz, &ny, &rpc);
    return (int64_t)ny * n_jobs * S;
}

__device__ __forceinline__ double ext_row_value(const double* __restrict__ Rt,
                                                const double* __restrict__ u, int64_t i, int n_c,
                                                int n_u, int k, double v) {
    if (k < n_c) return Rt[i * n_c + k];
    if (k < n_c + n_u) return u[i * n_u + (k - n_c)];
    return v;
}

__global__ __launch_bounds__(256) void k_gram(const double* __restrict__ V, const double* __restrict__ D,
                                              const double* __restrict__ Rt, const double* __restrict__ u,
                                              int64_t N, int S, int n_c, int n_u,
                                              const short* __restrict__ k_idx,
                                              const short* __restrict__ l_idx, int n_jobs,
                                              int64_t rows_per_chunk, double* __restrict__ slab,
                                              const int* __restrict__ done_flag) {
    __shared__ double red[3][kGramChunk][64];
    if (done_flag != nullptr && *done_flag) return;
    const int wave = __builtin_amdgcn_readfirstlane(threadIdx.x >> 6);
    const int lane = threadIdx.x & 63;
    const int s = blockIdx.x * 64 + lane;
    const bool active = s < S;
    const int a0 = blockIdx.z * kGramChunk;
    int kk[kGramChunk], ll[kGramChunk];
#pragma unroll
    for (int p = 0; p < kGramChunk; ++p) {
        const int a = a0 + p < n_jobs ? a0 + p : n_jobs - 1;
        kk[p] = k_idx[a];
        ll[p] = l_idx[a];
    }
    double acc[kGramChunk];
#pragma unroll
    for (int p = 0; p < kGramChunk; ++p) acc[p] = 0.0;
    const int64_t r0 = (int64_t)blockIdx.y * rows_per_chunk;
    const int64_t r1 = r0 + rows_per_chunk < N ? r0 + rows_per_chunk : N;
    for (int64_t i = r0 + wave; i < r1; i += 4) {
        const double d = active ? D[i * S + s] : 0.0;
        const double v = active ? V[i * S + s] : 0.0;
#pragma unroll
        for (int p = 0; p < kGramChunk; ++p) {
            const double xk = ext_row_value(Rt, u, i, n_c, n_u, kk[p], v);
            const double xl = ext_row_value(Rt, u, i, n_c, n_u, ll[p], v);
            acc[p] = fma(d * xk, xl, acc[p]);
        }
    }
    if (wave > 0) {
#pragma unroll
        for (int p = 0; p < kGramChunk; ++p) red[wave - 1][p][lane] = acc[p];
    }
    __syncthreads();
    if (wave == 0 && active) {
#pragma unroll
        for (int p = 0; p < kGramChunk; ++p) {
            if (a0 + p < n_jobs) {
                const double tot = ((acc[p] + red[0][p][lane]) + red[1][p][lane]) + red[2][p][lane];
                slab[((int64_t)blockIdx.y * n_jobs + (a0 + p)) * S + s] = tot;
            }
        }
// ... 61 lines not shown
```

demethify_amd/csrc/dmf_select.h:

```cpp
#pragma once
#include <cstddef>
#include <cstdint>

namespace dmf {

constexpr int kSplitInnerSteps = 50;
constexpr int kCmI8MinNu = 5;
constexpr int kSplitMinNu = 7;
constexpr int kGramI8MinFp64Acc = 48;
constexpr int kGramI8MinPairsNoKnown = 33;

struct ShapeKey {
    int64_t N = 0;
    int S = 0, n_c = 0, n_u = 0;
    int nd = 0;
    int SD = 0;
    bool x16 = false;
    bool rowpass_pair = true;
    int level = 0;
    bool d_f32_exact = false;
    bool rtp_present = true;
    unsigned v_align = 0;
    unsigned rtp_align = 0;
    bool alpha_unit = true;
};

struct PathSpec {
    int u_path = 2;
    bool use_gram_spec = false, use_gram_mfma = false, use_u_big = false;
    bool use_v2 = false, use_cm_i8 = false, use_gram_i8 = false, use_fused = false;
    bool supported = true;
};

enum class RowKind {
    RowpassV2,
    CmI8InnerBu,
    CmI8InnerRows,
    RowpassFused,
    UPhaseBig,
    UPhaseMfmaSplit,
    UPhaseMfma,
    UPhaseGram,
    UStepDirect
};
enum class GramKind { InRowPass, I8, BuColsI8, GramU, GramMfma, Gram };
enum class AlphaKind { FrankWolfeRow16, FrankWolfe, PhaseRow16, PhaseLanes, Phase, PhaseDyn };

struct IterationPlan {
    RowKind row = RowKind::UStepDirect;
    GramKind gram = GramKind::Gram;
    AlphaKind alpha = AlphaKind::PhaseDyn;
};

PathSpec select_path(const ShapeKey& k);
IterationPlan plan_iteration(const ShapeKey& k, const PathSpec& s, int n_iter2, bool purity);
int describe_plan(const ShapeKey& k, const IterationPlan& plan, char* buf, size_t cap);
PathSpec standalone_spec(PathSpec s);
int describe_u_phase(const ShapeKey& k, const PathSpec& s, int n_iter2, bool purity, bool standalone, char* buf, size_t cap);

struct CostKey {
    int S = 0, n_c = 0, n_u = 0;
    bool d16 = false;
    int SD = 0;
    unsigned v_align = 0;
    bool rtp_present = true;
    int level = 0;
};
enum class CostKind {
    Cols,
    Cols2,
    Cols2Wide,
    Generic
};
struct CostPlan {
    CostKind kind = CostKind::Generic;
    int nkc = 0, nu = 0;
    bool d16 = false;
    bool odd = false;
    bool alpha_in_lds = false;
};
constexpr int kCostPartials = 1024;
CostPlan cost_plan(const CostKey& k);
int describe_cost_plan(const CostPlan& plan, char* buf, size_t cap);

}
```

demethify_amd/device.py:

```python
from __future__ import annotations

import ctypes as C
import os

import numpy as np

from . import _lib as L

_contexts: dict[int, "Context"] = {}


def _is_torch(x) -> bool:
    return type(x).__module__.startswith("torch")


def _host_f64(x, name):
    a = np.ascontiguousarray(x, dtype=np.float64)
    if not np.all(np.isfinite(a)):
        raise ValueError(f"{name} holds non-finite values (use --fillna)")
    return a


def _ptr(a):
    if a is None:
        return None
    if _is_torch(a) or hasattr(a, "data_ptr"):
        return C.c_void_p(a.data_ptr())
    return a.ctypes.data_as(C.c_void_p)


def pack_mask(mask) -> np.ndarray:
    m = np.asarray(mask)
    if m.ndim != 2:
        raise ValueError(f"a mask is N x S, got shape {m.shape}")
    return np.packbits(m.astype(bool, copy=False), axis=1, bitorder="little")


def mask_threshold(fraction) -> int:
    import math

    f = float(fraction)
    if not f > 0.0:
        return 0
    if f >= 1.0:
        return 1 << 53
    return math.ceil(f * 9007199254740992.0)


class Context:

    def __init__(self, device: int = 0, stream: int | None = None):
        self._lib = L.load()
        h = C.c_void_p()
        L.check(self._lib.dmf_context_create(int(device), C.c_void_p(stream) if stream else None, C.byref(h)),
                "dmf_context_create")
        self._h = h
        self.device = int(device)
        self.generic_level = 0

    def close(self):
        if getattr(self, "_h", None):
            self._lib.dmf_context_destroy(self._h)
            self._h = None

    def __del__(self):
        try:
            self.close()
        except Exception:
            pass

    def synchronize(self):
        L.check(self._lib.dmf_context_synchronize(self._h), "dmf_context_synchronize")

    def set_profiling(self, enabled, families=None):
        mode = int(bool(enabled))
        if mode and families is not None:
            mode = sum(1 << (1 + int(f)) for f in families)
        L.check(self._lib.dmf_context_set_profiling(self._h, mode), "dmf_context_set_profiling")

    def set_generic(self, level: int):
        L.check(self._lib.dmf_context_set_generic(self._h, int(level)), "dmf_context_set_generic")
        self.generic_level = int(level)

    def set_x16(self, enabled: bool):
        L.check(self._lib.dmf_context_set_x16(self._h, int(bool(enabled))), "dmf_context_set_x16")

    def set_rowpass_pair(self, enabled: bool):
        L.check(self._lib.dmf_context_set_rowpass_pair(self._h, int(bool(enabled))), "dmf_context_set_rowpass_pair")

    def set_stop_confirmation(self, mode: int):
        L.check(self._lib.dmf_context_set_stop_confirmation(self._h, int(mode)), "dmf_context_set_stop_confirmation")

    def reset_kernel_time(self):
        L.check(self._lib.dmf_context_reset_kernel_time(self._h), "dmf_context_reset_kernel_time")

    def kernel_time(self, family: int):
        ms, n = C.c_double(), C.c_int64()
        L.check(self._lib.dmf_context_kernel_time(self._h, int(family), C.byref(ms), C.byref(n)),
                "dmf_context_kernel_time")
        return ms.value, n.value

    def project_simplex(self, X, z=1.0):
        X = np.ascontiguousarray(X, dtype=np.float64)
        out = np.empty_like(X)
        K, S = X.shape
        L.check(self._lib.dmf_project_simplex(self._h, _ptr(X), K, S, float(z), 0, _ptr(out)),
                "dmf_project_simplex")
        return out

    def percentile_axis0(self, x, q):
        qs = np.ascontiguousarray(np.atleast_1d(q), dtype=np.float64)
        if _is_torch(x) and x.is_cuda:
            import torch

            if x.dtype != torch.float64:
                raise TypeError("percentile_axis0 takes float64 data")
            x = x.contiguous()
            n, tail = x.shape[0], tuple(x.shape[1:])
            m = int(np.prod(tail, dtype=np.int64))
            out = torch.empty((len(qs),) + tail, dtype=torch.float64, device=x.device)
            torch.cuda.current_stream(x.device).synchronize()
            L.check(self._lib.dmf_percentile_axis0(self._h, _ptr(x), n, m, _ptr(qs), len(qs), L.DMF_PTR_DEVICE,
                                                   _ptr(out)), "dmf_percentile_axis0")
            return out
        if _is_torch(x):
            x = x.numpy()
        x = np.ascontiguousarray(x, dtype=np.float64)
        n, tail = x.shape[0], tuple(x.shape[1:])
        m = int(np.prod(tail, dtype=np.int64))
        out = np.empty((len(qs),) + tail, dtype=np.float64)
        L.check(self._lib.dmf_percentile_axis0(self._h, _ptr(x), n, m, _ptr(qs), len(qs), 0, _ptr(out)),
                "dmf_percentile_axis0")
        return out


def get_context(device: int | None = None) -> Context:
    if device is None:
        device = int(os.environ.get("DEMETHIFY_DEVICE", os.environ.get("LOCAL_RANK", "0")))
    ctx = _contexts.get(device)
    if ctx is None:
        ctx = _contexts[device] = Context(device)
    return ctx


def _route(route) -> int:
    try:
        return {"solver": L.DMF_ROUTE_SOLVER, "update_u": L.DMF_ROUTE_UPDATE_U}[route]
    except KeyError:
        raise ValueError(f'route must be "solver" or "update_u", got {route!r}') from None


def u_phase_describe(N, S, n_c, n_u, nd=0, level=0, n_iter2=20, flags=0, route="solver"):
    buf = C.create_string_buffer(2048)
    st = L.load().dmf_u_phase_describe(int(N), int(S), int(n_c), int(n_u), int(nd), int(level), int(n_iter2), int(flags),
                                       _route(route), buf, len(buf))
    if st == L.DMF_ERR_UNSUPPORTED:
        return None
    L.check(st, "dmf_u_phase_describe")
    return buf.value.decode()


class Problem:

    def __init__(self, ctx: Context, V, counts, Rt=None):
        self.ctx = ctx
        self._lib = ctx._lib
        flags = 0
        if _is_torch(V):
# ... 50 lines not shown
        if getattr(idx, "is_cuda", False):
            n = int(np.prod(idx.shape))
            L.check(self._lib.dmf_problem_gather_device(self.ctx._h, self._h, C.c_void_p(idx.data_ptr()), n, C.byref(h)),
                    "dmf_problem_gather_device")
            return Problem._from_handle(self.ctx, h, n, self.S, self.n_c)
        idx = np.ascontiguousarray(idx, dtype=np.int64)
        L.check(self._lib.dmf_problem_gather(self.ctx._h, self._h, _ptr(idx), idx.size, C.byref(h)),
                "dmf_problem_gather")
        return Problem._from_handle(self.ctx, h, int(idx.size), self.S, self.n_c)

    def masked(self, train_mask) -> "Problem":
        nb = (self.S + 7) // 8
        flags = 0
        if getattr(train_mask, "is_cuda", False):
            if _is_torch(train_mask):
                import torch

                ok = (train_mask.dtype == torch.uint8 and train_mask.is_contiguous()
                      and tuple(train_mask.shape) == (self.N, nb) and train_mask.device.index == self.ctx.device)
                if ok:
                    torch.cuda.current_stream(train_mask.device).synchronize()
            else:
                ok = getattr(train_mask, "packed_mask", None) == (self.N, nb) and train_mask.ctx is self.ctx
            if not ok:
                raise ValueError(f"a device mask must be the packed bits: contiguous uint8, shape {(self.N, nb)}, on the "
                                 "context's GPU")
            bits, flags = train_mask, L.DMF_PTR_DEVICE
        else:
            m = np.asarray(train_mask)
            if m.dtype == np.bool_:
                if m.shape != (self.N, self.S):
                    raise ValueError(f"mask shape {m.shape} != problem shape {(self.N, self.S)}")
                bits = pack_mask(m)
            elif m.dtype == np.uint8:
                if m.shape != (self.N, nb):
                    raise ValueError(f"packed mask shape {m.shape} != {(self.N, nb)} (ceil(S / 8) bytes per row)")
                bits = np.ascontiguousarray(m)
            else:
                raise TypeError("train_mask must be a bool N x S array or packed uint8 bits")
        h = C.c_void_p()
        L.check(self._lib.dmf_problem_mask(self.ctx._h, self._h, _ptr(bits), flags, C.byref(h)), "dmf_problem_mask")
        out = Problem._from_handle(self.ctx, h, self.N, self.S, self.n_c)
        out._keep = (self,)
        return out

    def close(self):
        if getattr(self, "_h", None):
            if getattr(self.ctx, "_h", None):
                self._lib.dmf_problem_destroy(self._h)
            self._h = None
            self._keep = ()

    def __del__(self):
        try:
            self.close()
        except Exception:
            pass

    def __enter__(self):
        return self

    def __exit__(self, *exc):
        self.close()

    def cost(self, u, alpha) -> float:
        alpha = np.ascontiguousarray(alpha, dtype=np.float64)
        n_u = 0
        if u is not None:
            u = np.ascontiguousarray(u, dtype=np.float64).reshape(self.N, -1)
            n_u = u.shape[1]
        if alpha.shape != (self.n_c + n_u, self.S):
            raise ValueError(f"alpha shape {alpha.shape} != {(self.n_c + n_u, self.S)}")
        out = C.c_double()
        L.check(self._lib.dmf_cost(self.ctx._h, self._h, _ptr(u) if n_u else None, n_u, _ptr(alpha), 0,
                                   C.byref(out)), "dmf_cost")
        return out.value

    def cost_describe(self, n_u: int) -> str:
        buf = C.create_string_buffer(128)
        L.check(self._lib.dmf_problem_cost_describe(self.ctx._h, self._h, int(n_u), buf, len(buf)),
                "dmf_problem_cost_describe")
        return buf.value.decode()

    def gram_known(self):
        out = np.empty(((self.n_c + 1) * (self.n_c + 2) // 2, self.S), dtype=np.float64)
        buf = C.create_string_buffer(256)
        L.check(self._lib.dmf_problem_gram_known(self._h, _ptr(out), buf, len(buf)), "dmf_problem_gram_known")
        return out, buf.value.decode()

    def report(self) -> dict:
        ints = (C.c_int64 * len(L.REPORT_INTS))()
        dbls = (C.c_double * len(L.REPORT_DBLS))()
        L.check(self._lib.dmf_problem_report(self._h, ints, dbls), "dmf_problem_report")
        out = {k: int(v) for k, v in zip(L.REPORT_INTS, ints)}
        out.update({k: float(v) for k, v in zip(L.REPORT_DBLS, dbls)})
        return out

    def copy_out(self, name: str, report: dict | None = None) -> np.ndarray:
        r = self.report() if report is None else report
        shape, dtype = {
            "V": ((r["N"], r["S"]), np.float64), "D": ((r["N"], r["S"]), np.float64),
            "Rt": ((r["N"], r["n_c"]), np.float64), "Rtp": ((r["N"], r["rtp_width"]), np.float64),
            "D16": ((r["N16"], r["SD"]), np.uint16), "X16": ((r["N16"], r["SD"]), np.uint16),
            "W16": ((r["N16"], r["SD"]), np.uint16),
            "Dt8": ((r["ND"], (r["N"] + 31) // 32, r["SD"] // 32, 32, 32), np.int8),
            "mask_bits": ((r["N"], (r["S"] + 7) // 8), np.uint8), "consts": ((6,), np.float64),
        }[name]
        out = np.empty(shape, dtype=dtype)
        L.check(self._lib.dmf_problem_copy_out(self._h, L.PROBLEM_ARRAYS[name], _ptr(out), out.nbytes),
                "dmf_problem_copy_out")
        return out

    def wls_intercept(self, u=None, target="v", host_arrays=None, f64_arrays=False):
        try:
            tg = {"v": L.DMF_WLS_TARGET_V, "dv": L.DMF_WLS_TARGET_DV}[target]
        except KeyError:
            raise ValueError(f'target must be "v" or "dv", got {target!r}') from None
        flags, n_u = 0, 0
        if u is not None:
            if getattr(u, "is_cuda", False):
                from .staging import DeviceArray

                if isinstance(u, DeviceArray):
                    ok = u.ctx is self.ctx
                else:
                    ok = (_is_torch(u) and u.is_contiguous() and u.element_size() == 8 and u.is_floating_point()
                          and u.device.index == self.ctx.device)
                    if ok:
                        import torch

                        torch.cuda.current_stream(u.device).synchronize()
                if not ok:
                    raise ValueError("a device u must be a float64 staging.DeviceArray / contiguous CUDA tensor on the "
                                     "context's GPU")
                u = u.reshape(self.N, -1)
                flags = L.DMF_PTR_DEVICE
            else:
                u = _host_f64(u, "u").reshape(self.N, -1)
            n_u = int(u.shape[1])
        if f64_arrays:
            flags |= L.DMF_WLS_F64_ARRAYS
        K = self.n_c + n_u
        out = np.zeros((K, self.S), dtype=np.float64)
        status = np.full(self.S, -1, dtype=np.intc)
        L.check(self._lib.dmf_wls_intercept(self.ctx._h, self._h, _ptr(u) if n_u else None, n_u, tg, flags, _ptr(out),
                                            status.ctypes.data_as(C.POINTER(C.c_int))), "dmf_wls_intercept")
        self.wls_status = status
        if (status == 2).any():
            raise ZeroDivisionError("Weights sum to zero, can't be normalized")
        redo = np.flatnonzero(status != 0)
        if redo.size:
            if host_arrays is None:
                raise RuntimeError(f"wls_intercept: the device did not solve samples {redo.tolist()} (rank-deficient "
                                   "profiles or iteration cap) and no host_arrays were given to solve them on the host")
            from .init_func import wls_intercept as host_wls

            meth_f, counts, R_full = host_arrays() if callable(host_arrays) else host_arrays
            for k in redo:
                x = counts[:, k:k + 1] * meth_f[:, k:k + 1] if target == "dv" else meth_f[:, k:k + 1]
                out[:, k:k + 1] = host_wls(x, counts[:, k:k + 1], R_full)
        return out

    def svd_gram(self, H1=None):
        if self.n_c:
            H1 = _host_f64(H1, "H1")
            if H1.shape != (self.n_c, self.S):
# ... 319 lines not shown
```

include/demethify_hip.h:

```cpp
#ifndef DEMETHIFY_HIP_H
#define DEMETHIFY_HIP_H

#include <stddef.h>
#include <stdint.h>

#ifdef __cplusplus
extern "C" {
#endif

typedef enum dmf_status {
    DMF_OK = 0,
    DMF_ERR_BAD_ARG = 1,
    DMF_ERR_BAD_SHAPE = 2,
    DMF_ERR_HIP = 3,
    DMF_ERR_NONFINITE = 4,
    DMF_ERR_UNSUPPORTED = 5,
    DMF_ERR_NO_DEVICE = 6
} dmf_status;

enum {
    DMF_PTR_DEVICE = 1,
    DMF_COUNTS_F64 = 2,
    DMF_INIT_IN_UNIT_RANGE = 4
};

enum {
    DMF_SELECT_COUNTS_F32_EXACT = 1,
    DMF_SELECT_PURITY = 2,
    DMF_SELECT_ALPHA_OUTSIDE_UNIT = 4,
    DMF_SELECT_V_UNALIGNED = 8,
    DMF_SELECT_X16 = 16
};

enum {
    DMF_MODE_PARTIAL = 0,
    DMF_MODE_UNSUPERVISED = 1
};

enum {
    DMF_KERNEL_ROWPASS = 0,
    DMF_KERNEL_GRAM = 1,
    DMF_KERNEL_ALPHA = 2,
    DMF_KERNEL_COST = 3,
    DMF_KERNEL_FAMILIES = 4
};

typedef struct dmf_context dmf_context;
typedef struct dmf_problem dmf_problem;
typedef struct dmf_solver dmf_solver;

const char* dmf_status_string(int status);
const char* dmf_last_error(void);
int dmf_abi_version(void);

int dmf_context_create(int device, void* stream, dmf_context** out);
int dmf_context_destroy(dmf_context* ctx);
int dmf_context_synchronize(dmf_context* ctx);
int dmf_context_set_profiling(dmf_context* ctx, int enabled);
int dmf_context_kernel_time(dmf_context* ctx, int family, double* total_ms, int64_t* launches);
int dmf_context_reset_kernel_time(dmf_context* ctx);
int dmf_context_set_generic(dmf_context* ctx, int level);
int dmf_context_set_x16(dmf_context* ctx, int enabled);
int dmf_context_set_rowpass_pair(dmf_context* ctx, int enabled);
int dmf_context_set_stop_confirmation(dmf_context* ctx, int mode);

int dmf_problem_create(dmf_context* ctx, int64_t N, int64_t S, int64_t n_c,
                       const double* V, const void* counts, const double* Rt,
                       int flags, dmf_problem** out);
int dmf_problem_gather(dmf_context* ctx, const dmf_problem* src, const int64_t* idx,
                       int64_t n_idx, dmf_problem** out);
int dmf_problem_gather_device(dmf_context* ctx, const dmf_problem* src, const int64_t* idx_dev,
                              int64_t n_idx, dmf_problem** out);
int dmf_problem_mask(dmf_context* ctx, const dmf_problem* src, const uint8_t* train_bits, int flags, dmf_problem** out);
int dmf_problem_destroy(dmf_problem* p);
int dmf_problem_shape(const dmf_problem* p, int64_t* N, int64_t* S, int64_t* n_c);
int dmf_problem_gram_known(const dmf_problem* p, double* out, char* out_text, int64_t cap);
enum { DMF_REPORT_INTS = 16, DMF_REPORT_DBLS = 8 };
int dmf_problem_report(const dmf_problem* p, int64_t* out_ints, double* out_dbls);
enum {
    DMF_ARRAY_V = 0, DMF_ARRAY_D = 1, DMF_ARRAY_RT = 2, DMF_ARRAY_RTP = 3, DMF_ARRAY_D16 = 4, DMF_ARRAY_X16 = 5,
    DMF_ARRAY_W16 = 6, DMF_ARRAY_DT8 = 7, DMF_ARRAY_MASK_BITS = 8, DMF_ARRAY_CONSTS = 9
};
int dmf_problem_copy_out(const dmf_problem* p, int which, void* out, int64_t bytes);

int dmf_cost(dmf_context* ctx, const dmf_problem* p, const double* u, int64_t n_u,
             const double* alpha, int flags, double* out_cost);
int dmf_cost_describe(int64_t S, int64_t n_c, int64_t n_u, int has_u16, int64_t SD, int v_align, int rtp_present, int level,
                      char* buf, int64_t cap);
int dmf_problem_cost_describe(dmf_context* ctx, const dmf_problem* p, int64_t n_u, char* buf, int64_t cap);
int dmf_gram_i8_describe(int64_t N, int64_t S, int64_t n_c, int64_t n_u, int nd, char* buf, int64_t cap);
int dmf_project_simplex(dmf_context* ctx, const double* X, int64_t K, int64_t S, double z,
                        int flags, double* out);
int dmf_update_u(dmf_context* ctx, const dmf_problem* p, const double* u, const double* u_prev,
                 const double* alpha, int64_t n_u, int64_t n_iter2, int mode, int flags,
                 double* scalars_io, double* out_u, double* out_u_prev);
int dmf_update_alpha(dmf_context* ctx, const dmf_problem* p, const double* u, int64_t n_u,
                     const double* alpha, const double* alpha_prev, int64_t n_iter2, int flags,
                     double* scalars_io, double* out_alpha, double* out_alpha_prev);

enum { DMF_WLS_TARGET_V = 0, DMF_WLS_TARGET_DV = 1 };
enum { DMF_WLS_F64_ARRAYS = 8 };
int dmf_wls_intercept(dmf_context* ctx, const dmf_problem* p, const double* u, int64_t n_u, int target,
                      int flags, double* out_alpha, int* out_status);

int dmf_svd_gram(dmf_context* ctx, const dmf_problem* p, const double* H1, int flags, double* out_C, int64_t* out_flags);
int dmf_svd_factor(dmf_context* ctx, const dmf_problem* p, const double* H1, const double* E_over_sigma, int64_t rank,
                   int flags, double* out_norms, void** out_T);
int dmf_svd_finish(dmf_context* ctx, void* T, int64_t N, int64_t rank, const double* sign, const double* scale, int flags,
                   double* out_u);

int dmf_percentile_axis0(dmf_context* ctx, const double* x, int64_t n, int64_t m, const double* q,
                         int64_t n_q, int flags, double* out);

int dmf_solver_create(dmf_context* ctx, const dmf_problem* p, const double* u0,
                      const double* alpha0, int64_t n_u, int mode, int flags, dmf_solver** out);
int dmf_solver_set_purity(dmf_solver* s, const double* purity, int flags);
int dmf_solver_step(dmf_solver* s, int64_t n_outer, int64_t n_iter2, double tol,
                    int64_t* iters_done_total, int* converged);
int dmf_solver_get(dmf_solver* s, int flags, double* out_u, double* out_alpha,
                   double* out_cost, int64_t* out_iters);
int dmf_solver_match_components(dmf_solver* s, const void* anchor_dev, int64_t n_anchor_rows, const int64_t* idx_dev,
                                double* out_P);
int dmf_solver_get_u_permuted(dmf_solver* s, const int32_t* src_col, void* dst_dev);
int dmf_solver_cost(dmf_solver* s, double* out_cost);
int dmf_solver_cost_begin(dmf_solver* s);
int dmf_solver_cost_end(dmf_solver* s, double* out_cost);
int dmf_solver_holdout_error(dmf_solver* s, const dmf_problem* full, double* sum_sq, int64_t* n_test);
enum { DMF_GRAM_INTEGER = 0, DMF_GRAM_FP64 = 1, DMF_GRAM_LAST = 2 };
int dmf_solver_gram(dmf_solver* s, int kind, double* out_gb, char* out_text, int64_t cap);
int dmf_solver_row_moments(dmf_solver* s, double* out_cm, char* out_text, int64_t cap);
enum { DMF_MOMENTUM_SCALARS = 16 };
int dmf_solver_momentum_state(const dmf_solver* s, double* scalars, double* alpha_prev, double* u_prev);
int dmf_solver_destroy(dmf_solver* s);
int dmf_solver_describe(const dmf_solver* s, int64_t n_iter2, char* buf, int64_t cap);
int dmf_select_describe(int64_t N, int64_t S, int64_t n_c, int64_t n_u, int nd, int level, int64_t n_iter2, int flags,
                        char* buf, int64_t cap);
enum { DMF_ROUTE_SOLVER = 0, DMF_ROUTE_UPDATE_U = 1 };
int dmf_u_phase_describe(int64_t N, int64_t S, int64_t n_c, int64_t n_u, int nd, int level, int64_t n_iter2, int flags, int route,
                         char* buf, int64_t cap);
int dmf_solver_u_phase_describe(const dmf_solver* s, int64_t n_iter2, int route, char* buf, int64_t cap);
int dmf_solver_stop_info(const dmf_solver* s, int* confirm_stops, int64_t* n_confirmed, int64_t* n_unconfirmed,
                         double* last_stream_cost);
int dmf_solver_rowpass_launches(const dmf_solver* s, int64_t* total, int64_t* paired);
int dmf_solve(dmf_context* ctx, const dmf_problem* p, const double* u0, const double* alpha0,
              int64_t n_u, int mode, int64_t n_iter1, int64_t n_iter2, double tol, int flags,
              double* out_u, double* out_alpha, double* out_cost, int64_t* out_iters);

int dmf_table_scan(const char* path, char sep, int64_t* n_rows, int* col_percent_modified, int* col_valid_coverage,
                   int* n_cols);
int dmf_table_read(const char* path, char sep, int col_percent_modified, int col_valid_coverage, int64_t n_rows,
                   double* out_freq, int64_t stride_freq, double divide_by, int64_t* out_cov, int64_t stride_cov,
                   int n_threads);
void* dmf_host_alloc(size_t bytes, int* pinned);
void dmf_host_free(void* p, int pinned);

int dmf_write_interval_csv(const char* path, const char* header_line, const double* lower, const double* upper,
                           int64_t n_rows, int n_cols, int numpy_scalar_repr, int n_threads);

int dmf_stage_upload(dmf_context* ctx, const void* host, size_t bytes, void** out_dev);
int dmf_stage_free(dmf_context* ctx, void* dev);
int dmf_stage_download(dmf_context* ctx, const void* dev, size_t bytes, void* host);

int dmf_mask_draw(dmf_context* ctx, uint32_t key[624], int* pos, int64_t N, int64_t S,
                  uint64_t threshold, void** out_bits, int64_t* n_kept);

#ifdef __cplusplus
}
#endif
#endif
```

Before: 1779 outer iters/s.

## Compute cost from 16-bit counts with reciprocal table and trim solver setup syncs

Adds an x16 variant of the Cols2 cost kernel. It reads 16-bit methylated counts and reconstructs V = X/D through an LDS reciprocal table plus an FMA-corrected quotient, which is checked for exactness when the counts are built, instead of streaming the f64 V matrix. It also fuses the u_prev copy with the u sum-of-squares reduction at solver init, folds the tolerance-setting kernel into the momentum upload, and skips the initial host state fetch when tol is zero. The cost pass and launch overhead shrink, in exchange for more code paths and an exactness precondition on the counts.

Result: no change. 1786 outer iters/s, median of 6 (+0.4%).

```diff
diff --git a/demethify_amd/_lib.py b/demethify_amd/_lib.py
--- a/demethify_amd/_lib.py
+++ b/demethify_amd/_lib.py
@@ -52,6 +52,7 @@
     "dmf_context_reset_kernel_time": (C.c_int, [_p]),
     "dmf_context_set_generic": (C.c_int, [_p, C.c_int]),
     "dmf_context_set_x16": (C.c_int, [_p, C.c_int]),
+    "dmf_context_set_cost_x16": (C.c_int, [_p, C.c_int]),
     "dmf_context_set_rowpass_pair": (C.c_int, [_p, C.c_int]),
     "dmf_context_set_stop_confirmation": (C.c_int, [_p, C.c_int]),
     "dmf_problem_create": (C.c_int, [_p, _i64, _i64, _i64, _p, _p, _p, C.c_int, C.POINTER(_p)]),
@@ -71,6 +72,9 @@
     "dmf_cost": (C.c_int, [_p, _p, _p, _i64, _p, C.c_int, _dbl_p]),
     "dmf_cost_describe": (C.c_int, [_i64, _i64, _i64, C.c_int, _i64, C.c_int, C.c_int, C.c_int, C.c_char_p, _i64]),
     "dmf_problem_cost_describe": (C.c_int, [_p, _p, _i64, C.c_char_p, _i64]),
+    "dmf_problem_cost_source": (C.c_char_p, [_p, _i64]),
+    "dmf_problem_quotient_exact": (C.c_int, [_p, C.POINTER(C.c_int), C.POINTER(_i64)]),
+    "dmf_x16_quotient_check": (_i64, [_i64, C.POINTER(_i64), C.POINTER(_i64)]),
     "dmf_project_simplex": (C.c_int, [_p, _p, _i64, _i64, C.c_double, C.c_int, _p]),
     "dmf_update_u": (C.c_int, [_p, _p, _p, _p, _p, _i64, _i64, C.c_int, C.c_int, _dbl_p, _p, _p]),
     "dmf_update_alpha": (C.c_int, [_p, _p, _p, _i64, _p, _p, _i64, C.c_int, _dbl_p, _p, _p]),
diff --git a/demethify_amd/csrc/dmf_api.h b/demethify_amd/csrc/dmf_api.h
--- a/demethify_amd/csrc/dmf_api.h
+++ b/demethify_amd/csrc/dmf_api.h
@@ -53,6 +53,7 @@
     int stop_confirmation = 0;
     int generic_level = 0;
     bool x16 = true;
+    bool cost_x16 = true;
     bool rowpass_pair = true;
     double* scratch = nullptr;
     hipMemPool_t pool = nullptr;
@@ -172,6 +173,9 @@
     int64_t N16 = 0, plane_stride = 0;
     dmf_api::DevBuf<unsigned short> X16;
     double x16_dev = 0.0, x16_sum = 0.0;
+    bool quot_exact = false;
+    dmf_api::DevBuf<double> rtab;
+    int rtab_n = 0;
     bool d_f32_exact = false;
     dmf_api::DevBuf<double> gb_known;
     dmf::GramRan known_ran;
@@ -181,6 +185,7 @@
     dmf::ProblemView view() const {
         dmf::ProblemView v;
         v.V = V, v.D = D, v.D16 = D16, v.X16 = X16, v.Dt8 = Dt8;
+        v.rtab = rtab, v.rtab_n = rtab_n;
         v.plane_stride = plane_stride, v.SD = SD, v.ND = ND;
         v.Rt = Rt, v.Rtp = Rtp;
         v.N = N, v.S = (int)S, v.n_c = (int)n_c;
@@ -217,6 +222,7 @@
     SolverState* h_state = nullptr;
     dmf_api::JobTable jobs;
     bool cf_pending = true;
+    bool state_fresh = false;
     double* mom_host = nullptr;
     dmf_api::DevBuf<double> mom_dev;
     hipEvent_t cost_event = nullptr;
diff --git a/demethify_amd/csrc/dmf_api_context.hip b/demethify_amd/csrc/dmf_api_context.hip
--- a/demethify_amd/csrc/dmf_api_context.hip
+++ b/demethify_amd/csrc/dmf_api_context.hip
@@ -312,6 +312,12 @@
     return DMF_OK;
 }
 
+int dmf_context_set_cost_x16(dmf_context* ctx, int enabled) {
+    if (ctx == nullptr || enabled < 0 || enabled > 1) return DMF_ERR_BAD_ARG;
+    ctx->cost_x16 = enabled != 0;
+    return DMF_OK;
+}
+
 int dmf_context_set_rowpass_pair(dmf_context* ctx, int enabled) {
     if (ctx == nullptr || enabled < 0 || enabled > 1) return DMF_ERR_BAD_ARG;
     ctx->rowpass_pair = enabled != 0;
diff --git a/demethify_amd/csrc/dmf_api_entry.hip b/demethify_amd/csrc/dmf_api_entry.hip
--- a/demethify_amd/csrc/dmf_api_entry.hip
+++ b/demethify_amd/csrc/dmf_api_entry.hip
@@ -99,6 +99,24 @@
     key.level = level;
     dmf::describe_cost_plan(dmf::cost_plan(key), buf, (size_t)cap);
     return DMF_OK;
+}
+
+int64_t dmf_x16_quotient_check(int64_t dmax, int64_t* mismatches, int64_t* mismatches_q0) {
+    if (dmax < 1 || dmax > 32639 || mismatches == nullptr || mismatches_q0 == nullptr) return -1;
+    int64_t pairs = 0, bad = 0, bad_q0 = 0;
+    for (int64_t di = 1; di <= dmax; ++di) {
+        const double d = (double)di;
+        volatile double one = 1.0;
+        const double r_d = one / d;
+        for (int64_t xi = 0; xi <= di; ++xi) {
+            const double x = (double)xi, want = x / d;
+            bad += dmf::x16_quotient(x, d, r_d) != want;
+            bad_q0 += x * r_d != want;
+        }
+        pairs += di + 1;
+    }
+    *mismatches = bad, *mismatches_q0 = bad_q0;
+    return pairs;
 }
 
 int dmf_gram_i8_describe(int64_t N, int64_t S, int64_t n_c, int64_t n_u, int nd, char* buf, int64_t cap) {
diff --git a/demethify_amd/csrc/dmf_api_problem.hip b/demethify_amd/csrc/dmf_api_problem.hip
--- a/demethify_amd/csrc/dmf_api_problem.hip
+++ b/demethify_amd/csrc/dmf_api_problem.hip
@@ -60,11 +60,11 @@
         S <= 2048 && n_c <= 48) {
         DMF_TRY(alloc_count_copies(p, h[kIntCountMax] <= 127.0 ? 1 : 2, ctx->x16, false));
         DevBuf<unsigned long long> x_stats;
-        if (ctx->x16) HIP_TRY(x_stats.alloc(ctx, 3));
+        if (ctx->x16) HIP_TRY(x_stats.alloc(ctx, 4));
         HIP_TRY(dmf::launch_build_counts_int(p->D, p->V, N, (int)S, p->ND, p->D16, p->X16, p->N16, p->SD, p->Dt8,
                                              p->plane_stride, x_stats, ctx->stream));
         if (p->X16 != nullptr) {
-            unsigned long long got[3] = {1, 0, 0};
+            unsigned long long got[4] = {1, 0, 0, 1};
             HIP_TRY(hipMemcpyAsync(got, x_stats, sizeof(got), hipMemcpyDeviceToHost, ctx->stream));
             HIP_TRY(hipStreamSynchronize(ctx->stream));
             if (got[0] != 0) {
@@ -72,8 +72,15 @@
             } else {
                 std::memcpy(&p->x16_dev, &got[1], sizeof(double));
                 p->x16_sum = (double)got[2];
+                p->quot_exact = got[3] == 0;
             }
         }
+    }
+    if (p->X16 == nullptr) p->quot_exact = false;
+    if (p->quot_exact && h[kDmax] >= 0.0 && h[kDmax] <= (double)dmf::kCostX16MaxCount) {
+        p->rtab_n = (int)h[kDmax] + 1;
+        HIP_TRY(p->rtab.alloc(ctx, (size_t)p->rtab_n));
+        HIP_TRY(dmf::launch_recip_table(p->rtab, p->rtab_n, ctx->stream));
     }
 
     if (n_c > 0 && n_c <= 48) {
@@ -149,7 +156,7 @@
 }
 
 static dmf::CostPlan cost_plan_of(dmf_context* ctx, const dmf::ProblemView& p, int n_u) {
-    return dmf::cost_plan(dmf::cost_key(p, n_u, ctx->generic_level));
+    return dmf::cost_plan(dmf::cost_key(p, n_u, ctx->generic_level, ctx->cost_x16));
 }
 
 hipError_t enqueue_cost(dmf_context* ctx, const dmf::ProblemView& p, const double* u, const double* alpha, int n_u,
@@ -217,6 +224,7 @@
         p->h_consts[kF32ResidualMax] = src->h_consts[kF32ResidualMax];
         p->h_consts[kRtOutsideUnit] = src->h_consts[kRtOutsideUnit];
         p->x16_dev = x16 ? src->x16_dev : 0.0;
+        p->quot_exact = x16 && src->quot_exact;
         p->x16_sum = (double)h_xsum;
         counts_done = true;
     }
@@ -325,6 +333,7 @@
     p->h_consts[kIntCountMax] = std::isfinite(src->h_consts[kIntCountMax]) ? dmax : src->h_consts[kIntCountMax];
     p->h_consts[kRtOutsideUnit] = src->h_consts[kRtOutsideUnit];
     p->x16_dev = x16 ? src->x16_dev : 0.0;
+    p->quot_exact = x16 && src->quot_exact;
     p->x16_sum = (double)h_stats[1];
     p->n_test = (int64_t)h_stats[2];
     DMF_TRY(problem_finalize(p.get(), true));
@@ -343,6 +352,18 @@
     if (ctx == nullptr || p == nullptr || buf == nullptr || cap < 1 || n_u < 0 || p->ctx != ctx) return DMF_ERR_BAD_ARG;
     if (p->n_c + n_u < 1 || p->n_c + n_u > dmf::kMaxK) return DMF_ERR_BAD_ARG;
     dmf::describe_cost_plan(cost_plan_of(ctx, p->view(), (int)n_u), buf, (size_t)cap);
+    return DMF_OK;
+}
+
+const char* dmf_problem_cost_source(const dmf_problem* p, int64_t n_u) {
+    if (p == nullptr || p->ctx == nullptr || n_u < 0 || p->n_c + n_u < 1 || p->n_c + n_u > dmf::kMaxK) return nullptr;
+    return cost_plan_of(p->ctx, p->view(), (int)n_u).x16 ? "x16" : "v";
+}
+
+int dmf_problem_quotient_exact(const dmf_problem* p, int* exact, int64_t* table_len) {
+    if (p == nullptr || exact == nullptr) return DMF_ERR_BAD_ARG;
+    *exact = p->quot_exact ? 1 : 0;
+    if (table_len != nullptr) *table_len = p->rtab != nullptr ? p->rtab_n : 0;
     return DMF_OK;
 }
 
diff --git a/demethify_amd/csrc/dmf_api_solver.hip b/demethify_amd/csrc/dmf_api_solver.hip
--- a/demethify_amd/csrc/dmf_api_solver.hip
+++ b/demethify_amd/csrc/dmf_api_solver.hip
@@ -219,12 +219,17 @@
 
 constexpr int kMomRows = 64, kMomSteps = 64;
 
-__global__ void k_set_momentum(SolverState* state, const double* mom, int stride, int rows, int n) {
+__global__ void k_set_momentum(SolverState* state, const double* mom, int stride, int rows, int n, int set_tol, double tol,
+                               double band) {
     state->mom = mom;
     state->mom_stride = stride;
     state->mom_rows = rows;
     state->mom_i = 0;
     state->mom_n = n;
+    if (set_tol) {
+        state->tol = tol;
+        state->band = band;
+    }
 }
 
 static double momentum_advance(double& a) {
@@ -235,7 +240,7 @@
     return (a0 - 1.0) / a;
 }
 
-static int upload_momentum_rows(dmf_solver* s, int rows, int n) {
+static int upload_momentum_rows(dmf_solver* s, int rows, int n, bool set_tol, double tol, double band) {
     dmf_context* ctx = s->ctx;
     const int stride = 2 + 2 * n;
     if (s->mom_host == nullptr) {
@@ -259,7 +264,7 @@
     }
     HIP_TRY(hipMemcpyAsync(s->mom_dev, s->mom_host, (size_t)rows * stride * sizeof(double), hipMemcpyHostToDevice, ctx->stream));
     hipLaunchKernelGGL(k_set_momentum, dim3(1), dim3(1), 0, ctx->stream, s->state.get(), (const double*)s->mom_dev.get(), stride,
-                       rows, n);
+                       rows, n, set_tol ? 1 : 0, tol, band);
     HIP_TRY(hipGetLastError());
     return DMF_OK;
 }
@@ -380,13 +385,17 @@
     HIP_TRY(hipMemsetAsync(s->state, 0, sizeof(SolverState), ctx->stream));
     HIP_TRY(hipMemsetAsync(s->gb, 0, gbn * sizeof(double), ctx->stream));
     HIP_TRY(hipMemcpyAsync(s->u, u0, un * sizeof(double), in_kind, ctx->stream));
-    HIP_TRY(hipMemcpyAsync(s->u_prev, s->u, un * sizeof(double), hipMemcpyDeviceToDevice, ctx->stream));
     HIP_TRY(hipMemcpyAsync(s->alpha, alpha0, an * sizeof(double), in_kind, ctx->stream));
     HIP_TRY(hipMemcpyAsync(s->alpha_prev, s->alpha, an * sizeof(double), hipMemcpyDeviceToDevice, ctx->stream));
     DMF_TRY(s->jobs.upload(ctx));
     HIP_TRY(dmf::launch_scatter_known_block(p->gb_known, s->gb, (int)n_c, (int)K, (int)S, ctx->stream));
-    HIP_TRY(dmf::launch_sumsq_f64(s->u, N * n_u, ctx->scratch, &s->state->u_norm2, nullptr, ctx->stream));
-    HIP_TRY(dmf::launch_init_state(s->state, p->consts, s->alpha, (int)S, (int)n_c, (int)n_u, ctx->stream));
+    int n_u2 = 0;
+    HIP_TRY(dmf::launch_sumsq_copy_partials(s->u, s->u_prev, N * n_u, ctx->scratch, &n_u2, ctx->stream));
+    HIP_TRY(dmf::launch_init_state(s->state, p->consts, s->alpha, (int)S, (int)n_c, (int)n_u, ctx->scratch, n_u2, ctx->stream));
+    std::memset(s->h_state, 0, sizeof(SolverState));
+    s->h_state->a1 = s->h_state->a2 = 1.0;
+    s->h_state->mom_n = -1;
+    s->state_fresh = true;
     if (!(flags & DMF_PTR_DEVICE)) HIP_TRY(hipStreamSynchronize(ctx->stream));
     return DMF_OK;
 }
@@ -425,15 +434,16 @@
     const double gram_err = kGramCostRelErr * (double)p->N * (double)p->S * p->h_consts[kDmax] +
                             (s->key.x16 ? p->x16_dev * p->x16_sum : 0.0);
     s->confirm_stops = tol > 0.0 && ctx->stop_confirmation != 2 && (ctx->stop_confirmation == 1 || gram_err >= tol / 20.0);
-    hipLaunchKernelGGL(k_set_tol, dim3(1), dim3(1), 0, ctx->stream, s->state.get(), tol, s->confirm_stops ? kConfirmBand : 1.0);
-    HIP_TRY(hipGetLastError());
+    const double band = s->confirm_stops ? kConfirmBand : 1.0;
+    bool tol_due = true;
     if (s->cf_pending && tol > 0.0 && n_outer > 0) {
         FamilyScope scope(ctx, DMF_KERNEL_COST);
         HIP_TRY(enqueue_cost(ctx, p->view(), s->u, s->alpha, (int)s->n_u, ctx->scratch + 1024, &s->state->cf));
         s->cf_pending = false;
         s->cf_stream_iter = -2;
     }
-    DMF_TRY(fetch_state(s));
+    if (!(s->state_fresh && tol == 0.0)) DMF_TRY(fetch_state(s));
+    s->state_fresh = false;
     if (s->cf_stream_iter == -2) {
         s->cf_stream = s->h_state->cf;
         s->cf_stream_iter = s->h_state->iters;
@@ -445,13 +455,22 @@
     const bool use_mom = n_iter2 >= 1 && n_iter2 <= kMomSteps && plan.row == dmf::RowKind::RowpassV2 &&
                          plan.alpha == dmf::AlphaKind::PhaseRow16;
     if (!use_mom && s->h_state->mom_n >= 0) {
-        hipLaunchKernelGGL(k_set_momentum, dim3(1), dim3(1), 0, ctx->stream, s->state.get(), (const double*)nullptr, 0, 0, -1);
+        hipLaunchKernelGGL(k_set_momentum, dim3(1), dim3(1), 0, ctx->stream, s->state.get(), (const double*)nullptr, 0, 0, -1, 1,
+                           tol, band);
         HIP_TRY(hipGetLastError());
+        tol_due = false;
     }
     while (s->h_state->iters - iters0 < n_outer && s->h_state->done != 1) {
         const int64_t left = n_outer - (s->h_state->iters - iters0);
         const int64_t batch = left < check_every ? left : check_every;
-        if (use_mom) DMF_TRY(upload_momentum_rows(s, (int)batch, (int)n_iter2));
+        if (use_mom) {
+            DMF_TRY(upload_momentum_rows(s, (int)batch, (int)n_iter2, tol_due, tol, band));
+            tol_due = false;
+        } else if (tol_due) {
+            hipLaunchKernelGGL(k_set_tol, dim3(1), dim3(1), 0, ctx->stream, s->state.get(), tol, band);
+            HIP_TRY(hipGetLastError());
+            tol_due = false;
+        }
         for (int64_t b = 0; b < batch; ++b) DMF_TRY(enqueue_outer_iteration(s, (int)n_iter2));
         DMF_TRY(fetch_state(s));
         if (s->h_state->iters > iters0) s->cf_pending = false;
@@ -475,6 +494,11 @@
             check_every *= 2;
         }
     }
+    if (tol_due) {
+        hipLaunchKernelGGL(k_set_tol, dim3(1), dim3(1), 0, ctx->stream, s->state.get(), tol, band);
+        HIP_TRY(hipGetLastError());
+        s->in_flight = true;
+    }
     if (iters_done_total) *iters_done_total = s->h_state->iters;
     if (converged) *converged = s->h_state->done == 1;
     return DMF_OK;
diff --git a/demethify_amd/csrc/dmf_internal.h b/demethify_amd/csrc/dmf_internal.h
--- a/demethify_amd/csrc/dmf_internal.h
+++ b/demethify_amd/csrc/dmf_internal.h
@@ -58,6 +58,8 @@
     const double* D = nullptr;
     const unsigned short* D16 = nullptr;
     const unsigned short* X16 = nullptr;
+    const double* rtab = nullptr;
+    int rtab_n = 0;
     const signed char* Dt8 = nullptr;
     int64_t plane_stride = 0;
     int SD = 0, ND = 0;
@@ -118,16 +120,19 @@
 hipError_t launch_unit_range_check(const double* x, int64_t n, double* scratch, double* out, hipStream_t st);
 hipError_t launch_sumsq_f64(const double* x, int64_t n, double* scratch, double* out,
                             const int* done_flag, hipStream_t st);
+hipError_t launch_sumsq_copy_partials(const double* x, double* copy, int64_t n, double* partial, int* n_partials,
+                                      hipStream_t st);
 hipError_t launch_pad_rows(const double* src, double* dst, int64_t n_rows, int width_src, int width_dst,
                            hipStream_t st);
 hipError_t launch_index_range_check(const long long* idx, int64_t n_idx, int64_t n_src, unsigned int* flag, hipStream_t st);
 hipError_t launch_gather_rows(const double* src, double* dst, const long long* idx, int64_t n_idx,
                               int64_t width, hipStream_t st);
 
-inline CostKey cost_key(const ProblemView& p, int n_u, int level) {
+inline CostKey cost_key(const ProblemView& p, int n_u, int level, bool x16_on = false) {
     CostKey k;
     k.S = p.S, k.n_c = p.n_c, k.n_u = n_u;
     k.d16 = p.D16 != nullptr;
+    k.x16 = x16_on && p.X16 != nullptr && p.rtab != nullptr && p.rtab_n >= 1 && p.rtab_n <= kCostX16MaxCount + 1;
     k.SD = p.SD;
     k.v_align = p.v_align();
     k.rtp_present = p.Rtp != nullptr;
@@ -136,6 +141,7 @@
 }
 hipError_t launch_cost_plan(const CostPlan& plan, const ProblemView& p, const double* u, const double* alpha, int n_u,
                             double* scratch, double* out, hipStream_t st);
+hipError_t launch_recip_table(double* r, int n, hipStream_t st);
 int vdv_cols_grid(int64_t N);
 hipError_t launch_vdv_cols(const ProblemView& p, double* slab, double* out, hipStream_t st);
 
@@ -211,7 +217,7 @@
 hipError_t launch_scatter_known_block(const double* gb_known, double* gb, int n_c, int K, int S,
                                       hipStream_t st);
 hipError_t launch_init_state(SolverState* state, const double* consts, const double* alpha,
-                             int S, int n_c, int n_u, hipStream_t st);
+                             int S, int n_c, int n_u, const double* u2_partials, int n_partials, hipStream_t st);
 
 int64_t u_phase_split_cm_doubles(int64_t N, int n_u);
 hipError_t launch_u_phase_split(const ProblemView& p, const IterateView& it, int n_iter2, const UScratch& scratch,
@@ -270,6 +276,11 @@
                                     signed char* Dt8, int64_t plane_stride, unsigned int* max_out,
                                     unsigned long long* xsum_out, hipStream_t st);
 constexpr double kX16MaxDev = 8.0 * 0x1p-53;
+__host__ __device__ inline double x16_quotient(double x, double d, double r_d) {
+    const double q0 = x * r_d;
+    const double r = __builtin_fma(-q0, d, x);
+    return __builtin_fma(r, r_d, q0);
+}
 hipError_t launch_build_counts_int(const double* D, const double* V, int64_t N, int S, int ND, unsigned short* D16,
                                    unsigned short* X16, int64_t N16, int SD, signed char* Dt8, int64_t plane_stride,
                                    unsigned long long* x_stats, hipStream_t st);
diff --git a/demethify_amd/csrc/dmf_kernels_alpha.hip b/demethify_amd/csrc/dmf_kernels_alpha.hip
--- a/demethify_amd/csrc/dmf_kernels_alpha.hip
+++ b/demethify_amd/csrc/dmf_kernels_alpha.hip
@@ -753,27 +753,30 @@
                                                        double* __restrict__ gb, int n_c, int K, int S) {
     const int s = blockIdx.x * 256 + threadIdx.x;
     if (s >= S) return;
-    for (int l = 0; l <= n_c; ++l) {
-        const int ld = l == n_c ? K : l;
-        for (int k = 0; k <= l; ++k) {
-            const int kd = k == n_c ? K : k;
-            gb[(int64_t)tri(kd, ld) * S + s] = gb_known[(int64_t)tri(k, l) * S + s];
-        }
-    }
+    const int e = blockIdx.y;
+    int l = 0;
+    while ((l + 1) * (l + 2) / 2 <= e) ++l;
+    const int k = e - l * (l + 1) / 2;
+    const int ld = l == n_c ? K : l, kd = k == n_c ? K : k;
+    gb[(int64_t)tri(kd, ld) * S + s] = gb_known[(int64_t)e * S + s];
 }
 
 hipError_t launch_scatter_known_block(const double* gb_known, double* gb, int n_c, int K, int S,
                                       hipStream_t st) {
-    hipLaunchKernelGGL(k_scatter_known, dim3((S + 255) / 256), dim3(256), 0, st, gb_known, gb, n_c, K, S);
+    hipLaunchKernelGGL(k_scatter_known, dim3((S + 255) / 256, (n_c + 1) * (n_c + 2) / 2), dim3(256), 0, st, gb_known, gb, n_c,
+                       K, S);
     return hipGetLastError();
 }
 
 __global__ __launch_bounds__(256) void k_init_state(SolverState* __restrict__ state,
                                                     const double* __restrict__ consts,
                                                     const double* __restrict__ alpha, int S, int n_c,
-                                                    int n_u) {
+                                                    int n_u, const double* __restrict__ u2_partials, int n_partials) {
     __shared__ double red[4];
     double acc = 0.0;
+    for (int i = threadIdx.x; i < n_partials; i += 256) acc += u2_partials[i];
+    const double u2 = block_sum<256>(acc, red);
+    acc = 0.0;
     const double* A2 = alpha + (int64_t)n_c * S;
     for (int i = threadIdx.x; i < n_u * S; i += 256) acc = fma(A2[i], A2[i], acc);
     const double n2 = block_sum<256>(acc, red);
@@ -785,7 +788,8 @@
         state->rt_norm2 = rt2;
         state->l_w = n2 * dsq;
         state->l_w_prev = state->l_w;
-        state->l_h = (rt2 + state->u_norm2) * dsq;
+        state->u_norm2 = u2;
+        state->l_h = (rt2 + u2) * dsq;
         state->l_h_prev = state->l_h;
         state->cf = __longlong_as_double(0x7FF8000000000000ll);
         state->cf_prev = state->cf;
@@ -800,8 +804,8 @@
 }
 
 hipError_t launch_init_state(SolverState* state, const double* consts, const double* alpha, int S,
-                             int n_c, int n_u, hipStream_t st) {
-    hipLaunchKernelGGL(k_init_state, dim3(1), dim3(256), 0, st, state, consts, alpha, S, n_c, n_u);
+                             int n_c, int n_u, const double* u2_partials, int n_partials, hipStream_t st) {
+    hipLaunchKernelGGL(k_init_state, dim3(1), dim3(256), 0, st, state, consts, alpha, S, n_c, n_u, u2_partials, n_partials);
     return hipGetLastError();
 }
 
diff --git a/demethify_amd/csrc/dmf_kernels_gram_i8.hip b/demethify_amd/csrc/dmf_kernels_gram_i8.hip
--- a/demethify_amd/csrc/dmf_kernels_gram_i8.hip
+++ b/demethify_amd/csrc/dmf_kernels_gram_i8.hip
@@ -23,7 +23,7 @@
                                                    unsigned short* __restrict__ D16, unsigned short* __restrict__ X16,
                                                    int64_t N16, int SD, unsigned long long* __restrict__ x_stats) {
     const int64_t chunks = N16 * (SD / 8);
-    unsigned long long bad = 0, xsum = 0;
+    unsigned long long bad = 0, xsum = 0, qbad = 0;
     double dev = 0.0;
     for (int64_t c = (int64_t)blockIdx.x * 256 + threadIdx.x; c < chunks; c += (int64_t)gridDim.x * 256) {
         const int64_t row = c / (SD / 8);
@@ -47,9 +47,12 @@
                             xh[h] = (unsigned int)x;
                             xsum += xh[h];
                             dev = fmax(dev, err / xm);
+                            if (v != x / d) ++qbad;
                         } else {
                             ++bad;
                         }
+                    } else if (X16 != nullptr && !isfinite(V[row * S + col])) {
+                        ++qbad;
                     }
                 }
             }
@@ -64,23 +67,27 @@
     for (int off = 32; off > 0; off >>= 1) {
         bad += __shfl_xor(bad, off, 64);
         xsum += __shfl_xor(xsum, off, 64);
+        qbad += __shfl_xor(qbad, off, 64);
         dev = fmax(dev, __shfl_xor(dev, off, 64));
     }
-    __shared__ unsigned long long wst[4][3];
+    __shared__ unsigned long long wst[4][4];
     const int wave = threadIdx.x >> 6;
     if ((threadIdx.x & 63) == 0) {
         wst[wave][0] = bad;
         wst[wave][1] = (unsigned long long)__double_as_longlong(dev);
         wst[wave][2] = xsum;
+        wst[wave][3] = qbad;
     }
     __syncthreads();
     if (threadIdx.x == 0) {
-        unsigned long long b = 0, m = 0, x = 0;
+        unsigned long long b = 0, m = 0, x = 0, q = 0;
         for (int w = 0; w < 4; ++w) {
             b += wst[w][0];
             m = m > wst[w][1] ? m : wst[w][1];
             x += wst[w][2];
-        }
+            q += wst[w][3];
+        }
+        if (q > 0) atomicAdd(x_stats + 3, q);
         if (b > 0) atomicAdd(x_stats, b);
         if (m > 0) atomicMax(x_stats + 1, m);
         if (x > 0) atomicAdd(x_stats + 2, x);
@@ -124,7 +131,7 @@
     if (g < 1) g = 1;
     if (X16 != nullptr) {
         if (V == nullptr || x_stats == nullptr) return hipErrorInvalidValue;
-        const hipError_t e = hipMemsetAsync(x_stats, 0, 3 * sizeof(unsigned long long), st);
+        const hipError_t e = hipMemsetAsync(x_stats, 0, 4 * sizeof(unsigned long long), st);
         if (e != hipSuccess) return e;
     }
     hipLaunchKernelGGL(k_build_d16, dim3((unsigned)g), dim3(256), 0, st, D, V, N, S, D16, X16, N16, SD, x_stats);
diff --git a/demethify_amd/csrc/dmf_kernels_stream.hip b/demethify_amd/csrc/dmf_kernels_stream.hip
--- a/demethify_amd/csrc/dmf_kernels_stream.hip
+++ b/demethify_amd/csrc/dmf_kernels_stream.hip
@@ -99,6 +99,29 @@
     return hipGetLastError();
 }
 
+__global__ __launch_bounds__(256) void k_sumsq_copy_partial(const double* __restrict__ x, double* __restrict__ copy, int64_t n,
+                                                            double* __restrict__ partial) {
+    __shared__ double red[4];
+    double acc = 0.0;
+    int64_t i = (int64_t)blockIdx.x * 256 + threadIdx.x;
+    const int64_t stride = (int64_t)gridDim.x * 256;
+    for (; i < n; i += stride) {
+        const double v = x[i];
+        copy[i] = v;
+        acc = fma(v, v, acc);
+    }
+    const double tot = block_sum<256>(acc, red);
+    if (threadIdx.x == 0) partial[blockIdx.x] = tot;
+}
+
+hipError_t launch_sumsq_copy_partials(const double* x, double* copy, int64_t n, double* partial, int* n_partials,
+                                      hipStream_t st) {
+    const int nb = reduce_blocks(n);
+    hipLaunchKernelGGL(k_sumsq_copy_partial, dim3(nb), dim3(256), 0, st, x, copy, n, partial);
+    *n_partials = nb;
+    return hipGetLastError();
+}
+
 __global__ __launch_bounds__(256) void k_gather_rows(const double* __restrict__ src,
                                                      double* __restrict__ dst,
                                                      const long long* __restrict__ idx,
@@ -271,21 +294,43 @@
     if (threadIdx.x == 0) partial[blockIdx.y * gridDim.x + blockIdx.x] = tot;
 }
 
-template <int NKC, int NU, bool ODD>
-__global__ __launch_bounds__(256) void k_cost_cols2(const double* __restrict__ V, const unsigned short* __restrict__ Dh, int SD,
-                                                    const double* __restrict__ Rtp, const double* __restrict__ u,
-                                                    const double* __restrict__ alpha, int64_t N, int S, int n_c,
-                                                    double* __restrict__ partial) {
+template <int NCT, int NU>
+__device__ __forceinline__ const double* row_feature(const double* __restrict__ Rtp, const double* __restrict__ u, int64_t row,
+                                                     int feat) {
+    if constexpr (NCT == 0) return u + row * NU + (feat < NU ? feat : 0);
+    else if constexpr (NU == 0) return Rtp + row * NCT + (feat < NCT ? feat : 0);
+    else return feat >= NCT && feat < NCT + NU ? u + row * NU + (feat - NCT) : Rtp + row * NCT + (feat < NCT ? feat : 0);
+}
+
+__device__ __forceinline__ double lane_value(double v, int k) {
+    const long long b = __double_as_longlong(v);
+    const unsigned int lo = (unsigned int)__builtin_amdgcn_readlane((int)(unsigned int)b, k);
+    const unsigned int hi = (unsigned int)__builtin_amdgcn_readlane((int)(unsigned int)((unsigned long long)b >> 32), k);
+    return __longlong_as_double((long long)(((unsigned long long)hi << 32) | lo));
+}
+
+template <int NKC, int NU, bool ODD, bool X16>
+__device__ __forceinline__ void cost_cols2_body(const double* __restrict__ V, const unsigned short* __restrict__ Xh,
+                                                const double* __restrict__ rtab, int rtab_n, const unsigned short* __restrict__ Dh,
+                                                int SD, const double* __restrict__ Rtp, const double* __restrict__ u,
+                                                const double* __restrict__ alpha, int64_t N, int S, int n_c,
+                                                double* __restrict__ partial, double* __restrict__ rt) {
     typedef double v2d __attribute__((ext_vector_type(2)));
     constexpr int NCT = 4 * NKC;
     constexpr int kRows = 8;
     __shared__ double red[4];
+    if constexpr (X16) {
+        for (int i = threadIdx.x; i < rtab_n; i += 256) rt[i] = rtab[i];
+        __syncthreads();
+    }
     const int wave = __builtin_amdgcn_readfirstlane(threadIdx.x >> 6), lane = threadIdx.x & 63;
     const int s = blockIdx.y * 128 + 2 * lane;
     const bool active = s < S;
     const bool lone = ODD && s == S - 1;
     const int sc = lone ? S - 2 : (active ? s : 0);
     const int sd = active ? s : 0;
+    constexpr int kFeatLanes = NCT + NU <= 16 ? 16 : 32, kRowsPerLoad = 64 / kFeatLanes, kFeatLoads = kRows / kRowsPerLoad;
+    const int feat = lane & (kFeatLanes - 1), slot = lane / kFeatLanes;
     typedef double v2d_u __attribute__((ext_vector_type(2), aligned(8)));
     double ak[NCT > 0 ? NCT : 1][2], aj[NU > 0 ? NU : 1][2];
 #pragma unroll
@@ -304,14 +349,26 @@
     const int64_t stride = (int64_t)gridDim.x * 4;
     for (int64_t i0 = (int64_t)blockIdx.x * 4 + wave; i0 < N; i0 += kRows * stride) {
         v2d v[kRows];
-        unsigned int dd[kRows];
+        unsigned int dd[kRows], xx[kRows];
+        double rf[kFeatLoads];
         int64_t row[kRows];
+        if constexpr (X16) {
+#pragma unroll
+            for (int m = 0; m < kFeatLoads; ++m) {
+                const int64_t i = i0 + (m * kRowsPerLoad + slot) * stride;
+                rf[m] = *row_feature<NCT, NU>(Rtp, u, i < N ? i : N - 1, feat);
+            }
+        }
 #pragma unroll
         for (int x = 0; x < kRows; ++x) {
             const int64_t i = i0 + x * stride;
             row[x] = i < N ? i : N - 1;
-            const v2d_u vl = *reinterpret_cast<const v2d_u*>(V + row[x] * S + sc);
-            v[x] = v2d{lone ? vl.y : vl.x, vl.y};
+            if constexpr (X16) {
+                xx[x] = *reinterpret_cast<const unsigned int*>(Xh + row[x] * SD + sd);
+            } else {
+                const v2d_u vl = *reinterpret_cast<const v2d_u*>(V + row[x] * S + sc);
+                v[x] = v2d{lone ? vl.y : vl.x, vl.y};
+            }
             dd[x] = *reinterpret_cast<const unsigned int*>(Dh + row[x] * SD + sd);
             if (i >= N) dd[x] = 0u;
         }
@@ -322,15 +379,20 @@
             double p0 = 0.0, p1 = 0.0;
 #pragma unroll
             for (int k = 0; k < NCT; ++k) {
-                const double r = rt_row[k];
+                const double r = X16 ? lane_value(rf[x / kRowsPerLoad], (x % kRowsPerLoad) * kFeatLanes + k) : rt_row[k];
                 p0 = fma(r, ak[k][0], p0);
                 p1 = fma(r, ak[k][1], p1);
             }
 #pragma unroll
             for (int j = 0; j < NU; ++j) {
-                const double r = u_row[j];
+                const double r = X16 ? lane_value(rf[x / kRowsPerLoad], (x % kRowsPerLoad) * kFeatLanes + NCT + j) : u_row[j];
                 p0 = fma(r, aj[j][0], p0);
                 p1 = fma(r, aj[j][1], p1);
+            }
+            if constexpr (X16) {
+                const unsigned int d0 = dd[x] & 0xFFFFu, d1 = dd[x] >> 16;
+                v[x] = v2d{x16_quotient((double)(xx[x] & 0xFFFFu), (double)d0, rt[d0]),
+                           x16_quotient((double)(xx[x] >> 16), (double)d1, rt[d1])};
             }
             const double e0 = v[x].x - p0, e1 = v[x].y - p1;
             acc0 = fma((double)(dd[x] & 0xFFFFu) * e0, e0, acc0);
@@ -341,6 +403,35 @@
     if (!active) acc = 0.0;
     const double tot = block_sum<256>(acc, red);
     if (threadIdx.x == 0) partial[blockIdx.y * gridDim.x + blockIdx.x] = tot;
+}
+
+template <int NKC, int NU, bool ODD>
+__global__ __launch_bounds__(256) void k_cost_cols2(const double* __restrict__ V, const unsigned short* __restrict__ Dh, int SD,
+                                                    const double* __restrict__ Rtp, const double* __restrict__ u,
+                                                    const double* __restrict__ alpha, int64_t N, int S, int n_c,
+                                                    double* __restrict__ partial) {
+    cost_cols2_body<NKC, NU, ODD, false>(V, nullptr, nullptr, 0, Dh, SD, Rtp, u, alpha, N, S, n_c, partial, nullptr);
+}
+
+template <int NKC, int NU, bool ODD>
+__global__ __launch_bounds__(256) __attribute__((amdgpu_waves_per_eu(4 * NKC + NU <= 16 ? 4 : 3, 8))) void k_cost_cols2_x16(const unsigned short* __restrict__ Xh, const double* __restrict__ rtab,
+                                                        int rtab_n, const unsigned short* __restrict__ Dh, int SD,
+                                                        const double* __restrict__ Rtp, const double* __restrict__ u,
+                                                        const double* __restrict__ alpha, int64_t N, int S, int n_c,
+                                                        double* __restrict__ partial) {
+    extern __shared__ double rt_lds[];
+    cost_cols2_body<NKC, NU, ODD, true>(nullptr, Xh, rtab, rtab_n, Dh, SD, Rtp, u, alpha, N, S, n_c, partial, rt_lds);
+}
+
+__global__ __launch_bounds__(256) void k_recip_table(double* __restrict__ r, int n) {
+    const int i = blockIdx.x * 256 + threadIdx.x;
+    if (i < n) r[i] = i > 0 ? 1.0 / (double)i : 0.0;
+}
+
+hipError_t launch_recip_table(double* r, int n, hipStream_t st) {
+    if (r == nullptr || n < 1) return hipErrorInvalidValue;
+    hipLaunchKernelGGL(k_recip_table, dim3((n + 255) / 256), dim3(256), 0, st, r, n);
+    return hipGetLastError();
 }
 
 template <bool D16>
@@ -417,6 +508,7 @@
         if (pair_ok && S >= 128) {
             plan.kind = CostKind::Cols2;
             plan.d16 = true;
+            plan.x16 = k.x16;
             return plan;
         }
         if ((S + 63) / 64 <= kCostPartials) {
@@ -454,10 +546,25 @@
 }
 
 template <int NKC, int NU>
-static hipError_t launch_cost_cols2_t(bool odd, const ProblemView& p, const double* u, const double* alpha, double* scratch,
-                                      double* out, hipStream_t st) {
+static hipError_t launch_cost_cols2_t(bool odd, bool x16, const ProblemView& p, const double* u, const double* alpha,
+                                      double* scratch, double* out, hipStream_t st) {
     const int S = p.S, ny2 = (S + 127) / 128;
     const int nbx = cost_cols_row_blocks(p.N, ny2);
+    if constexpr (NU <= 4) {
+        if (x16) {
+            const size_t lds = (size_t)p.rtab_n * sizeof(double);
+            if (odd)
+                hipLaunchKernelGGL((k_cost_cols2_x16<NKC, NU, true>), dim3(nbx, ny2), dim3(256), lds, st, p.X16, p.rtab, p.rtab_n,
+                                   p.D16, p.SD, p.Rtp, u, alpha, p.N, S, p.n_c, scratch);
+            else
+                hipLaunchKernelGGL((k_cost_cols2_x16<NKC, NU, false>), dim3(nbx, ny2), dim3(256), lds, st, p.X16, p.rtab, p.rtab_n,
+                                   p.D16, p.SD, p.Rtp, u, alpha, p.N, S, p.n_c, scratch);
+            hipLaunchKernelGGL(k_reduce_final<1>, dim3(1), dim3(256), 0, st, scratch, nbx * ny2, out, (const int*)nullptr);
+            return hipGetLastError();
+        }
+    } else if (x16) {
+        return hipErrorInvalidValue;
+    }
     if (odd)
         hipLaunchKernelGGL((k_cost_cols2<NKC, NU, true>), dim3(nbx, ny2), dim3(256), 0, st, p.V, p.D16, p.SD, p.Rtp, u, alpha,
                            p.N, S, p.n_c, scratch);
@@ -505,6 +612,9 @@
          (p.n_c > 0 && p.Rtp == nullptr)))
         return hipErrorInvalidValue;
     if (plan.kind == CostKind::Generic && p.D == nullptr) return hipErrorInvalidValue;
+    if (plan.x16 && (plan.kind != CostKind::Cols2 || p.X16 == nullptr || p.rtab == nullptr || p.rtab_n < 1 ||
+                     p.rtab_n > kCostX16MaxCount + 1))
+        return hipErrorInvalidValue;
     switch (plan.kind) {
         case CostKind::Cols:
         case CostKind::Cols2:
@@ -512,15 +622,15 @@
                 return dispatch_int<0, 4>(plan.nu, [&](auto nu) {
                     constexpr int NKC = decltype(nkc)::value, NU = decltype(nu)::value;
                     if (plan.kind == CostKind::Cols2)
-                        return launch_cost_cols2_t<NKC, NU>(plan.odd, p, u, alpha, scratch, out, st);
+                        return launch_cost_cols2_t<NKC, NU>(plan.odd, plan.x16, p, u, alpha, scratch, out, st);
                     return launch_cost_cols_t<NKC, NU>(plan.d16, p, u, alpha, scratch, out, st);
                 });
             });
         case CostKind::Cols2Wide:
             return dispatch_int<0, 4>(plan.nkc, [&](auto nkc) {
                 return dispatch_int<5, 16>(plan.nu, [&](auto nu) {
-                    return launch_cost_cols2_t<decltype(nkc)::value, decltype(nu)::value>(plan.odd, p, u, alpha, scratch, out,
-                                                                                         st);
+                    return launch_cost_cols2_t<decltype(nkc)::value, decltype(nu)::value>(plan.odd, false, p, u, alpha, scratch,
+                                                                                         out, st);
                 });
             });
         default: return launch_cost(plan.alpha_in_lds, p, u, alpha, n_u, scratch, out, st);
diff --git a/demethify_amd/csrc/dmf_select.h b/demethify_amd/csrc/dmf_select.h
--- a/demethify_amd/csrc/dmf_select.h
+++ b/demethify_amd/csrc/dmf_select.h
@@ -65,6 +65,7 @@
     unsigned v_align = 0;
     bool rtp_present = true;
     int level = 0;
+    bool x16 = false;
 };
 enum class CostKind {
     Cols,
@@ -78,8 +79,10 @@
     bool d16 = false;
     bool odd = false;
     bool alpha_in_lds = false;
+    bool x16 = false;
 };
 constexpr int kCostPartials = 1024;
+constexpr int kCostX16MaxCount = 4095;
 CostPlan cost_plan(const CostKey& k);
 int describe_cost_plan(const CostPlan& plan, char* buf, size_t cap);
 
diff --git a/demethify_amd/device.py b/demethify_amd/device.py
--- a/demethify_amd/device.py
+++ b/demethify_amd/device.py
@@ -84,6 +84,9 @@
 
     def set_x16(self, enabled: bool):
         L.check(self._lib.dmf_context_set_x16(self._h, int(bool(enabled))), "dmf_context_set_x16")
+
+    def set_cost_x16(self, enabled: bool):
+        L.check(self._lib.dmf_context_set_cost_x16(self._h, int(bool(enabled))), "dmf_context_set_cost_x16")
 
     def set_rowpass_pair(self, enabled: bool):
         L.check(self._lib.dmf_context_set_rowpass_pair(self._h, int(bool(enabled))), "dmf_context_set_rowpass_pair")
@@ -300,6 +303,17 @@
                 "dmf_problem_cost_describe")
         return buf.value.decode()
 
+    def cost_source(self, n_u: int) -> str:
+        got = self._lib.dmf_problem_cost_source(self._h, int(n_u))
+        if got is None:
+            raise ValueError(f"no cost plan for n_u = {n_u}")
+        return got.decode()
+
+    def quotient_exact(self):
+        exact, n = C.c_int(), C.c_int64()
+        L.check(self._lib.dmf_problem_quotient_exact(self._h, C.byref(exact), C.byref(n)), "dmf_problem_quotient_exact")
+        return bool(exact.value), int(n.value)
+
     def gram_known(self):
         out = np.empty(((self.n_c + 1) * (self.n_c + 2) // 2, self.S), dtype=np.float64)
         buf = C.create_string_buffer(256)
diff --git a/include/demethify_hip.h b/include/demethify_hip.h
--- a/include/demethify_hip.h
+++ b/include/demethify_hip.h
@@ -61,6 +61,7 @@
 int dmf_context_reset_kernel_time(dmf_context* ctx);
 int dmf_context_set_generic(dmf_context* ctx, int level);
 int dmf_context_set_x16(dmf_context* ctx, int enabled);
+int dmf_context_set_cost_x16(dmf_context* ctx, int enabled);
 int dmf_context_set_rowpass_pair(dmf_context* ctx, int enabled);
 int dmf_context_set_stop_confirmation(dmf_context* ctx, int mode);
 
@@ -88,6 +89,9 @@
 int dmf_cost_describe(int64_t S, int64_t n_c, int64_t n_u, int has_u16, int64_t SD, int v_align, int rtp_present, int level,
                       char* buf, int64_t cap);
 int dmf_problem_cost_describe(dmf_context* ctx, const dmf_problem* p, int64_t n_u, char* buf, int64_t cap);
+const char* dmf_problem_cost_source(const dmf_problem* p, int64_t n_u);
+int dmf_problem_quotient_exact(const dmf_problem* p, int* exact, int64_t* table_len);
+int64_t dmf_x16_quotient_check(int64_t dmax, int64_t* mismatches, int64_t* mismatches_q0);
 int dmf_gram_i8_describe(int64_t N, int64_t S, int64_t n_c, int64_t n_u, int nd, char* buf, int64_t cap);
 int dmf_project_simplex(dmf_context* ctx, const double* X, int64_t K, int64_t S, double z,
                         int flags, double* out);
```
